# status-im/nim-blscurve

Measured on NVIDIA B200. Metric: batch-verified signature sets/sec, higher is better.
Workload: dtype u32x12 (Fp 381-bit Montgomery)

## Files before the change

nim_blscurve_b200/csrc/acc_team.cuh:

```cuda
#pragma once
#include "pairing.cuh"

namespace bls {

#define ACC_TPW 5
#define ACC_BS 128
#define ACC_TPB (ACC_TPW * ACC_BS / 32)

enum { FV_C0 = 0, FV_C1 = 1, FV_S = 2, FV_D = 3, FV_DD = 4 };
struct __align__(16) acc_team_sm {
    fp f[6][5];
    fp l[9];
};

#ifdef __CUDACC__
template <int K>
__device__ __forceinline__ void fp_dot(fp &r, const uint32_t (&a)[K][12], const fp *const (&b)[K]) {
#ifdef __CUDA_ARCH__
    uint32_t E[13], O[12];
#pragma unroll
    for (int i = 0; i < 12; i++) { E[i] = 0; O[i] = 0; }
    E[12] = 0;
    uint32_t bl[K][4];
#pragma unroll
    for (int i = 0; i < 12; i++) {
        if ((i & 3) == 0) {
#pragma unroll
            for (int t = 0; t < K; t++) {
                uint4 v = ((const uint4 *)b[t])[i >> 2];
                bl[t][0] = v.x; bl[t][1] = v.y; bl[t][2] = v.z; bl[t][3] = v.w;
            }
        }
        if (i == 0) {
            mad6(O, a[0][1], a[0][3], a[0][5], a[0][7], a[0][9], a[0][11], bl[0][0]);
        } else {
            uint32_t s = E[1];
            uint32_t nO[12];
#pragma unroll
            for (int k = 0; k < 11; k++) nO[k] = E[k + 2];
            nO[11] = 0;
#pragma unroll
            for (int k = 0; k < 12; k++) E[k] = O[k];
            E[12] = 0;
#pragma unroll
            for (int k = 0; k < 12; k++) O[k] = nO[k];
            mad6_stray(O, E[0], s, a[0][1], a[0][3], a[0][5], a[0][7], a[0][9], a[0][11], bl[0][i & 3]);
        }
        mad6_top(E, a[0][0], a[0][2], a[0][4], a[0][6], a[0][8], a[0][10], bl[0][i & 3]);
#pragma unroll
        for (int t = 1; t < K; t++) {
            mad6(O, a[t][1], a[t][3], a[t][5], a[t][7], a[t][9], a[t][11], bl[t][i & 3]);
            mad6_top(E, a[t][0], a[t][2], a[t][4], a[t][6], a[t][8], a[t][10], bl[t][i & 3]);
        }
        const uint32_t m = E[0] * BLS_N0;
        mad6(O, P32(1), P32(3), P32(5), P32(7), P32(9), P32(11), m);
        mad6_top(E, P32(0), P32(2), P32(4), P32(6), P32(8), P32(10), m);
    }
    add12(O, E + 1);
    reduce_once12(r.l, O);
#endif
}

__device__ __forceinline__ void load_fp_regs(uint32_t (&dst)[12], const fp *src) {
    const uint4 *s = (const uint4 *)src;
    uint4 v0 = s[0], v1 = s[1], v2 = s[2];
    dst[0] = v0.x; dst[1] = v0.y; dst[2] = v0.z; dst[3] = v0.w;
    dst[4] = v1.x; dst[5] = v1.y; dst[6] = v1.z; dst[7] = v1.w;
    dst[8] = v2.x; dst[9] = v2.y; dst[10] = v2.z; dst[11] = v2.w;
}

__device__ __noinline__ void team_dot3(fp &r, const fp *a0, const fp *a1, const fp *a2, const fp *b0, const fp *b1, const fp *b2) {
    uint32_t a[3][12];
    load_fp_regs(a[0], a0);
    load_fp_regs(a[1], a1);
    load_fp_regs(a[2], a2);
    const fp *const b[3] = {b0, b1, b2};
    fp t;
    fp_dot<3>(t, a, b);
    r = t;
}

__device__ __noinline__ void team_dot4(fp &r, const fp *const *ap, const fp *const *bp, uint32_t dbl_mask, uint32_t zero_mask) {
    uint32_t a[4][12];
#pragma unroll
    for (int t = 0; t < 4; t++) {
        fp x;
        load_fp_regs(x.l, ap[t]);
        fp x2;
        fp_dbl(x2, x);
        const bool d = (dbl_mask >> t) & 1, z = (zero_mask >> t) & 1;
#pragma unroll
        for (int i = 0; i < 12; i++) a[t][i] = z ? 0u : (d ? x2.l[i] : x.l[i]);
    }
    const fp *const b[4] = {bp[0], bp[1], bp[2], bp[3]};
    fp t;
    fp_dot<4>(t, a, b);
    r = t;
}

__device__ __forceinline__ void team_store_coeff(acc_team_sm &T, int k, const fp &c0, const fp &c1) {
    fp s, d, dd;
    fp_add(s, c0, c1);
    fp_sub(d, c0, c1);
    fp_dbl(dd, c0);
    T.f[k][FV_C0] = c0;
    T.f[k][FV_C1] = c1;
    T.f[k][FV_S] = s;
    T.f[k][FV_D] = d;
    T.f[k][FV_DD] = dd;
}

__device__ __forceinline__ void team_operand(const acc_team_sm &T, int j, bool x, const fp *&re, const fp *&im, const fp *&sum) {
    re = x ? &T.f[j][FV_D] : &T.f[j][FV_C0];
    im = x ? &T.f[j][FV_S] : &T.f[j][FV_C1];
    sum = x ? &T.f[j][FV_DD] : &T.f[j][FV_S];
}

__device__ __forceinline__ void team_mul_line(acc_team_sm &T, int k, uint32_t mask) {
    const fp *x0[3], *x1[3], *sx[3];
    team_operand(T, k, false, x0[0], x1[0], sx[0]);
    team_operand(T, (k + 4) % 6, k < 2, x0[1], x1[1], sx[1]);
    team_operand(T, (k + 3) % 6, k < 3, x0[2], x1[2], sx[2]);
    fp D0, D1, D2, c0, c1;
    team_dot3(D0, &T.l[0], &T.l[2], &T.l[4], x0[0], x0[1], x0[2]);
    team_dot3(D1, &T.l[1], &T.l[3], &T.l[5], x1[0], x1[1], x1[2]);
    team_dot3(D2, &T.l[6], &T.l[7], &T.l[8], sx[0], sx[1], sx[2]);
    fp_sub(c0, D0, D1);
    fp_sub(c1, D2, D0);
    fp_sub(c1, c1, D1);
    __syncwarp(mask);
    team_store_coeff(T, k, c0, c1);
    __syncwarp(mask);
}

__device__ __forceinline__ void team_square(acc_team_sm &T, int k, uint32_t mask) {
    const int LI[6][4] = {{0, 3, 1, 2}, {0, 2, 3, 0}, {1, 4, 0, 3}, {0, 1, 4, 0}, {2, 5, 0, 1}, {0, 1, 2, 0}};
    const int RI[6][4] = {{0, 3, 5, 4}, {1, 5, 4, 0}, {1, 4, 2, 5}, {3, 2, 5, 0}, {2, 5, 4, 3}, {5, 4, 3, 0}};
    const int XI[6][4] = {{0, 1, 1, 1}, {0, 1, 1, 0}, {0, 1, 0, 1}, {0, 0, 1, 0}, {0, 1, 0, 0}, {0, 0, 0, 0}};
    const uint32_t DBL[6] = {0xc, 0x7, 0xc, 0x7, 0xc, 0x7}, ZERO[6] = {0, 8, 0, 8, 0, 8};
    const fp *a0[4], *a1[4], *as[4], *b0[4], *b1[4], *bs[4];
#pragma unroll
    for (int t = 0; t < 4; t++) {
        team_operand(T, RI[k][t], false, a0[t], a1[t], as[t]);
        team_operand(T, LI[k][t], XI[k][t] != 0, b0[t], b1[t], bs[t]);
    }
    fp D0, D1, D2, c0, c1;
    team_dot4(D0, a0, b0, DBL[k], ZERO[k]);
    team_dot4(D1, a1, b1, DBL[k], ZERO[k]);
    team_dot4(D2, as, bs, DBL[k], ZERO[k]);
    fp_sub(c0, D0, D1);
    fp_sub(c1, D2, D0);
    fp_sub(c1, c1, D1);
    __syncwarp(mask);
    team_store_coeff(T, k, c0, c1);
    __syncwarp(mask);
}
#endif

}
```

nim_blscurve_b200/csrc/ec.cuh:

```cuda
#pragma once
#include "fpx.cuh"

namespace bls {

BLS_FN void f_add(fp &r, const fp &a, const fp &b) { fp_add(r, a, b); }
BLS_FN void f_sub(fp &r, const fp &a, const fp &b) { fp_sub(r, a, b); }
BLS_FN void f_dbl(fp &r, const fp &a) { fp_dbl(r, a); }
BLS_FN void f_neg(fp &r, const fp &a) { fp_neg(r, a); }
BLS_FN void f_mul(fp &r, const fp &a, const fp &b) { fp_mul_ni(r, a, b); }
BLS_FN void f_sqr(fp &r, const fp &a) { fp_sqr_ni(r, a); }
BLS_FN bool f_is_zero(const fp &a) { return fp_is_zero(a); }
BLS_FN bool f_eq(const fp &a, const fp &b) { return fp_eq(a, b); }
BLS_FN void f_set_zero(fp &r) { fp_set_zero(r); }
BLS_FN void f_set_one(fp &r) { r = FP_ONE; }
BLS_FN void f_inv(fp &r, const fp &a) { fp_inv(r, a); }

BLS_FN void f_add(fp2 &r, const fp2 &a, const fp2 &b) { fp2_add(r, a, b); }
BLS_FN void f_sub(fp2 &r, const fp2 &a, const fp2 &b) { fp2_sub(r, a, b); }
BLS_FN void f_dbl(fp2 &r, const fp2 &a) { fp2_dbl(r, a); }
BLS_FN void f_neg(fp2 &r, const fp2 &a) { fp2_neg(r, a); }
BLS_FN void f_mul(fp2 &r, const fp2 &a, const fp2 &b) { fp2_mul(r, a, b); }
BLS_FN void f_sqr(fp2 &r, const fp2 &a) { fp2_sqr(r, a); }
BLS_FN bool f_is_zero(const fp2 &a) { return fp2_is_zero(a); }
BLS_FN bool f_eq(const fp2 &a, const fp2 &b) { return fp2_eq(a, b); }
BLS_FN void f_set_zero(fp2 &r) { fp2_set_zero(r); }
BLS_FN void f_set_one(fp2 &r) { r.c0 = FP_ONE; fp_set_zero(r.c1); }
BLS_FN void f_inv(fp2 &r, const fp2 &a) { fp2_inv(r, a); }
BLS_FN void f_inv_vt(fp &r, const fp &a) { fp_inv_vartime(r, a); }
BLS_FN void f_inv_vt(fp2 &r, const fp2 &a) { fp2_inv_vartime(r, a); }

template <class F> struct jac_t { F x, y, z; };
template <class F> struct aff_t { F x, y; };
typedef jac_t<fp> g1_jac;
typedef aff_t<fp> g1_aff;
typedef jac_t<fp2> g2_jac;
typedef aff_t<fp2> g2_aff;

template <class F> BLS_FN bool pt_is_inf(const jac_t<F> &p) { return f_is_zero(p.z); }
template <class F> BLS_FN bool aff_is_inf(const aff_t<F> &p) { return f_is_zero(p.x) & f_is_zero(p.y); }
template <class F> BLS_FN void pt_set_inf(jac_t<F> &p) { f_set_zero(p.x); f_set_zero(p.y); f_set_zero(p.z); }
template <class F> BLS_FN void pt_from_affine(jac_t<F> &r, const aff_t<F> &a) {
    r.x = a.x;
    r.y = a.y;
    if (aff_is_inf(a)) f_set_zero(r.z); else f_set_one(r.z);
}
template <class F> BLS_FN void pt_neg(jac_t<F> &r, const jac_t<F> &a) { r.x = a.x; f_neg(r.y, a.y); r.z = a.z; }

template <class F> BLS_NOINLINE void pt_dbl(jac_t<F> &r, const jac_t<F> &p) {
    F A, B, C, D, E, Fq, t;
    f_sqr(A, p.x);
    f_sqr(B, p.y);
    f_sqr(C, B);
    f_add(t, p.x, B);
    f_sqr(t, t);
    f_sub(t, t, A);
    f_sub(t, t, C);
    f_dbl(D, t);
    f_dbl(E, A);
    f_add(E, E, A);
    f_sqr(Fq, E);
    f_mul(t, p.y, p.z);
    f_dbl(r.z, t);
    f_sub(Fq, Fq, D);
    f_sub(Fq, Fq, D);
    f_sub(t, D, Fq);
    f_mul(t, E, t);
    f_dbl(C, C);
    f_dbl(C, C);
    f_dbl(C, C);
    r.x = Fq;
    f_sub(r.y, t, C);
}

template <class F> BLS_NOINLINE void pt_dbl_a(jac_t<F> &r, const jac_t<F> &p, const F &a) {
    F XX, YY, YYYY, ZZ, S, M, T, t;
    f_sqr(XX, p.x);
    f_sqr(YY, p.y);
    f_sqr(YYYY, YY);
    f_sqr(ZZ, p.z);
    f_add(t, p.x, YY);
    f_sqr(t, t);
    f_sub(t, t, XX);
    f_sub(t, t, YYYY);
    f_dbl(S, t);
    f_sqr(t, ZZ);
    f_mul(t, a, t);
    f_dbl(M, XX);
    f_add(M, M, XX);
    f_add(M, M, t);
    f_sqr(T, M);
    f_sub(T, T, S);
    f_sub(T, T, S);
    f_add(t, p.y, p.z);
    f_sqr(t, t);
    f_sub(t, t, YY);
    f_sub(r.z, t, ZZ);
    r.x = T;
    f_sub(t, S, T);
    f_mul(t, M, t);
    f_dbl(YYYY, YYYY);
    f_dbl(YYYY, YYYY);
    f_dbl(YYYY, YYYY);
    f_sub(r.y, t, YYYY);
}

template <class F> BLS_NOINLINE void pt_add(jac_t<F> &r, const jac_t<F> &p, const jac_t<F> &q, const F *a_coeff = nullptr) {
    if (pt_is_inf(p)) { r = q; return; }
    if (pt_is_inf(q)) { r = p; return; }
    F Z1Z1, Z2Z2, U1, U2, S1, S2, H, I, J, rr, V, t;
    f_sqr(Z1Z1, p.z);
    f_sqr(Z2Z2, q.z);
    f_mul(U1, p.x, Z2Z2);
    f_mul(U2, q.x, Z1Z1);
    f_mul(t, q.z, Z2Z2);
    f_mul(S1, p.y, t);
    f_mul(t, p.z, Z1Z1);
    f_mul(S2, q.y, t);
    f_sub(H, U2, U1);
    f_sub(rr, S2, S1);
    if (f_is_zero(H)) {
        if (f_is_zero(rr)) {
            if (a_coeff) pt_dbl_a(r, p, *a_coeff); else pt_dbl(r, p);
        } else {
            pt_set_inf(r);
        }
        return;
    }
    f_dbl(rr, rr);
    f_dbl(I, H);
    f_sqr(I, I);
    f_mul(J, H, I);
    f_mul(V, U1, I);
    f_add(t, p.z, q.z);
    f_sqr(t, t);
    f_sub(t, t, Z1Z1);
    f_sub(t, t, Z2Z2);
    f_mul(r.z, t, H);
    f_sqr(t, rr);
    f_sub(t, t, J);
    f_sub(t, t, V);
    f_sub(t, t, V);
    r.x = t;
    f_sub(t, V, t);
    f_mul(t, rr, t);
    f_mul(S1, S1, J);
    f_dbl(S1, S1);
    f_sub(r.y, t, S1);
}

template <class F> BLS_NOINLINE void pt_add_affine(jac_t<F> &r, const jac_t<F> &p, const aff_t<F> &q) {
    if (aff_is_inf(q)) { r = p; return; }
    if (pt_is_inf(p)) { pt_from_affine(r, q); return; }
    F Z1Z1, U2, S2, H, HH, I, J, rr, V, t;
    f_sqr(Z1Z1, p.z);
    f_mul(U2, q.x, Z1Z1);
    f_mul(t, p.z, Z1Z1);
    f_mul(S2, q.y, t);
    f_sub(H, U2, p.x);
    f_sub(rr, S2, p.y);
    if (f_is_zero(H)) {
        if (f_is_zero(rr)) pt_dbl(r, p); else pt_set_inf(r);
        return;
    }
    f_dbl(rr, rr);
    f_sqr(HH, H);
    f_dbl(I, HH);
    f_dbl(I, I);
    f_mul(J, H, I);
    f_mul(V, p.x, I);
    f_add(t, p.z, H);
    f_sqr(t, t);
    f_sub(t, t, Z1Z1);
    F y1 = p.y;
    f_sub(r.z, t, HH);
    f_sqr(t, rr);
    f_sub(t, t, J);
    f_sub(t, t, V);
    f_sub(t, t, V);
    r.x = t;
    f_sub(t, V, t);
    f_mul(t, rr, t);
    f_mul(J, y1, J);
    f_dbl(J, J);
    f_sub(r.y, t, J);
}

template <class F> BLS_NOINLINE void pt_to_affine(aff_t<F> &r, const jac_t<F> &p) {
    if (pt_is_inf(p)) { f_set_zero(r.x); f_set_zero(r.y); return; }
    F zi, zi2;
    f_inv(zi, p.z);
    f_sqr(zi2, zi);
    f_mul(r.x, p.x, zi2);
    f_mul(zi2, zi2, zi);
    f_mul(r.y, p.y, zi2);
}

template <class F> BLS_NOINLINE void pt_to_affine_vt(aff_t<F> &r, const jac_t<F> &p) {
    if (pt_is_inf(p)) { f_set_zero(r.x); f_set_zero(r.y); return; }
    F zi, zi2;
    f_inv_vt(zi, p.z);
    f_sqr(zi2, zi);
    f_mul(r.x, p.x, zi2);
    f_mul(zi2, zi2, zi);
    f_mul(r.y, p.y, zi2);
}

template <class F> BLS_NOINLINE void pt_to_affine_zinv(aff_t<F> &r, const jac_t<F> &p, const F &zi) {
    if (pt_is_inf(p)) { f_set_zero(r.x); f_set_zero(r.y); return; }
    F zi2;
    f_sqr(zi2, zi);
    f_mul(r.x, p.x, zi2);
    f_mul(zi2, zi2, zi);
    f_mul(r.y, p.y, zi2);
}

template <class F> BLS_NOINLINE void pt_mul_u64(jac_t<F> &r, const aff_t<F> &p, uint64_t k) {
    jac_t<F> acc;
    pt_set_inf(acc);
    if (k != 0 && !aff_is_inf(p)) {
        int top = 63;
        while (!((k >> top) & 1)) top--;
        pt_from_affine(acc, p);
        for (int i = top - 1; i >= 0; i--) {
            pt_dbl(acc, acc);
            if ((k >> i) & 1) pt_add_affine(acc, acc, p);
        }
    }
    r = acc;
}

template <class F> BLS_NOINLINE void pt_mul_u64_w4(jac_t<F> &r, const aff_t<F> &p, uint64_t k) {
    jac_t<F> tbl[8], acc;
    pt_from_affine(tbl[0], p);
    pt_dbl(tbl[1], tbl[0]);
    pt_add_affine(tbl[2], tbl[1], p);
    pt_dbl(tbl[3], tbl[1]);
    pt_add_affine(tbl[4], tbl[3], p);
    pt_dbl(tbl[5], tbl[2]);
    pt_add_affine(tbl[6], tbl[5], p);
    pt_dbl(tbl[7], tbl[3]);
    int dig[17], carry = 0;
    for (int j = 0; j < 16; j++) {
        int w = (int)((k >> (4 * j)) & 15) + carry;
        if (w > 8) { w -= 16; carry = 1; } else carry = 0;
        dig[j] = w;
    }
    dig[16] = carry;
    pt_set_inf(acc);
    for (int j = 16; j >= 0; j--) {
        if (j != 16) for (int d = 0; d < 4; d++) pt_dbl(acc, acc);
        const int d = dig[j];
        if (d != 0) {
            jac_t<F> q = tbl[(d < 0 ? -d : d) - 1];
            if (d < 0) f_neg(q.y, q.y);
            pt_add(acc, acc, q);
        }
    }
    r = acc;
}

template <class F> BLS_NOINLINE void pt_mul_words(jac_t<F> &r, const jac_t<F> &p, const uint32_t *k, int nwords) {
    jac_t<F> acc;
    pt_set_inf(acc);
    int i = nwords * 32 - 1;
    while (i >= 0 && !((k[i >> 5] >> (i & 31)) & 1)) i--;
    for (; i >= 0; i--) {
        pt_dbl(acc, acc);
        if ((k[i >> 5] >> (i & 31)) & 1) pt_add(acc, acc, p);
    }
    r = acc;
}

}
```

nim_blscurve_b200/csrc/fp.cuh:

```cuda
#pragma once
#include <stdint.h>

#ifdef __CUDACC__
#define BLS_FN __device__ __forceinline__
#define BLS_HD __host__ __device__ __forceinline__
#define BLS_NOINLINE __device__ __noinline__
#define BLS_TABLE __device__ __constant__ const
#else
#define BLS_FN static inline
#define BLS_HD static inline
#define BLS_NOINLINE static
#define BLS_TABLE static const
#endif

namespace bls {

struct alignas(16) fp { uint32_t l[12]; };

BLS_FN constexpr uint32_t P32(int i) {
    return i == 0 ? 0xffffaaabu : i == 1 ? 0xb9feffffu : i == 2 ? 0xb153ffffu : i == 3 ? 0x1eabfffeu
         : i == 4 ? 0xf6b0f624u : i == 5 ? 0x6730d2a0u : i == 6 ? 0xf38512bfu : i == 7 ? 0x64774b84u
         : i == 8 ? 0x434bacd7u : i == 9 ? 0x4b1ba7b6u : i == 10 ? 0x397fe69au : 0x1a0111eau;
}
#define BLS_N0 0xfffcfffdu

BLS_FN void fp_set_zero(fp &r) {
#pragma unroll
    for (int i = 0; i < 12; i++) r.l[i] = 0;
}

BLS_FN bool fp_is_zero(const fp &a) {
    uint32_t t = 0;
#pragma unroll
    for (int i = 0; i < 12; i++) t |= a.l[i];
    return t == 0;
}

BLS_FN bool fp_eq(const fp &a, const fp &b) {
    uint32_t t = 0;
#pragma unroll
    for (int i = 0; i < 12; i++) t |= a.l[i] ^ b.l[i];
    return t == 0;
}

BLS_FN void fp_select(fp &r, bool c, const fp &a, const fp &b) {
#pragma unroll
    for (int i = 0; i < 12; i++) r.l[i] = c ? a.l[i] : b.l[i];
}

#ifdef __CUDA_ARCH__
#define BLS_R12(x) "+r"(x[0]), "+r"(x[1]), "+r"(x[2]), "+r"(x[3]), "+r"(x[4]), "+r"(x[5]), \
                   "+r"(x[6]), "+r"(x[7]), "+r"(x[8]), "+r"(x[9]), "+r"(x[10]), "+r"(x[11])

BLS_FN void add12(uint32_t *acc, const uint32_t *b) {
    asm("add.cc.u32 %0,%0,%12;\n\taddc.cc.u32 %1,%1,%13;\n\taddc.cc.u32 %2,%2,%14;\n\t"
        "addc.cc.u32 %3,%3,%15;\n\taddc.cc.u32 %4,%4,%16;\n\taddc.cc.u32 %5,%5,%17;\n\t"
        "addc.cc.u32 %6,%6,%18;\n\taddc.cc.u32 %7,%7,%19;\n\taddc.cc.u32 %8,%8,%20;\n\t"
        "addc.cc.u32 %9,%9,%21;\n\taddc.cc.u32 %10,%10,%22;\n\taddc.u32 %11,%11,%23;"
        : BLS_R12(acc)
        : "r"(b[0]), "r"(b[1]), "r"(b[2]), "r"(b[3]), "r"(b[4]), "r"(b[5]), "r"(b[6]), "r"(b[7]), "r"(b[8]),
          "r"(b[9]), "r"(b[10]), "r"(b[11]));
}

BLS_FN uint32_t sub12(uint32_t *acc, const uint32_t *b) {
    uint32_t bw;
    asm("sub.cc.u32 %0,%0,%13;\n\tsubc.cc.u32 %1,%1,%14;\n\tsubc.cc.u32 %2,%2,%15;\n\t"
        "subc.cc.u32 %3,%3,%16;\n\tsubc.cc.u32 %4,%4,%17;\n\tsubc.cc.u32 %5,%5,%18;\n\t"
        "subc.cc.u32 %6,%6,%19;\n\tsubc.cc.u32 %7,%7,%20;\n\tsubc.cc.u32 %8,%8,%21;\n\t"
        "subc.cc.u32 %9,%9,%22;\n\tsubc.cc.u32 %10,%10,%23;\n\tsubc.cc.u32 %11,%11,%24;\n\t"
        "subc.u32 %12,0,0;"
        : BLS_R12(acc), "=r"(bw)
        : "r"(b[0]), "r"(b[1]), "r"(b[2]), "r"(b[3]), "r"(b[4]), "r"(b[5]), "r"(b[6]), "r"(b[7]), "r"(b[8]),
          "r"(b[9]), "r"(b[10]), "r"(b[11]));
    return bw;
}

BLS_FN uint32_t sub_p12(uint32_t *acc) {
    uint32_t bw;
    asm("sub.cc.u32 %0,%0,0xffffaaab;\n\tsubc.cc.u32 %1,%1,0xb9feffff;\n\tsubc.cc.u32 %2,%2,0xb153ffff;\n\t"
        "subc.cc.u32 %3,%3,0x1eabfffe;\n\tsubc.cc.u32 %4,%4,0xf6b0f624;\n\tsubc.cc.u32 %5,%5,0x6730d2a0;\n\t"
        "subc.cc.u32 %6,%6,0xf38512bf;\n\tsubc.cc.u32 %7,%7,0x64774b84;\n\tsubc.cc.u32 %8,%8,0x434bacd7;\n\t"
        "subc.cc.u32 %9,%9,0x4b1ba7b6;\n\tsubc.cc.u32 %10,%10,0x397fe69a;\n\tsubc.cc.u32 %11,%11,0x1a0111ea;\n\t"
        "subc.u32 %12,0,0;"
        : BLS_R12(acc), "=r"(bw));
    return bw;
}

BLS_FN void add_p12(uint32_t *acc) {
    asm("add.cc.u32 %0,%0,0xffffaaab;\n\taddc.cc.u32 %1,%1,0xb9feffff;\n\taddc.cc.u32 %2,%2,0xb153ffff;\n\t"
        "addc.cc.u32 %3,%3,0x1eabfffe;\n\taddc.cc.u32 %4,%4,0xf6b0f624;\n\taddc.cc.u32 %5,%5,0x6730d2a0;\n\t"
        "addc.cc.u32 %6,%6,0xf38512bf;\n\taddc.cc.u32 %7,%7,0x64774b84;\n\taddc.cc.u32 %8,%8,0x434bacd7;\n\t"
        "addc.cc.u32 %9,%9,0x4b1ba7b6;\n\taddc.cc.u32 %10,%10,0x397fe69a;\n\taddc.u32 %11,%11,0x1a0111ea;"
        : BLS_R12(acc));
}

BLS_FN void reduce_once12(uint32_t *r, const uint32_t *t) {
    uint32_t u[12];
#pragma unroll
    for (int i = 0; i < 12; i++) u[i] = t[i];
    uint32_t bw = sub_p12(u);
#pragma unroll
    for (int i = 0; i < 12; i++) r[i] = bw ? t[i] : u[i];
}

#define BLS_LANE_C(lo, hi, a, b) \
    "madc.lo.cc.u32 " lo "," a "," b "," lo ";\n\tmadc.hi.cc.u32 " hi "," a "," b "," hi ";\n\t"
#define BLS_LANE_0(lo, hi, a, b) \
    "mad.lo.cc.u32 " lo "," a "," b "," lo ";\n\tmadc.hi.cc.u32 " hi "," a "," b "," hi ";\n\t"

BLS_FN void mad6_top(uint32_t *acc, uint32_t x0, uint32_t x1, uint32_t x2, uint32_t x3, uint32_t x4,
                     uint32_t x5, uint32_t m) {
    asm(BLS_LANE_0("%0", "%1", "%13", "%19") BLS_LANE_C("%2", "%3", "%14", "%19")
        BLS_LANE_C("%4", "%5", "%15", "%19") BLS_LANE_C("%6", "%7", "%16", "%19")
        BLS_LANE_C("%8", "%9", "%17", "%19") BLS_LANE_C("%10", "%11", "%18", "%19")
        "addc.u32 %12,%12,0;"
        : BLS_R12(acc), "+r"(acc[12])
        : "r"(x0), "r"(x1), "r"(x2), "r"(x3), "r"(x4), "r"(x5), "r"(m));
}

BLS_FN void mad6(uint32_t *acc, uint32_t x0, uint32_t x1, uint32_t x2, uint32_t x3, uint32_t x4,
                 uint32_t x5, uint32_t m) {
    asm(BLS_LANE_0("%0", "%1", "%12", "%18") BLS_LANE_C("%2", "%3", "%13", "%18")
        BLS_LANE_C("%4", "%5", "%14", "%18") BLS_LANE_C("%6", "%7", "%15", "%18")
        BLS_LANE_C("%8", "%9", "%16", "%18") BLS_LANE_C("%10", "%11", "%17", "%18")
        : BLS_R12(acc)
        : "r"(x0), "r"(x1), "r"(x2), "r"(x3), "r"(x4), "r"(x5), "r"(m));
}

BLS_FN void mad6_stray(uint32_t *acc, uint32_t &lo, uint32_t s, uint32_t x0, uint32_t x1, uint32_t x2,
                       uint32_t x3, uint32_t x4, uint32_t x5, uint32_t m) {
    asm("add.cc.u32 %12,%12,%13;\n\t"
        BLS_LANE_C("%0", "%1", "%14", "%20") BLS_LANE_C("%2", "%3", "%15", "%20")
        BLS_LANE_C("%4", "%5", "%16", "%20") BLS_LANE_C("%6", "%7", "%17", "%20")
        BLS_LANE_C("%8", "%9", "%18", "%20") BLS_LANE_C("%10", "%11", "%19", "%20")
        : BLS_R12(acc), "+r"(lo)
        : "r"(s), "r"(x0), "r"(x1), "r"(x2), "r"(x3), "r"(x4), "r"(x5), "r"(m));
}
#endif

BLS_FN void fp_add(fp &r, const fp &a, const fp &b) {
#ifdef __CUDA_ARCH__
    uint32_t t[12];
#pragma unroll
    for (int i = 0; i < 12; i++) t[i] = a.l[i];
    add12(t, b.l);
    reduce_once12(r.l, t);
#else
    uint32_t t[12], u[12];
    uint64_t c = 0;
    for (int i = 0; i < 12; i++) { c += (uint64_t)a.l[i] + b.l[i]; t[i] = (uint32_t)c; c >>= 32; }
    int64_t bw = 0;
    for (int i = 0; i < 12; i++) { bw += (int64_t)t[i] - P32(i); u[i] = (uint32_t)bw; bw >>= 32; }
    for (int i = 0; i < 12; i++) r.l[i] = bw ? t[i] : u[i];
#endif
}

BLS_FN void fp_sub(fp &r, const fp &a, const fp &b) {
#ifdef __CUDA_ARCH__
    uint32_t t[12], u[12];
#pragma unroll
    for (int i = 0; i < 12; i++) t[i] = a.l[i];
    uint32_t bw = sub12(t, b.l);
#pragma unroll
    for (int i = 0; i < 12; i++) u[i] = t[i];
    add_p12(u);
#pragma unroll
    for (int i = 0; i < 12; i++) r.l[i] = bw ? u[i] : t[i];
#else
    uint32_t t[12];
    int64_t bw = 0;
    for (int i = 0; i < 12; i++) { bw += (int64_t)a.l[i] - b.l[i]; t[i] = (uint32_t)bw; bw >>= 32; }
    uint64_t c = 0;
    for (int i = 0; i < 12; i++) { c += (uint64_t)t[i] + (bw ? P32(i) : 0u); r.l[i] = (uint32_t)c; c >>= 32; }
#endif
}

BLS_FN void fp_neg(fp &r, const fp &a) {
    fp z;
    fp_set_zero(z);
    fp_sub(r, z, a);
}

BLS_FN void fp_cneg(fp &r, const fp &a, bool c) {
    fp n;
    fp_neg(n, a);
    fp_select(r, c, n, a);
}

BLS_FN void fp_dbl(fp &r, const fp &a) { fp_add(r, a, a); }

BLS_FN void fp_mul(fp &r, const fp &a, const fp &b) {
#ifdef __CUDA_ARCH__
    uint32_t E[13], O[12];
#pragma unroll
    for (int i = 0; i < 12; i++) { E[i] = 0; O[i] = 0; }
    E[12] = 0;
#pragma unroll
    for (int i = 0; i < 12; i++) {
        const uint32_t bi = b.l[i];
        if (i == 0) {
            mad6(O, a.l[1], a.l[3], a.l[5], a.l[7], a.l[9], a.l[11], bi);
        } else {
            uint32_t s = E[1];
            uint32_t nO[12];
#pragma unroll
            for (int k = 0; k < 11; k++) nO[k] = E[k + 2];
            nO[11] = 0;
#pragma unroll
            for (int k = 0; k < 12; k++) E[k] = O[k];
            E[12] = 0;
#pragma unroll
            for (int k = 0; k < 12; k++) O[k] = nO[k];
            mad6_stray(O, E[0], s, a.l[1], a.l[3], a.l[5], a.l[7], a.l[9], a.l[11], bi);
        }
        mad6_top(E, a.l[0], a.l[2], a.l[4], a.l[6], a.l[8], a.l[10], bi);
        const uint32_t m = E[0] * BLS_N0;
        mad6(O, P32(1), P32(3), P32(5), P32(7), P32(9), P32(11), m);
        mad6_top(E, P32(0), P32(2), P32(4), P32(6), P32(8), P32(10), m);
    }
    add12(O, E + 1);
    reduce_once12(r.l, O);
#else
#ifdef BLS_COUNT_MULS
    extern unsigned long long g_fp_mul_count;
    g_fp_mul_count++;
#endif
    uint32_t t[14];
    for (int i = 0; i < 14; i++) t[i] = 0;
    for (int i = 0; i < 12; i++) {
        uint64_t c = 0;
        for (int j = 0; j < 12; j++) {
            c += (uint64_t)a.l[j] * b.l[i] + t[j];
            t[j] = (uint32_t)c; c >>= 32;
        }
        c += t[12]; t[12] = (uint32_t)c; t[13] = (uint32_t)(c >> 32);
        uint32_t m = t[0] * BLS_N0;
        c = ((uint64_t)m * P32(0) + t[0]) >> 32;
        for (int j = 1; j < 12; j++) {
            c += (uint64_t)m * P32(j) + t[j];
            t[j - 1] = (uint32_t)c; c >>= 32;
        }
        c += t[12]; t[11] = (uint32_t)c;
        t[12] = t[13] + (uint32_t)(c >> 32);
    }
    uint32_t u[12];
    int64_t bw = 0;
    for (int i = 0; i < 12; i++) { bw += (int64_t)t[i] - P32(i); u[i] = (uint32_t)bw; bw >>= 32; }
    for (int i = 0; i < 12; i++) r.l[i] = bw ? t[i] : u[i];
#endif
}

}
#include "fp_gen.cuh"
namespace bls {

BLS_FN void fp_sqr(fp &r, const fp &a) {
#if defined(__CUDA_ARCH__) && !defined(BLS_NO_FP_SQR)
    uint32_t t[12];
    fp_sqr_ptx(t, a.l);
    reduce_once12(r.l, t);
#else
    fp_mul(r, a, a);
#endif
}

BLS_FN void fp_from_mont(fp &r, const fp &a) {
    fp one;
    fp_set_zero(one);
    one.l[0] = 1;
    fp_mul(r, a, one);
}

BLS_FN uint32_t fp_parity(const fp &a) {
    fp t;
    fp_from_mont(t, a);
    return t.l[0] & 1;
}

BLS_FN bool fp_is_lexically_largest_canon(const fp &c) {
    uint64_t carry = 0;
    uint32_t d[13];
    for (int i = 0; i < 12; i++) {
        carry += ((uint64_t)c.l[i] << 1);
        d[i] = (uint32_t)carry;
        carry >>= 32;
    }
    d[12] = (uint32_t)carry;
    int64_t bw = 0;
    for (int i = 0; i < 12; i++) { bw += (int64_t)d[i] - P32(i); bw >>= 32; }
    bw += d[12];
    return bw >= 0;
}

}
```

nim_blscurve_b200/csrc/fp2.cuh:

```cuda
#pragma once
#include "fp.cuh"

namespace bls {

struct fp2 { fp c0, c1; };

BLS_NOINLINE void fp_mul_ni(fp &r, const fp &a, const fp &b) {
    fp x = a, y = b, t;
    fp_mul(t, x, y);
    r = t;
}
BLS_NOINLINE void fp_sqr_ni(fp &r, const fp &a) {
    fp x = a, t;
    fp_sqr(t, x);
    r = t;
}

#if defined(__CUDACC__) && !defined(BLS_SMALL_CODE)
#define BLS_SMALL_CODE 1
#endif
#if defined(BLS_SMALL_CODE) && BLS_SMALL_CODE >= 2
BLS_NOINLINE void fp_add_ni(fp &r, const fp &a, const fp &b) { fp t; fp_add(t, a, b); r = t; }
BLS_NOINLINE void fp_sub_ni(fp &r, const fp &a, const fp &b) { fp t; fp_sub(t, a, b); r = t; }
#define FP_ADD fp_add_ni
#define FP_SUB fp_sub_ni
#define FP_MUL fp_mul_ni
#elif defined(BLS_SMALL_CODE) && BLS_SMALL_CODE >= 1
#define FP_ADD fp_add
#define FP_SUB fp_sub
#define FP_MUL fp_mul_ni
#else
#define FP_ADD fp_add
#define FP_SUB fp_sub
#define FP_MUL fp_mul
#endif

BLS_FN void fp2_set_zero(fp2 &r) { fp_set_zero(r.c0); fp_set_zero(r.c1); }
BLS_FN bool fp2_is_zero(const fp2 &a) { return fp_is_zero(a.c0) & fp_is_zero(a.c1); }
BLS_FN bool fp2_eq(const fp2 &a, const fp2 &b) { return fp_eq(a.c0, b.c0) & fp_eq(a.c1, b.c1); }
BLS_FN void fp2_select(fp2 &r, bool c, const fp2 &a, const fp2 &b) {
    fp_select(r.c0, c, a.c0, b.c0);
    fp_select(r.c1, c, a.c1, b.c1);
}
BLS_FN void fp2_add(fp2 &r, const fp2 &a, const fp2 &b) { FP_ADD(r.c0, a.c0, b.c0); FP_ADD(r.c1, a.c1, b.c1); }
BLS_FN void fp2_sub(fp2 &r, const fp2 &a, const fp2 &b) { FP_SUB(r.c0, a.c0, b.c0); FP_SUB(r.c1, a.c1, b.c1); }
BLS_FN void fp2_neg(fp2 &r, const fp2 &a) { fp_neg(r.c0, a.c0); fp_neg(r.c1, a.c1); }
BLS_FN void fp2_dbl(fp2 &r, const fp2 &a) { FP_ADD(r.c0, a.c0, a.c0); FP_ADD(r.c1, a.c1, a.c1); }
BLS_FN void fp2_conj(fp2 &r, const fp2 &a) { r.c0 = a.c0; fp_neg(r.c1, a.c1); }
BLS_FN void fp2_cneg(fp2 &r, const fp2 &a, bool c) { fp_cneg(r.c0, a.c0, c); fp_cneg(r.c1, a.c1, c); }

BLS_FN void fp2_mul_xi(fp2 &r, const fp2 &a) {
    fp t0, t1;
    FP_SUB(t0, a.c0, a.c1);
    FP_ADD(t1, a.c0, a.c1);
    r.c0 = t0;
    r.c1 = t1;
}

#ifdef __CUDA_ARCH__
BLS_FN void mul_wide12(uint32_t *T, const uint32_t *a, const uint32_t *b) {
    uint32_t E[13], O[12];
#pragma unroll
    for (int i = 0; i < 12; i++) { E[i] = 0; O[i] = 0; }
    E[12] = 0;
#pragma unroll
    for (int i = 0; i < 12; i++) {
        const uint32_t bi = b[i];
        if (i == 0) {
            mad6(O, a[1], a[3], a[5], a[7], a[9], a[11], bi);
        } else {
            uint32_t s = E[1];
            uint32_t nO[12];
#pragma unroll
            for (int k = 0; k < 11; k++) nO[k] = E[k + 2];
            nO[11] = 0;
#pragma unroll
            for (int k = 0; k < 12; k++) E[k] = O[k];
            E[12] = 0;
#pragma unroll
            for (int k = 0; k < 12; k++) O[k] = nO[k];
            mad6_stray(O, E[0], s, a[1], a[3], a[5], a[7], a[9], a[11], bi);
        }
        mad6_top(E, a[0], a[2], a[4], a[6], a[8], a[10], bi);
        T[i] = E[0];
    }
    add12(O, E + 1);
#pragma unroll
    for (int k = 0; k < 12; k++) T[12 + k] = O[k];
}
BLS_FN void redc24(uint32_t *r, const uint32_t *T) {
    uint32_t E[13], O[12];
#pragma unroll
    for (int i = 0; i < 12; i++) { E[i] = T[i]; O[i] = 0; }
    E[12] = 0;
#pragma unroll
    for (int i = 0; i < 12; i++) {
        uint32_t m;
        if (i == 0) {
            m = E[0] * BLS_N0;
            mad6(O, P32(1), P32(3), P32(5), P32(7), P32(9), P32(11), m);
        } else {
            uint32_t s = E[1];
            uint32_t nO[12];
#pragma unroll
            for (int k = 0; k < 11; k++) nO[k] = E[k + 2];
            nO[11] = 0;
#pragma unroll
            for (int k = 0; k < 12; k++) E[k] = O[k];
            E[12] = 0;
#pragma unroll
            for (int k = 0; k < 12; k++) O[k] = nO[k];
            m = (E[0] + s) * BLS_N0;
            mad6_stray(O, E[0], s, P32(1), P32(3), P32(5), P32(7), P32(9), P32(11), m);
        }
        mad6_top(E, P32(0), P32(2), P32(4), P32(6), P32(8), P32(10), m);
    }
    add12(O, E + 1);
    add12(O, T + 12);
    reduce_once12(r, O);
}
BLS_FN uint32_t sub12_b(uint32_t *acc, const uint32_t *b, uint32_t bw_in) {
    uint32_t bw;
    asm("{\n\t.reg .u32 t;\n\tsub.cc.u32 t,0,%25;\n\tsubc.cc.u32 %0,%0,%13;\n\tsubc.cc.u32 %1,%1,%14;\n\tsubc.cc.u32 %2,%2,%15;\n\t"
        "subc.cc.u32 %3,%3,%16;\n\tsubc.cc.u32 %4,%4,%17;\n\tsubc.cc.u32 %5,%5,%18;\n\t"
        "subc.cc.u32 %6,%6,%19;\n\tsubc.cc.u32 %7,%7,%20;\n\tsubc.cc.u32 %8,%8,%21;\n\t"
        "subc.cc.u32 %9,%9,%22;\n\tsubc.cc.u32 %10,%10,%23;\n\tsubc.cc.u32 %11,%11,%24;\n\t"
        "subc.u32 %12,0,0;\n\t}"
        : BLS_R12(acc), "=r"(bw)
        : "r"(b[0]), "r"(b[1]), "r"(b[2]), "r"(b[3]), "r"(b[4]), "r"(b[5]), "r"(b[6]), "r"(b[7]), "r"(b[8]),
          "r"(b[9]), "r"(b[10]), "r"(b[11]), "r"(bw_in));
    return bw;
}
BLS_FN uint32_t sub24(uint32_t *acc, const uint32_t *b) {
    const uint32_t bw = sub12(acc, b);
    return sub12_b(acc + 12, b + 12, bw);
}
#endif

BLS_NOINLINE void fp2_mul_r3(fp2 &r, const fp2 &a, const fp2 &b) {
    fp s0, s1, t0, t1, t2;
    FP_ADD(s0, a.c0, a.c1);
    FP_ADD(s1, b.c0, b.c1);
    FP_MUL(t2, s0, s1);
    FP_MUL(t0, a.c0, b.c0);
    FP_MUL(t1, a.c1, b.c1);
    FP_SUB(t2, t2, t0);
    FP_SUB(t2, t2, t1);
    FP_SUB(t0, t0, t1);
    r.c0 = t0;
    r.c1 = t2;
}

#ifndef BLS_FP2_LAZY
#define BLS_FP2_LAZY 0
#endif

BLS_NOINLINE void fp2_mul(fp2 &r, const fp2 &a, const fp2 &b) {
#if defined(__CUDA_ARCH__) && BLS_FP2_LAZY
    uint32_t T2[24], T0[24];
    {
        uint32_t s0[12], s1[12];
#pragma unroll
        for (int i = 0; i < 12; i++) { s0[i] = a.c0.l[i]; s1[i] = b.c0.l[i]; }
        add12(s0, a.c1.l);
        add12(s1, b.c1.l);
        mul_wide12(T2, s0, s1);
    }
    mul_wide12(T0, a.c0.l, b.c0.l);
    sub24(T2, T0);
    {
        uint32_t T1[24];
        mul_wide12(T1, a.c1.l, b.c1.l);
        sub24(T2, T1);
        const uint32_t bw = sub24(T0, T1);
        uint32_t u[12];
#pragma unroll
        for (int i = 0; i < 12; i++) u[i] = T0[12 + i];
        add_p12(u);
#pragma unroll
        for (int i = 0; i < 12; i++) T0[12 + i] = bw ? u[i] : T0[12 + i];
    }
    fp re, im;
    redc24(im.l, T2);
    redc24(re.l, T0);
    r.c0 = re;
    r.c1 = im;
    return;
#else
    fp2_mul_r3(r, a, b);
#endif
}

BLS_NOINLINE void fp2_sqr(fp2 &r, const fp2 &a) {
    fp s, d, t, u;
    FP_ADD(s, a.c0, a.c1);
    FP_SUB(d, a.c0, a.c1);
    FP_MUL(u, s, d);
    FP_MUL(t, a.c0, a.c1);
    FP_ADD(t, t, t);
    r.c0 = u;
    r.c1 = t;
}

BLS_FN void fp2_mul_fp(fp2 &r, const fp2 &a, const fp &k) {
    fp_mul_ni(r.c0, a.c0, k);
    fp_mul_ni(r.c1, a.c1, k);
}

BLS_FN void fp2_mul3(fp2 &r, const fp2 &a) { fp2 t; fp2_dbl(t, a); fp2_add(r, t, a); }
BLS_FN void fp_mul3(fp &r, const fp &a) { fp t; fp_dbl(t, a); fp_add(r, t, a); }

}
```

nim_blscurve_b200/csrc/fp2h.cuh:

```cuda
#pragma once
#include "tower.cuh"

namespace bls {
#ifdef __CUDACC__

struct fp2h { fp v; };

__device__ __forceinline__ bool h_odd() { return (threadIdx.x & 1) != 0; }
__device__ __forceinline__ uint32_t h_mask() { return 3u << (threadIdx.x & 30); }

__device__ __forceinline__ void h_xchg(fp &r, const fp &a) {
    const uint32_t m = h_mask();
#pragma unroll
    for (int i = 0; i < 12; i++) r.l[i] = __shfl_xor_sync(m, a.l[i], 1);
}
__device__ __forceinline__ bool h_both(bool mine) {
    const uint32_t m = h_mask();
    return mine & (__shfl_xor_sync(m, (int)mine, 1) != 0);
}
__device__ __forceinline__ void h_take(fp2h &r, const fp2 &a) { r.v = h_odd() ? a.c1 : a.c0; }
__device__ __forceinline__ void h_full(fp2 &r, const fp2h &a) {
    fp o;
    h_xchg(o, a.v);
    const bool odd = h_odd();
    fp_select(r.c0, odd, o, a.v);
    fp_select(r.c1, odd, a.v, o);
}

__device__ __forceinline__ void fp_dot2(fp &r, const fp &x0, const fp &y0, const fp &x1, const fp &y1) {
#ifdef __CUDA_ARCH__
    uint32_t E[13], O[12];
#pragma unroll
    for (int i = 0; i < 12; i++) { E[i] = 0; O[i] = 0; }
    E[12] = 0;
#pragma unroll
    for (int i = 0; i < 12; i++) {
        if (i == 0) {
            mad6(O, x0.l[1], x0.l[3], x0.l[5], x0.l[7], x0.l[9], x0.l[11], y0.l[0]);
        } else {
            uint32_t s = E[1];
            uint32_t nO[12];
#pragma unroll
            for (int k = 0; k < 11; k++) nO[k] = E[k + 2];
            nO[11] = 0;
#pragma unroll
            for (int k = 0; k < 12; k++) E[k] = O[k];
            E[12] = 0;
#pragma unroll
            for (int k = 0; k < 12; k++) O[k] = nO[k];
            mad6_stray(O, E[0], s, x0.l[1], x0.l[3], x0.l[5], x0.l[7], x0.l[9], x0.l[11], y0.l[i]);
        }
        mad6_top(E, x0.l[0], x0.l[2], x0.l[4], x0.l[6], x0.l[8], x0.l[10], y0.l[i]);
        mad6(O, x1.l[1], x1.l[3], x1.l[5], x1.l[7], x1.l[9], x1.l[11], y1.l[i]);
        mad6_top(E, x1.l[0], x1.l[2], x1.l[4], x1.l[6], x1.l[8], x1.l[10], y1.l[i]);
        const uint32_t m = E[0] * BLS_N0;
        mad6(O, P32(1), P32(3), P32(5), P32(7), P32(9), P32(11), m);
        mad6_top(E, P32(0), P32(2), P32(4), P32(6), P32(8), P32(10), m);
    }
    add12(O, E + 1);
    reduce_once12(r.l, O);
#endif
}

BLS_NOINLINE void h_mul(fp2h &r, const fp2h &a, const fp2h &b) {
    fp ao = a.v, bo = b.v, ap, bp, nap, x0, x1, t;
    h_xchg(ap, ao);
    h_xchg(bp, bo);
    fp_neg(nap, ap);
    const bool odd = h_odd();
    fp_select(x0, odd, ap, ao);
    fp_select(x1, odd, ao, nap);
    fp_dot2(t, x0, bo, x1, bp);
    r.v = t;
}
BLS_NOINLINE void h_sqr(fp2h &r, const fp2h &a) {
    fp ao = a.v, ap, x, y, d, t;
    h_xchg(ap, ao);
    const bool odd = h_odd();
    fp_select(t, odd, ao, ap);
    fp_add(x, ao, t);
    fp_sub(d, ao, ap);
    fp_select(y, odd, ap, d);
    fp_mul(t, x, y);
    r.v = t;
}
__device__ __forceinline__ void h_mul_fp(fp2h &r, const fp2h &a, const fp &k) { fp_mul_ni(r.v, a.v, k); }
__device__ __forceinline__ void h_mul_xi(fp2h &r, const fp2h &a) {
    fp ap, s, d;
    h_xchg(ap, a.v);
    fp_add(s, a.v, ap);
    fp_sub(d, a.v, ap);
    fp_select(r.v, h_odd(), s, d);
}
__device__ __forceinline__ void h_conj(fp2h &r, const fp2h &a) { fp_cneg(r.v, a.v, h_odd()); }
__device__ __forceinline__ void h_cneg(fp2h &r, const fp2h &a, bool c) { fp_cneg(r.v, a.v, c); }
__device__ __forceinline__ void h_mul3(fp2h &r, const fp2h &a) { fp t; fp_dbl(t, a.v); fp_add(r.v, t, a.v); }
BLS_NOINLINE void h_inv(fp2h &r, const fp2h &a) {
    fp n, np, t;
    fp_sqr_ni(n, a.v);
    h_xchg(np, n);
    fp_add(n, n, np);
    fp_inv(n, n);
    fp_mul_ni(t, a.v, n);
    fp_cneg(r.v, t, h_odd());
}

__device__ __forceinline__ void f_add(fp2h &r, const fp2h &a, const fp2h &b) { fp_add(r.v, a.v, b.v); }
__device__ __forceinline__ void f_sub(fp2h &r, const fp2h &a, const fp2h &b) { fp_sub(r.v, a.v, b.v); }
__device__ __forceinline__ void f_dbl(fp2h &r, const fp2h &a) { fp_add(r.v, a.v, a.v); }
__device__ __forceinline__ void f_neg(fp2h &r, const fp2h &a) { fp_neg(r.v, a.v); }
__device__ __forceinline__ void f_mul(fp2h &r, const fp2h &a, const fp2h &b) { h_mul(r, a, b); }
__device__ __forceinline__ void f_sqr(fp2h &r, const fp2h &a) { h_sqr(r, a); }
__device__ __forceinline__ bool f_is_zero(const fp2h &a) { return h_both(fp_is_zero(a.v)); }
__device__ __forceinline__ bool f_eq(const fp2h &a, const fp2h &b) { return h_both(fp_eq(a.v, b.v)); }
__device__ __forceinline__ void f_set_zero(fp2h &r) { fp_set_zero(r.v); }
__device__ __forceinline__ void f_set_one(fp2h &r) { if (h_odd()) fp_set_zero(r.v); else r.v = FP_ONE; }
__device__ __forceinline__ void f_inv(fp2h &r, const fp2h &a) { h_inv(r, a); }
__device__ __forceinline__ void f_inv_vt(fp2h &r, const fp2h &a) { h_inv(r, a); }

typedef jac_t<fp2h> g2h_jac;
typedef aff_t<fp2h> g2h_aff;

#endif
}
```

nim_blscurve_b200/csrc/fpx.cuh:

```cuda
#pragma once
#include "consts.cuh"

namespace bls {

BLS_NOINLINE void fp_pow_chain(fp &r, const fp &a, int first, const uint8_t (*ops)[2], int len) {
    fp tbl[16];
    fp a2, acc;
    tbl[0] = a;
    fp_sqr_ni(a2, a);
    for (int i = 1; i < 16; i++) fp_mul_ni(tbl[i], tbl[i - 1], a2);
    acc = tbl[first];
    for (int k = 0; k < len; k++) {
        int ns = ops[k][0], idx = ops[k][1];
        for (int s = 0; s < ns; s++) fp_sqr_ni(acc, acc);
        if (idx != 255) fp_mul_ni(acc, acc, tbl[idx]);
    }
    r = acc;
}

BLS_FN void fp_inv(fp &r, const fp &a) { fp_pow_chain(r, a, CHAIN_PM2_FIRST, CHAIN_PM2_OPS, CHAIN_PM2_LEN); }

BLS_NOINLINE void fp_inv_vartime(fp &r, const fp &a) {
    if (fp_is_zero(a)) { fp_set_zero(r); return; }
    uint32_t u[12], v[12], x1[12], x2[12];
#pragma unroll
    for (int i = 0; i < 12; i++) { u[i] = a.l[i]; v[i] = P32(i); x1[i] = 0; x2[i] = 0; }
    x1[0] = 1;
    auto is_one = [](const uint32_t *t) {
        uint32_t z = t[0] ^ 1u;
#pragma unroll
        for (int i = 1; i < 12; i++) z |= t[i];
        return z == 0;
    };
    auto halve = [](uint32_t *t, uint32_t *x) {
#pragma unroll
        for (int i = 0; i < 11; i++) t[i] = (t[i] >> 1) | (t[i + 1] << 31);
        t[11] >>= 1;
        uint32_t top = 0;
        if (x[0] & 1) {
            uint64_t c = 0;
#pragma unroll
            for (int i = 0; i < 12; i++) { c += (uint64_t)x[i] + P32(i); x[i] = (uint32_t)c; c >>= 32; }
            top = (uint32_t)c;
        }
#pragma unroll
        for (int i = 0; i < 11; i++) x[i] = (x[i] >> 1) | (x[i + 1] << 31);
        x[11] = (x[11] >> 1) | (top << 31);
    };
    auto sub_step = [](uint32_t *t, const uint32_t *s, uint32_t *x, const uint32_t *y) {
        int64_t bw = 0;
#pragma unroll
        for (int i = 0; i < 12; i++) { bw += (int64_t)t[i] - s[i]; t[i] = (uint32_t)bw; bw >>= 32; }
        bw = 0;
#pragma unroll
        for (int i = 0; i < 12; i++) { bw += (int64_t)x[i] - y[i]; x[i] = (uint32_t)bw; bw >>= 32; }
        if (bw) {
            uint64_t c = 0;
#pragma unroll
            for (int i = 0; i < 12; i++) { c += (uint64_t)x[i] + P32(i); x[i] = (uint32_t)c; c >>= 32; }
        }
    };
    while (!is_one(u) && !is_one(v)) {
        while (!(u[0] & 1)) halve(u, x1);
        while (!(v[0] & 1)) halve(v, x2);
        bool ge = true;
        for (int i = 11; i >= 0; i--) if (u[i] != v[i]) { ge = u[i] > v[i]; break; }
        if (ge) sub_step(u, v, x1, x2); else sub_step(v, u, x2, x1);
    }
    fp x, t;
    const bool first = is_one(u);
#pragma unroll
    for (int i = 0; i < 12; i++) x.l[i] = first ? x1[i] : x2[i];
    fp_mul_ni(t, x, FP_R2);
    fp_mul_ni(r, t, FP_R2);
}

BLS_FN void fp_pow_p34(fp &r, const fp &a) { fp_pow_chain(r, a, CHAIN_P34_FIRST, CHAIN_P34_OPS, CHAIN_P34_LEN); }

BLS_NOINLINE void fp2_inv(fp2 &r, const fp2 &a) {
    fp n, t;
    fp_sqr_ni(n, a.c0);
    fp_sqr_ni(t, a.c1);
    fp_add(n, n, t);
    fp_inv(n, n);
    fp_mul_ni(r.c0, a.c0, n);
    fp_mul_ni(t, a.c1, n);
    fp_neg(r.c1, t);
}

BLS_NOINLINE void fp2_inv_vartime(fp2 &r, const fp2 &a) {
    fp n, t;
    fp_sqr_ni(n, a.c0);
    fp_sqr_ni(t, a.c1);
    fp_add(n, n, t);
    fp_inv_vartime(n, n);
    fp_mul_ni(r.c0, a.c0, n);
    fp_mul_ni(t, a.c1, n);
    fp_neg(r.c1, t);
}

BLS_FN uint32_t fp2_sgn0(const fp2 &a) {
    uint32_t s0 = fp_parity(a.c0), s1 = fp_parity(a.c1);
    return fp_is_zero(a.c0) ? s1 : s0;
}

BLS_FN bool fp2_is_lexically_largest(const fp2 &a) {
    fp c0, c1;
    fp_from_mont(c0, a.c0);
    fp_from_mont(c1, a.c1);
    return fp_is_zero(c1) ? fp_is_lexically_largest_canon(c0) : fp_is_lexically_largest_canon(c1);
}

BLS_NOINLINE bool fp2_rsqrt_or_z(fp2 &r, const fp2 &a_in) {
    fp2 a = a_in;
    fp n, t, rs, s, chk;
    fp_sqr_ni(n, a.c0);
    fp_sqr_ni(t, a.c1);
    fp_add(n, n, t);
    fp_pow_p34(rs, n);
    fp_mul_ni(s, rs, n);
    fp_mul_ni(chk, s, rs);
    bool is_sq = fp_eq(chk, FP_ONE) | fp_is_zero(n);
    if (!is_sq) {
        fp2 za;
        fp2_mul(za, a, SSWU_Z);
        a = za;
        fp_mul_ni(n, n, FP_FIVE);
        fp_mul_ni(rs, rs, FP_C5);
        fp_mul_ni(s, rs, n);
    }
    fp h, e, x, xi, other, two_inv_x;
    fp_add(h, a.c0, s);
    fp_mul_ni(h, h, FP_INV2);
    if (fp_is_zero(h)) {
        fp_sub(h, a.c0, s);
        fp_mul_ni(h, h, FP_INV2);
    }
    fp_pow_p34(e, h);
    fp_mul_ni(x, e, h);
    fp_mul_ni(chk, x, e);
    bool h_sq = fp_eq(chk, FP_ONE);
    fp_mul_ni(xi, e, chk);
    fp_mul_ni(two_inv_x, xi, FP_INV2);
    fp_mul_ni(other, a.c1, two_inv_x);
    fp2 root;
    if (h_sq) {
        root.c0 = x;
        root.c1 = other;
    } else {
        root.c0 = other;
        root.c1 = x;
    }
    fp nr, t2;
    fp_sqr_ni(nr, root.c0);
    fp_sqr_ni(t2, root.c1);
    fp_add(nr, nr, t2);
    bool pos = fp_eq(nr, s);
    fp sc;
    fp_cneg(sc, rs, !pos);
    fp_mul_ni(r.c0, root.c0, sc);
    fp_mul_ni(t2, root.c1, sc);
    fp_neg(r.c1, t2);
    return is_sq;
}

}
```

nim_blscurve_b200/csrc/kernels.cuh:

```cuda
#pragma once
#include <cuda_runtime.h>
#include "h2c.cuh"
#include "pairing.cuh"
#include "acc_team.cuh"
#include "io.cuh"
#include "pair_route.cuh"
#include "tma_stage.cuh"
#include "fplin.cuh"

namespace bls {

constexpr int fpprog_const_count = 36;

#ifndef BLS_LB_BLOCKS
#define BLS_LB_BLOCKS 4
#endif
#define BLS_LB __launch_bounds__(128, BLS_LB_BLOCKS)

struct sigset { g1_aff pk; uint8_t msg[32]; g2_aff sig; };
static_assert(sizeof(sigset) == 320, "SignatureSet layout (bls_batch_verifier.nim:34)");
static_assert(sizeof(fp12) == 576 && sizeof(g2_jac) == 288 && sizeof(g1_jac) == 144, "layout");


struct words8 { uint32_t w[8]; };

__device__ __forceinline__ void sha256_of_32(uint32_t *out, const uint32_t *in) {
    uint32_t h[8] = {0x6a09e667u, 0xbb67ae85u, 0x3c6ef372u, 0xa54ff53au, 0x510e527fu, 0x9b05688cu, 0x1f83d9abu, 0x5be0cd19u};
    uint32_t w[16];
#pragma unroll
    for (int i = 0; i < 8; i++) w[i] = in[i];
    w[8] = 0x80000000u;
#pragma unroll
    for (int i = 9; i < 15; i++) w[i] = 0;
    w[15] = 256;
    sha256_block_regs(h, w);
#pragma unroll
    for (int i = 0; i < 8; i++) out[i] = h[i];
}

__device__ __forceinline__ uint64_t le64_of_be_words(const uint32_t *d) {
    uint32_t lo = __byte_perm(d[0], 0, 0x0123), hi = __byte_perm(d[1], 0, 0x0123);
    return ((uint64_t)hi << 32) | lo;
}

__device__ __forceinline__ void chunk_range(size_t nchunks, size_t total, size_t cid, size_t &off, size_t &len) {
    size_t base = total / nchunks, rem = total % nchunks;
    if (cid < rem) { off = (base + 1) * cid; len = base + 1; }
    else { off = base * cid + rem; len = base; }
}

__device__ __forceinline__ unsigned long long gtimer() { unsigned long long t; asm volatile("mov.u64 %0, %%globaltimer;" : "=l"(t)); return t; }
__device__ __forceinline__ unsigned smid() { unsigned v; asm volatile("mov.u32 %0, %%smid;" : "=r"(v)); return v; }
__device__ __forceinline__ void rlc_chains(words8 &srb, const uint32_t *d_srb, size_t total_n, uint32_t chunks, size_t first,
                                           size_t n, uint64_t *out, unsigned long long *dbg, size_t block) {
    if (d_srb) for (int k = 0; k < 8; k++) srb.w[k] = d_srb[k];
    size_t nb = chunks == 0 ? 1 : (total_n < chunks ? total_n : (size_t)chunks);
    size_t c = block * blockDim.x + threadIdx.x;
    if (c >= nb) return;
    size_t off, len;
    chunk_range(nb, total_n, c, off, len);
    if (off >= first + n || off + len <= first) return;
    uint32_t seed[8];
    if (chunks == 0) {
        sha256_of_32(seed, srb.w);
    } else {
        uint32_t h[8] = {0x6a09e667u, 0xbb67ae85u, 0x3c6ef372u, 0xa54ff53au, 0x510e527fu, 0x9b05688cu, 0x1f83d9abu, 0x5be0cd19u};
        uint32_t w[16];
        for (int i = 0; i < 8; i++) w[i] = srb.w[i];
        w[8] = __byte_perm((uint32_t)c, 0, 0x0123);
        w[9] = __byte_perm((uint32_t)((uint64_t)c >> 32), 0, 0x0123);
        w[10] = 0x80000000u;
        for (int i = 11; i < 15; i++) w[i] = 0;
        w[15] = 320;
        sha256_block(h, w);
        for (int i = 0; i < 8; i++) seed[i] = h[i];
    }
    for (size_t i = off; i < off + len; i++) {
        uint64_t r;
        do {
            uint32_t t[8];
            sha256_of_32(t, seed);
#pragma unroll
            for (int k = 0; k < 8; k++) seed[k] = t[k];
            r = le64_of_be_words(seed);
        } while (r == 0);
        if (i >= first && i < first + n) out[i - first] = r;
    }
    if (dbg && c == 0) dbg[1] = gtimer();
}
__global__ void k_rlc_scalars(words8 srb, const uint32_t *d_srb, size_t total_n, uint32_t chunks, size_t first, size_t n,
                              uint64_t *out, volatile int *started, unsigned long long *dbg = nullptr) {
    if (started && blockIdx.x == 0 && threadIdx.x == 0) { *started = 1; __threadfence(); }
    if (dbg && blockIdx.x == 0 && threadIdx.x == 0) { dbg[0] = gtimer(); dbg[3] = smid(); }
    rlc_chains(srb, d_srb, total_n, chunks, first, n, out, dbg, blockIdx.x);
}

__global__ void k_wait_started(volatile int *started, long long budget, unsigned long long *dbg = nullptr) {
    if (blockIdx.x != 0 || threadIdx.x != 0) return;
    const long long t0 = clock64();
    while (*started == 0 && clock64() - t0 < budget) __nanosleep(200);
    if (dbg) { dbg[2] = gtimer(); dbg[4] = *started; }
}

__global__ void k_combine_scalars(words8 srb, size_t n, uint64_t *out) {
    if (blockIdx.x != 0 || threadIdx.x != 0) return;
    uint32_t seed[8];
    for (int k = 0; k < 8; k++) seed[k] = srb.w[k];
    int avail = 0;
    for (size_t i = 0; i < n; i++) {
        for (;;) {
            if (avail == 0) {
                uint32_t t[8];
                sha256_of_32(t, seed);
                for (int k = 0; k < 8; k++) seed[k] = t[k];
                avail = 4;
            }
            avail--;
            uint64_t v = le64_of_be_words(seed + 2 * avail);
            if (v != 0) { out[i] = v; break; }
        }
    }
}

__global__ void BLS_LB k_hash_sets(const sigset *sets, size_t n, g2_jac *H) {
    __shared__ __align__(128) uint8_t tile[128 * 32];
    __shared__ uint64_t bar;
    const size_t base = (size_t)blockIdx.x * blockDim.x;
    const size_t cnt = n - base < blockDim.x ? n - base : blockDim.x;
    tma_stage_rows(tile, 32, sets[base].msg, sizeof(sigset), (uint32_t)cnt, &bar);
    size_t i = base + threadIdx.x;
    if (i >= n) return;
    alignas(16) uint8_t msg[32];
    {
        const uint4 *m = (const uint4 *)(tile + 32 * threadIdx.x);
        uint4 m0 = m[0], m1 = m[1];
        *(uint4 *)msg = m0;
        *(uint4 *)(msg + 16) = m1;
    }
    g2_jac h;
    hash_to_g2_jac_eth2(h, msg);
    H[i] = h;
}

__global__ void BLS_LB k_hash_sets_pair(const sigset *sets, size_t n, g2_jac *H) {
    const size_t t = (size_t)blockIdx.x * blockDim.x + threadIdx.x;
    const size_t i = t >> 1;
    const bool odd = t & 1;
    const bool live = i < n;
    uint8_t msg[32], dst[43];
    for (int k = 0; k < 32; k++) msg[k] = live ? sets[i].msg[k] : 0;
    for (int k = 0; k < 43; k++) dst[k] = DST_ETH2[k];
    fp2 u0, u1;
    hash_to_field_fp2x2(u0, u1, msg, 32, dst, 43);
    g2_jac q, other;
    sswu_g2(q, odd ? u1 : u0);
    {
        uint32_t *d = (uint32_t *)&other;
        const uint32_t *sp = (const uint32_t *)&q;
        for (int k = 0; k < (int)(sizeof(g2_jac) / 4); k++) d[k] = __shfl_down_sync(0xffffffffu, sp[k], 1);
    }
    if (odd || !live) return;
    pt_add(q, q, other, &SSWU_A);
    iso3_g2(q, q);
    g2_jac h;
    g2_clear_cofactor(h, q);
    H[i] = h;
}

__global__ void BLS_LB k_hash_sets_lanes2(const sigset *sets, size_t n, g2_jac *H) {
    __shared__ __align__(128) uint8_t tile[64 * 32];
    __shared__ uint64_t bar;
    const size_t base = (size_t)blockIdx.x * (blockDim.x >> 1);
    const size_t cnt = n - base < (blockDim.x >> 1) ? n - base : (blockDim.x >> 1);
    tma_stage_rows(tile, 32, sets[base].msg, sizeof(sigset), (uint32_t)cnt, &bar);
    const size_t i = base + (threadIdx.x >> 1);
    if (i >= n) return;
    alignas(16) uint8_t msg[32];
    {
        const uint4 *m = (const uint4 *)(tile + 32 * (threadIdx.x >> 1));
        *(uint4 *)msg = m[0];
        *(uint4 *)(msg + 16) = m[1];
    }
    g2h_jac h;
    hash_to_g2_pair(h, msg, 32, nullptr, 0);
    fp *out = (fp *)&H[i] + (h_odd() ? 1 : 0);
    out[0] = h.x.v;
    out[2] = h.y.v;
    out[4] = h.z.v;
}
__global__ void __launch_bounds__(128, BLS_LB_BLOCKS) k_miller_lines_lanes2(const g2_aff *Q, const g1_aff *P, size_t np,
                                                                            uint32_t *lines, size_t stride) {
    const size_t t = (size_t)blockIdx.x * blockDim.x + threadIdx.x;
    const size_t p = t >> 1;
    if (p >= np) return;
    const fp *q = (const fp *)&Q[p] + (h_odd() ? 1 : 0);
    g2h_aff qh;
    qh.x.v = q[0];
    qh.y.v = q[2];
    g1_aff a = P[p];
    const bool inf = (f_is_zero(qh.x) & f_is_zero(qh.y)) | aff_is_inf(a);
    miller_lines_pair(qh, a, inf, lines + p, stride);
}

BLS_NOINLINE void g2_jac_to_hom(fp *hom, const g2_jac &p) {
    fp2 x, y, z;
    if (pt_is_inf(p)) {
        fp2_set_zero(x); fp2_set_zero(y); y.c0 = FP_ONE; fp2_set_zero(z);
    } else {
        fp2 z2;
        fp2_mul(x, p.x, p.z);
        y = p.y;
        fp2_sqr(z2, p.z);
        fp2_mul(z, z2, p.z);
    }
    hom[0] = x.c0; hom[1] = x.c1; hom[2] = y.c0; hom[3] = y.c1; hom[4] = z.c0; hom[5] = z.c1;
}
__global__ void BLS_LB k_hash_map_pair(const sigset *sets, size_t n, fp *hom) {
    const size_t t = (size_t)blockIdx.x * blockDim.x + threadIdx.x;
    const size_t i = t >> 1;
    const bool odd = t & 1;
    const bool live = i < n;
    uint8_t msg[32], dst[43];
    for (int k = 0; k < 32; k++) msg[k] = live ? sets[i].msg[k] : 0;
    for (int k = 0; k < 43; k++) dst[k] = DST_ETH2[k];
    fp2 u0, u1;
    hash_to_field_fp2x2(u0, u1, msg, 32, dst, 43);
    g2_jac q, other;
    sswu_g2(q, odd ? u1 : u0);
    {
        uint32_t *d = (uint32_t *)&other;
        const uint32_t *sp = (const uint32_t *)&q;
        for (int k = 0; k < (int)(sizeof(g2_jac) / 4); k++) d[k] = __shfl_down_sync(0xffffffffu, sp[k], 1);
    }
    if (odd || !live) return;
    pt_add(q, q, other, &SSWU_A);
    iso3_g2(q, q);
    g2_jac_to_hom(hom + 6 * i, q);
}
__global__ void BLS_LB k_hash_map_lanes2(const sigset *sets, const uint8_t *msgs, const uint32_t *offs, const uint8_t *dst_g,
                                         uint32_t dst_len, size_t n, fp *hom) {
    const size_t t = (size_t)blockIdx.x * blockDim.x + threadIdx.x;
    const size_t i = t >> 1;
    if (i >= n) return;
    g2h_jac q;
    if (msgs) {
        hash_map_to_e2_pair(q, msgs + offs[i], offs[i + 1] - offs[i], dst_g, dst_len);
    } else {
        uint8_t msg[32];
        for (int k = 0; k < 32; k++) msg[k] = sets[i].msg[k];
        hash_map_to_e2_pair(q, msg, 32, nullptr, 0);
    }
    fp2h X, Y, Z;
    jac_to_hom_pair(X, Y, Z, q);
    fp *out = hom + 6 * i + (h_odd() ? 1 : 0);
    out[0] = X.v;
    out[2] = Y.v;
    out[4] = Z.v;
}
__global__ void BLS_LB k_hash_map_pair_msgs(const uint8_t *msgs, const uint32_t *offs, const uint8_t *dst, uint32_t dst_len,
                                            size_t n, fp *hom) {
    const size_t t = (size_t)blockIdx.x * blockDim.x + threadIdx.x;
    const size_t i = t >> 1;
    const bool odd = t & 1;
    const bool live = i < n;
    const size_t j = live ? i : 0;
    fp2 u0, u1;
    hash_to_field_fp2x2(u0, u1, msgs + offs[j], offs[j + 1] - offs[j], dst, dst_len);
    g2_jac q, other;
    sswu_g2(q, odd ? u1 : u0);
    {
        uint32_t *d = (uint32_t *)&other;
        const uint32_t *sp = (const uint32_t *)&q;
        for (int k = 0; k < (int)(sizeof(g2_jac) / 4); k++) d[k] = __shfl_down_sync(0xffffffffu, sp[k], 1);
    }
    if (odd || !live) return;
    pt_add(q, q, other, &SSWU_A);
    iso3_g2(q, q);
    g2_jac_to_hom(hom + 6 * i, q);
}
__global__ void k_g2_hom_to_affine(const fp *hom, size_t n, g2_aff *out) {
    if (threadIdx.x != 0 || blockIdx.x >= n) return;
    const fp *h = hom + 6 * (size_t)blockIdx.x;
    fp2 X, Y, Z, zi;
    X.c0 = h[0]; X.c1 = h[1]; Y.c0 = h[2]; Y.c1 = h[3]; Z.c0 = h[4]; Z.c1 = h[5];
    g2_aff a;
    fp2_inv_vartime(zi, Z);
    fp2_mul(a.x, X, zi);
    fp2_mul(a.y, Y, zi);
    out[blockIdx.x] = a;
}
__global__ void k_g2_hom_to_jac(const fp *hom, size_t n, g2_jac *out) {
    const size_t i = (size_t)blockIdx.x * blockDim.x + threadIdx.x;
    if (i >= n) return;
    const fp *h = hom + 6 * i;
    fp2 X, Y, Z;
    X.c0 = h[0]; X.c1 = h[1]; Y.c0 = h[2]; Y.c1 = h[3]; Z.c0 = h[4]; Z.c1 = h[5];
    g2_jac j;
    if (fp2_is_zero(Z)) pt_set_inf(j);
    else { fp2 z2; fp2_mul(j.x, X, Z); fp2_sqr(z2, Z); fp2_mul(j.y, Y, z2); j.z = Z; }
    out[i] = j;
}
__global__ void k_g2_mul_prep(const sigset *sets, const uint64_t *r, size_t n, fp *hom, fp *bits) {
    const size_t t = (size_t)blockIdx.x * blockDim.x + threadIdx.x;
    const size_t i = t >> 6;
    const int b = (int)(t & 63);
    if (i >= n) return;
    fp v;
    if ((r[i] >> b) & 1) v = FP_ONE; else fp_set_zero(v);
    bits[64 * i + b] = v;
    if (b == 0) {
        g2_aff a = sets[i].sig;
        g2_jac j;
        pt_from_affine(j, a);
        g2_jac_to_hom(hom + 6 * i, j);
    }
}

__global__ void BLS_LB k_g1_mul(const sigset *sets, const uint64_t *r, size_t n, g1_jac *Pj, int *flags) {
    __shared__ __align__(128) sigset tile[128];
    __shared__ uint64_t bar;
    const size_t base = (size_t)blockIdx.x * blockDim.x;
    const size_t cnt = n - base < blockDim.x ? n - base : blockDim.x;
    tma_stage_tile(tile, sets + base, (uint32_t)(cnt * sizeof(sigset)), &bar);
    size_t i = base + threadIdx.x;
    if (i >= n) return;
    g1_aff pk = tile[threadIdx.x].pk;
    if (aff_is_inf(pk)) atomicOr(flags, 1);
    g1_jac j;
    pt_mul_u64_w4(j, pk, r[i]);
    Pj[i] = j;
}

#define AFF_B 8
__global__ void BLS_LB k_pairs_affine(const g2_jac *H, const g1_jac *Pj, size_t n, g2_aff *Q, g1_aff *P, int vartime, int spread,
                                      int per) {
    __shared__ fp sc[2][128];
    __shared__ fp sinv;
    size_t t = (size_t)blockIdx.x * blockDim.x + threadIdx.x, nthreads = (size_t)gridDim.x * blockDim.x;
    if (spread) {
        if (threadIdx.x != 0) return;
        t = blockIdx.x;
        nthreads = gridDim.x;
    }
    const bool block_mode = vartime == 2;
    if (t >= n && !block_mode) return;
    fp nz[AFF_B], zp[AFF_B], pre[AFF_B];
    int cnt = 0;
    for (int k = 0; k < per; k++) {
        const size_t i = t + (size_t)k * nthreads;
        if (i >= n) break;
        fp2 hz = H[i].z;
        fp a, b;
        fp_sqr_ni(a, hz.c0);
        fp_sqr_ni(b, hz.c1);
        fp_add(a, a, b);
        b = Pj[i].z;
        if (fp_is_zero(a)) a = FP_ONE;
        if (fp_is_zero(b)) b = FP_ONE;
        nz[k] = a;
        zp[k] = b;
        fp c;
        fp_mul_ni(c, a, b);
        if (k) fp_mul_ni(pre[k], pre[k - 1], c); else pre[k] = c;
        cnt = k + 1;
    }
    fp inv;
    if (block_mode) {
        const int tid = threadIdx.x;
        fp tot;
        if (cnt) tot = pre[cnt - 1]; else tot = FP_ONE;
        sc[0][tid] = tot;
        sc[1][tid] = tot;
        __syncthreads();
        for (int d = 1; d < 128; d <<= 1) {
            fp a, b, x, y;
            const bool ha = tid >= d, hb = tid + d < 128;
            if (ha) { a = sc[0][tid - d]; x = sc[0][tid]; }
            if (hb) { b = sc[1][tid + d]; y = sc[1][tid]; }
            __syncthreads();
            if (ha) { fp_mul_ni(x, x, a); sc[0][tid] = x; }
            if (hb) { fp_mul_ni(y, y, b); sc[1][tid] = y; }
            __syncthreads();
        }
        if (tid == 0) { fp all = sc[0][127], r; fp_inv_vartime(r, all); sinv = r; }
        __syncthreads();
        inv = sinv;
        if (tid > 0) { fp a = sc[0][tid - 1]; fp_mul_ni(inv, inv, a); }
        if (tid < 127) { fp b = sc[1][tid + 1]; fp_mul_ni(inv, inv, b); }
        if (!cnt) return;
    } else if (vartime) fp_inv_vartime(inv, pre[cnt - 1]);
    else fp_inv(inv, pre[cnt - 1]);
    for (int k = cnt - 1; k >= 0; k--) {
        const size_t i = t + (size_t)k * nthreads;
        fp ik, ninv, zpinv, tt;
        if (k) {
            fp_mul_ni(ik, inv, pre[k - 1]);
            fp_mul_ni(tt, nz[k], zp[k]);
            fp_mul_ni(inv, inv, tt);
        } else {
            ik = inv;
        }
        fp_mul_ni(ninv, ik, zp[k]);
        fp_mul_ni(zpinv, ik, nz[k]);
        g2_jac h = H[i];
        g1_jac p = Pj[i];
        fp2 zhinv;
        fp_mul_ni(zhinv.c0, h.z.c0, ninv);
        fp_mul_ni(tt, h.z.c1, ninv);
        fp_neg(zhinv.c1, tt);
        g2_aff q;
        g1_aff a;
        pt_to_affine_zinv(q, h, zhinv);
        pt_to_affine_zinv(a, p, zpinv);
        Q[i] = q;
        P[i] = a;
    }
}

__global__ void BLS_LB k_g2_mul(const sigset *sets, const uint64_t *r, size_t n, g2_jac *S) {
    size_t i = (size_t)blockIdx.x * blockDim.x + threadIdx.x;
    if (i >= n) return;
    g2_aff sig = sets[i].sig;
    g2_jac j;
    pt_mul_u64(j, sig, r[i]);
    S[i] = j;
}

__global__ void BLS_LB k_g2_tree(g2_jac *S, size_t n, size_t half) {
    size_t i = (size_t)blockIdx.x * blockDim.x + threadIdx.x;
    if (i >= half || i + half >= n) return;
    g2_jac a = S[i], b = S[i + half];
    pt_add(a, a, b);
    S[i] = a;
}

__global__ void BLS_LB k_g1_tree(g1_jac *S, size_t n, size_t half) {
    size_t i = (size_t)blockIdx.x * blockDim.x + threadIdx.x;
    if (i >= half || i + half >= n) return;
    g1_jac a = S[i], b = S[i + half];
    pt_add(a, a, b);
    S[i] = a;
}

__global__ void BLS_LB k_fp12_tree(fp12 *F, size_t n, size_t half) {
    size_t i = (size_t)blockIdx.x * blockDim.x + threadIdx.x;
    if (i >= half || i + half >= n) return;
    fp12 a = F[i], b = F[i + half];
    fp12_mul(a, a, b);
    F[i] = a;
}


__global__ void k_sig_pair(const g2_jac *S, size_t n, g2_aff *Q, g1_aff *P) {
    if (blockIdx.x != 0 || threadIdx.x != 0) return;
    g2_jac s = *S;
    g2_aff sa;
    pt_to_affine_vt(sa, s);
    Q[n] = sa;
    g1_aff g;
    g.x = G1_GEN_X;
    fp_neg(g.y, G1_GEN_Y);
    P[n] = g;
}

#ifndef BLS_LINES_BLOCKS
#define BLS_LINES_BLOCKS 4
#endif
__global__ void __launch_bounds__(128, BLS_LINES_BLOCKS) k_miller_lines(const g2_aff *Q, const g1_aff *P, size_t np,
                                                                       uint32_t *lines, size_t stride) {
    size_t p = (size_t)blockIdx.x * blockDim.x + threadIdx.x;
    if (p >= np) return;
    g2_aff q = Q[p];
    g1_aff a = P[p];
    miller_lines(q, a, lines + p, stride);
}

__global__ void k_lines_from_prog(const uint32_t *prog_out, const g2_aff *Q, const g1_aff *P, size_t np, uint32_t *lines,
                                  size_t stride) {
    const size_t t = (size_t)blockIdx.x * blockDim.x + threadIdx.x;
    const size_t per = (size_t)ML_NLINES * ML_LINE_WORDS;
    if (t >= np * per) return;
    const size_t p = t % np, sw = t / np;
    uint32_t v;
    if (aff_is_inf(Q[p]) | aff_is_inf(P[p])) {
        const int w = (int)(sw % ML_LINE_WORDS);
        v = w < 12 ? FP_ONE.l[w] : 0u;
    } else {
        v = prog_out[p * per + sw];
    }
    lines[sw * stride + p] = v;
}

#define BLS_ACC_BS 128
#ifndef BLS_ACC_BLOCKS
#define BLS_ACC_BLOCKS 2
#endif
__device__ __forceinline__ void block_fp12_product(fp12 &f, uint32_t *sm, int live = BLS_ACC_BS) {
    const int tid = threadIdx.x;
    int top = BLS_ACC_BS / 2;
    while (top >= 1 && top >= live) top >>= 1;
    for (int half = top; half >= 1; half >>= 1) {
        if (tid >= half && tid < 2 * half) {
            const uint32_t *w = (const uint32_t *)&f;
            for (int k = 0; k < 144; k++) sm[k * half + (tid - half)] = w[k];
        }
        __syncthreads();
        if (tid < half) {
            fp12 b;
            uint32_t *w = (uint32_t *)&b;
            for (int k = 0; k < 144; k++) w[k] = sm[k * half + tid];
            fp12_mul(f, f, b);
        }
        __syncthreads();
    }
}

__global__ void __launch_bounds__(BLS_ACC_BS, BLS_ACC_BLOCKS) k_miller_acc(const uint32_t *lines, size_t stride, size_t np,
                                                                           size_t ngroups, int G, int nseg, fp12 *Fseg,
                                                                           size_t row_stride, size_t col_off) {
    __shared__ uint32_t sm[(BLS_ACC_BS / 2) * 144];
    const size_t g = (size_t)blockIdx.x * blockDim.x + threadIdx.x;
    const int j = blockIdx.y;
    fp12 f;
    if (g < ngroups) miller_accumulate(f, lines, stride, np, g, ngroups, G, ml_seg_hi(j, nseg), ml_seg_lo(j, nseg));
    else fp12_set_one(f);
    block_fp12_product(f, sm);
    if (threadIdx.x == 0) Fseg[(size_t)j * row_stride + col_off + blockIdx.x] = f;
}

#ifndef BLS_ACCT_BLOCKS
#define BLS_ACCT_BLOCKS 3
#endif
__global__ void __launch_bounds__(ACC_BS, BLS_ACCT_BLOCKS) k_miller_acc_team(const uint32_t *lines, size_t stride, size_t np,
                                                                            size_t ngroups, int G, int nseg, fp12 *Fteam,
                                                                            size_t row_stride, size_t col_off) {
    __shared__ acc_team_sm sm[ACC_TPB];
    const int lane = threadIdx.x & 31, warp = threadIdx.x >> 5;
    if (lane >= 6 * ACC_TPW) return;
    const uint32_t mask = (1u << (6 * ACC_TPW)) - 1;
    const int team = lane / 6, k = lane % 6;
    acc_team_sm &T = sm[warp * ACC_TPW + team];
    const size_t g = ((size_t)blockIdx.x * (ACC_BS / 32) + warp) * ACC_TPW + team;
    const int j = blockIdx.y, i_hi = ml_seg_hi(j, nseg), i_lo = ml_seg_lo(j, nseg);
    const bool team_valid = g < ngroups;
    bool first = true;
    for (int i = i_hi; i >= i_lo; i--) {
        if (!first) team_square(T, k, mask);
        const int s0 = ml_line_index(i), nl = 1 + ml_bit(i);
        for (int a = 0; a < nl; a++)
            for (int kk = 0; kk < G; kk++) {
                const size_t p = g + (size_t)kk * ngroups;
                fp v;
                if (team_valid && p < np) {
                    const uint32_t *src = lines + ((size_t)(s0 + a) * ML_LINE_WORDS + 12 * k) * stride + p;
#pragma unroll
                    for (int w = 0; w < 12; w++) v.l[w] = src[(size_t)w * stride];
                } else if (k == 0) {
                    v = FP_ONE;
                } else {
                    fp_set_zero(v);
                }
                T.l[k] = v;
                __syncwarp(mask);
                if (k < 3) { fp sum; fp_add(sum, T.l[2 * k], T.l[2 * k + 1]); T.l[6 + k] = sum; }
                __syncwarp(mask);
                if (first) {
                    fp c0, c1;
                    const int li = k == 0 ? 0 : (k == 2 ? 1 : (k == 3 ? 2 : -1));
                    if (li >= 0) { c0 = T.l[2 * li]; c1 = T.l[2 * li + 1]; } else { fp_set_zero(c0); fp_set_zero(c1); }
                    team_store_coeff(T, k, c0, c1);
                    __syncwarp(mask);
                    first = false;
                } else {
                    team_mul_line(T, k, mask);
                }
            }
    }
    if (team_valid) {
        fp2 *dst = (fp2 *)&Fteam[(size_t)j * row_stride + col_off + g];
        fp2 out;
        out.c0 = T.f[k][FV_C0];
        out.c1 = T.f[k][FV_C1];
        dst[3 * (k & 1) + (k >> 1)] = out;
    }
}

__global__ void __launch_bounds__(BLS_ACC_BS, BLS_ACC_BLOCKS) k_fp12_rows_step(const fp12 *in, size_t in_stride, size_t ncols,
                                                                               fp12 *out, size_t out_stride) {
    __shared__ uint32_t sm[(BLS_ACC_BS / 2) * 144];
    const size_t c = (size_t)blockIdx.x * BLS_ACC_BS + threadIdx.x;
    fp12 f;
    if (c < ncols) f = in[(size_t)blockIdx.y * in_stride + c]; else fp12_set_one(f);
    block_fp12_product(f, sm);
    if (threadIdx.x == 0) out[(size_t)blockIdx.y * out_stride + blockIdx.x] = f;
}

__global__ void k_fp12_pad_one(fp12 *F, size_t stride, size_t ncols) {
    const size_t c = ncols + threadIdx.x;
    if (c >= stride) return;
    fp12 one;
    fp12_set_one(one);
    F[(size_t)blockIdx.x * stride + c] = one;
}

__global__ void __launch_bounds__(BLS_ACC_BS, BLS_ACC_BLOCKS) k_fp12_rows(const fp12 *Fseg, size_t row_stride, size_t ncols,
                                                                          fp12 *seg) {
    __shared__ uint32_t sm[(BLS_ACC_BS / 2) * 144];
    const fp12 *row = Fseg + (size_t)blockIdx.x * row_stride;
    fp12 f;
    fp12_set_one(f);
    bool have = false;
    for (size_t c = threadIdx.x; c < ncols; c += BLS_ACC_BS) {
        fp12 b = row[c];
        if (have) fp12_mul(f, f, b); else { f = b; have = true; }
    }
    block_fp12_product(f, sm, ncols < BLS_ACC_BS ? (int)ncols : BLS_ACC_BS);
    if (threadIdx.x == 0) seg[blockIdx.x] = f;
}

__global__ void k_combine(const fp12 *seg, int nseg, fp12 *out) {
    if (blockIdx.x != 0 || threadIdx.x != 0) return;
    fp12 F;
    miller_combine(F, seg, nseg);
    *out = F;
}

__global__ void k_partial_one(fp12 *out, int *flag_out) {
    if (blockIdx.x != 0 || threadIdx.x != 0) return;
    fp12 one;
    fp12_set_one(one);
    *out = one;
    if (flag_out) *flag_out = 0;
}
__global__ void k_partial_seal(const int *flags, uint32_t *partial, int *flag_out) {
    const int f = flags[0];
    if (flag_out && threadIdx.x == 0) *flag_out = f;
    if (f) for (int w = threadIdx.x; w < 144; w += blockDim.x) partial[w] = 0u;
}

__global__ void k_fill_consts(fp *dst) {
    const int t = threadIdx.x;
    if (t >= fpprog_const_count) return;
    const fp *src;
    int k;
    if (t < 10) { src = (const fp *)FROB1; k = t; }
    else if (t < 20) { src = (const fp *)FROB2; k = t - 10; }
    else if (t < 30) { src = (const fp *)FROB3; k = t - 20; }
    else if (t < 32) { src = (const fp *)&PSI_CX; k = t - 30; }
    else if (t < 34) { src = (const fp *)&PSI_CY; k = t - 32; }
    else if (t < 35) { src = &PSI2_CX; k = 0; }
    else { src = &FP_ONE; k = 0; }
    dst[t] = src[k];
}

template <bool STREAM>
__device__ __forceinline__ void fp_program_body(const uint32_t *prog, const fp *in0, const fp *in1, const fp *cst, fp *out0,
                                                size_t s_in0, size_t s_in1, size_t s_out) {
    extern __shared__ uint4 sm4[];
    fp *slots = (fp *)sm4;
    const int lane = threadIdx.x;
    if (s_in0 != ~(size_t)0) {
        in0 += (size_t)blockIdx.x * s_in0;
        if (in1) in1 += (size_t)blockIdx.x * s_in1;
        out0 += (size_t)blockIdx.x * s_out;
    }
    const uint32_t nr = prog[0], nin = prog[2], nout = prog[3];
    if (lane == 0) fp_set_zero(slots[0]);
    for (uint32_t e = lane; e < nin; e += 32) {
        uint32_t sl = prog[4 + 2 * e], ref = prog[5 + 2 * e], buf = ref >> 24, idx = ref & 0xffffffu;
        const fp *src = buf == 0 ? in0 : (buf == 1 ? in1 : cst);
        slots[sl] = src[idx];
    }
    __syncwarp();
    const uint32_t *rp = prog + 4 + 2 * (nin + nout) + lane;
    uint32_t wq[4];
#pragma unroll
    for (int k = 0; k < 4; k++) wq[k] = (uint32_t)k < nr ? rp[32 * k] : 0u;
    for (uint32_t r = 0; r < nr; r += 4) {
#pragma unroll
        for (int k = 0; k < 4; k++) {
            const uint32_t w = wq[k];
            wq[k] = r + k + 4 < nr ? rp[32 * (r + k + 4)] : 0u;
            if (STREAM) {
                const uint32_t opc = w >> 30;
                if (opc) {
                    fp x = slots[(w >> 10) & 1023], y = slots[w & 1023], t;
                    if (opc == 1) fp_mul(t, x, y);
                    else if (opc == 2) fp_add(t, x, y);
                    else fp_sub(t, x, y);
                    slots[(w >> 20) & 1023] = t;
                } else if (w) {
                    out0[(((w >> 20) & 1023) << 10) | (w & 1023)] = slots[(w >> 10) & 1023];
                }
            } else if (w) {
                fp x = slots[(w >> 10) & 1023], y = slots[w & 1023], t;
                const uint32_t opc = w >> 30;
                if (opc == 1) fp_mul(t, x, y);
                else if (opc == 2) fp_add(t, x, y);
                else fp_sub(t, x, y);
                slots[(w >> 20) & 1023] = t;
            }
            __syncwarp();
        }
    }
    const uint32_t *op = prog + 4 + 2 * nin;
    for (uint32_t e = lane; e < nout; e += 32) out0[op[2 * e + 1] & 0xffffffu] = slots[op[2 * e]];
}
__global__ void __launch_bounds__(32) k_fp_program(const uint32_t *prog, const fp *in0, const fp *in1, const fp *cst, fp *out0,
                                                   size_t s_in0, size_t s_in1, size_t s_out) {
    fp_program_body<false>(prog, in0, in1, cst, out0, s_in0, s_in1, s_out);
}
__global__ void __launch_bounds__(32) k_fp_program_stream(const uint32_t *prog, const fp *in0, const fp *in1, const fp *cst,
                                                          fp *out0, size_t s_in0, size_t s_in1, size_t s_out) {
    fp_program_body<true>(prog, in0, in1, cst, out0, s_in0, s_in1, s_out);
}

template <bool STREAM>
__device__ __forceinline__ void fp_program2_body(const uint32_t *prog, const fp *in0, const fp *in1, const fp *cst, fp *out0,
                                                 size_t s_in0, size_t s_in1, size_t s_out) {
    extern __shared__ uint4 sm4[];
    fp *slots = (fp *)sm4;
    const int lane = threadIdx.x;
    if (s_in0 != ~(size_t)0) {
        in0 += (size_t)blockIdx.x * s_in0;
        if (in1) in1 += (size_t)blockIdx.x * s_in1;
        out0 += (size_t)blockIdx.x * s_out;
    }
    const uint32_t nr = prog[0], nin = prog[2], nout = prog[3];
    if (lane == 0) fp_set_zero(slots[0]);
    for (uint32_t e = lane; e < nin; e += 32) {
        uint32_t sl = prog[4 + 2 * e], ref = prog[5 + 2 * e], buf = ref >> 24, idx = ref & 0xffffffu;
        const fp *src = buf == 0 ? in0 : (buf == 1 ? in1 : cst);
        slots[sl] = src[idx];
    }
    __syncwarp();
    const uint4 *rp = (const uint4 *)(prog + ((4 + 2 * (nin + nout) + 3) & ~3u)) + lane;
    uint4 wq[4];
#pragma unroll
    for (int k = 0; k < 4; k++) wq[k] = (uint32_t)k < nr ? rp[32 * k] : make_uint4(0, 0, 0, 0);
    for (uint32_t r = 0; r < nr; r += 4) {
#pragma unroll
        for (int k = 0; k < 4; k++) {
            const uint4 w = wq[k];
            wq[k] = r + k + 4 < nr ? rp[32 * (r + k + 4)] : make_uint4(0, 0, 0, 0);
            const uint32_t op = w.x >> 30;
            if (__any_sync(0xffffffffu, op == 1)) {
                if (op == 1) {
                    fp x = slots[w.y & 1023], y = slots[(w.y >> 10) & 1023], t;
                    fp_mul(t, x, y);
                    slots[(w.x >> 20) & 1023] = t;
                }
            } else {
                const uint32_t npos = op == 2 ? (w.x >> 17) & 7 : 0, nneg = op == 2 ? (w.x >> 14) & 7 : 0;
                const uint32_t mp = __reduce_max_sync(0xffffffffu, npos), mn = __reduce_max_sync(0xffffffffu, nneg);
                if (__any_sync(0xffffffffu, op == 2)) {
                    const uint32_t t[7] = {w.y & 0x3fffu, (w.y >> 14) & 0x3fffu, w.z & 0x3fffu, (w.z >> 14) & 0x3fffu,
                                           w.w & 0x3fffu, (w.w >> 14) & 0x3fffu, w.x & 0x3fffu};
                    lin_acc A;
                    lin_clear(A);
#pragma unroll
                    for (int j = 0; j < 7; j++)
                        if ((uint32_t)j < mp) {
                            const uint32_t code = (uint32_t)j < npos ? t[j] : 0u;
                            fp x = slots[code & 1023];
                            lin_add_term(A.P, x, code >> 10);
                        }
#pragma unroll
                    for (int j = 0; j < 7; j++)
                        if ((uint32_t)j < mn) {
                            const uint32_t code = (uint32_t)j < nneg ? t[6 - j] : 0u;
                            fp x = slots[code & 1023];
                            lin_add_term(A.N, x, code >> 10);
                        }
                    if (op == 2) {
                        fp rr;
                        lin_finish(rr, A);
                        slots[(w.x >> 20) & 1023] = rr;
                    }
                }
            }
            if (STREAM && op == 0 && w.x) out0[w.z] = slots[w.y];
            __syncwarp();
        }
    }
    const uint32_t *op = prog + 4 + 2 * nin;
    for (uint32_t e = lane; e < nout; e += 32) out0[op[2 * e + 1] & 0xffffffu] = slots[op[2 * e]];
}
__global__ void __launch_bounds__(32) k_fp_program2(const uint32_t *prog, const fp *in0, const fp *in1, const fp *cst, fp *out0,
                                                    size_t s_in0, size_t s_in1, size_t s_out) {
    fp_program2_body<false>(prog, in0, in1, cst, out0, s_in0, s_in1, s_out);
}
__global__ void __launch_bounds__(32) k_fp_program2_stream(const uint32_t *prog, const fp *in0, const fp *in1, const fp *cst,
                                                           fp *out0, size_t s_in0, size_t s_in1, size_t s_out) {
    fp_program2_body<true>(prog, in0, in1, cst, out0, s_in0, s_in1, s_out);
}
__global__ void __launch_bounds__(32) k_fp_program2_rows(const uint32_t *prog, const fp *in, const fp *cst, fp *out, unsigned m,
                                                         size_t in_stride, size_t out_stride) {
    const size_t j = blockIdx.x / m, g = blockIdx.x % m;
    fp_program2_body<false>(prog, in + (j * in_stride + 8 * g) * 12, nullptr, cst, out + (j * out_stride + g) * 12, ~(size_t)0, 0, 0);
}

__global__ void __launch_bounds__(32) k_fp_program_rows(const uint32_t *prog, const fp *in, const fp *cst, fp *out, unsigned m,
                                                        size_t in_stride, size_t out_stride) {
    const size_t j = blockIdx.x / m, g = blockIdx.x % m;
    fp_program_body<false>(prog, in + (j * in_stride + 8 * g) * 12, nullptr, cst, out + (j * out_stride + g) * 12, ~(size_t)0, 0, 0);
}

__global__ void k_fp_inv_one(const fp *in, fp *out) {
    if (blockIdx.x != 0 || threadIdx.x != 0) return;
    fp a = *in, r;
    fp_inv_vartime(r, a);
    *out = r;
}

__global__ void k_final_out(const fp12 *gt, int count, const int *flags, uint8_t *gt_bytes, int *is_one) {
    const int t = threadIdx.x;
    if (blockIdx.x != 0 || t >= 12) return;
    if (t == 0) {
        int bad = 0;
        if (flags) for (int i = 0; i < count; i++) bad |= flags[i];
        is_one[1] = bad;
        is_one[0] = fp12_is_one(*gt) ? 1 : 0;
    }
    const int i = t >> 2, j = (t >> 1) & 1, k = t & 1;
    const fp2 *c = &gt->c0.c0;
    fp v;
    fp_from_mont(v, k ? c[3 * j + i].c1 : c[3 * j + i].c0);
    uint8_t *out = gt_bytes + 48 * t;
    for (int b = 0; b < 48; b++) out[b] = (uint8_t)(v.l[(47 - b) >> 2] >> (8 * ((47 - b) & 3)));
}

__global__ void k_final(const fp12 *partials, int count, const int *flags, uint8_t *gt_bytes, int *is_one) {
    if (blockIdx.x != 0 || threadIdx.x != 0) return;
    int bad = 0;
    if (flags) for (int i = 0; i < count; i++) bad |= flags[i];
    is_one[1] = bad;
    fp12 acc = partials[0];
    for (int i = 1; i < count; i++) { fp12 b = partials[i]; fp12_mul(acc, acc, b); }
    fp12 gt;
    final_exp(gt, acc);
    *is_one = fp12_is_one(gt) ? 1 : 0;
    fp12_to_bytes(gt_bytes, gt);
}

__global__ void BLS_LB k_hash_to_g2(const uint8_t *msgs, size_t n, size_t msg_len, const uint32_t *offs, const uint8_t *dst,
                                    uint32_t dst_len, g2_aff *out_aff, uint8_t *out_comp) {
    size_t i = (size_t)blockIdx.x * blockDim.x + threadIdx.x;
    if (i >= n) return;
    g2_jac h;
    if (offs) hash_to_g2_jac(h, msgs + offs[i], offs[i + 1] - offs[i], dst, dst_len);
    else hash_to_g2_jac(h, msgs + i * msg_len, msg_len, dst, dst_len);
    g2_aff a;
    pt_to_affine(a, h);
    if (out_aff) out_aff[i] = a;
    if (out_comp) g2_compress(out_comp + 96 * i, a);
}

__global__ void k_verify_pairs(const g1_aff *pks, size_t n, const g2_aff *sig, g2_aff *Q, g1_aff *P, int *flags) {
    size_t i = (size_t)blockIdx.x * blockDim.x + threadIdx.x;
    if (i < n) {
        g1_aff pk = pks[i];
        if (aff_is_inf(pk)) atomicOr(flags, 1);
        P[i] = pk;
    } else if (i == n) {
        Q[n] = *sig;
        g1_aff g;
        g.x = G1_GEN_X;
        fp_neg(g.y, G1_GEN_Y);
        P[n] = g;
    }
}

__global__ void __launch_bounds__(128) k_g1_seg_sum(const g1_aff *pts, const uint32_t *offs, size_t nseg, g1_jac *out) {
    __shared__ g1_jac sm[4][16];
    const int lane = threadIdx.x & 31, warp = threadIdx.x >> 5;
    const size_t sgm = (size_t)blockIdx.x * 4 + warp;
    if (sgm >= nseg) return;
    const uint32_t lo = offs[sgm], hi = offs[sgm + 1];
    g1_jac acc;
    pt_set_inf(acc);
    for (uint32_t i = lo + lane; i < hi; i += 32) {
        g1_aff a = pts[i];
        pt_add_affine(acc, acc, a);
    }
    for (int half = 16; half >= 1; half >>= 1) {
        if (lane >= half && lane < 2 * half) sm[warp][lane - half] = acc;
        __syncwarp();
        if (lane < half) {
            g1_jac b = sm[warp][lane];
            pt_add(acc, acc, b);
        }
        __syncwarp();
    }
    if (lane == 0) out[sgm] = acc;
}
__global__ void BLS_LB k_g1_to_affine_many(const g1_jac *in, size_t n, g1_aff *out) {
    size_t i = (size_t)blockIdx.x * blockDim.x + threadIdx.x;
    if (i >= n) return;
    g1_jac j = in[i];
    g1_aff a;
    pt_to_affine(a, j);
    out[i] = a;
}

__global__ void BLS_LB k_pubkeys_from_bytes(const uint8_t *in, size_t n, int len, int group_check, g1_aff *out,
                                            uint8_t *status, int *nfail) {
    size_t i = (size_t)blockIdx.x * blockDim.x + threadIdx.x;
    if (i >= n) return;
    uint8_t raw[96];
    for (int k = 0; k < len; k++) raw[k] = in[i * len + k];
    g1_aff p;
    int err = pubkey_from_bytes(p, raw, len, group_check != 0);
    out[i] = p;
    status[i] = (uint8_t)err;
    if (err) atomicAdd(nfail, 1);
}
__global__ void BLS_LB k_signatures_from_bytes(const uint8_t *in, size_t n, int len, int group_check, g2_aff *out,
                                               uint8_t *status, int *nfail) {
    size_t i = (size_t)blockIdx.x * blockDim.x + threadIdx.x;
    if (i >= n) return;
    uint8_t raw[192];
    for (int k = 0; k < len; k++) raw[k] = in[i * len + k];
    g2_aff p;
    int err = signature_from_bytes(p, raw, len, group_check != 0);
    out[i] = p;
    status[i] = (uint8_t)err;
    if (err) atomicAdd(nfail, 1);
}
__global__ void k_g1_compress(const g1_aff *in, size_t n, uint8_t *out) {
    size_t i = (size_t)blockIdx.x * blockDim.x + threadIdx.x;
    if (i >= n) return;
    g1_aff a = in[i];
    g1_compress(out + 48 * i, a);
}
__global__ void k_g2_compress(const g2_aff *in, size_t n, uint8_t *out) {
    size_t i = (size_t)blockIdx.x * blockDim.x + threadIdx.x;
    if (i >= n) return;
    g2_aff a = in[i];
    g2_compress(out + 96 * i, a);
}

__global__ void __launch_bounds__(128) k_g1_load(const g1_aff *in, size_t n, g1_jac *out) {
    size_t i = (size_t)blockIdx.x * blockDim.x + threadIdx.x;
    if (i >= n) return;
    g1_aff a = in[i];
    g1_jac j;
    pt_from_affine(j, a);
    out[i] = j;
}
__global__ void __launch_bounds__(128) k_g2_load(const g2_aff *in, size_t n, g2_jac *out) {
    size_t i = (size_t)blockIdx.x * blockDim.x + threadIdx.x;
    if (i >= n) return;
    g2_aff a = in[i];
    g2_jac j;
    pt_from_affine(j, a);
    out[i] = j;
}
__global__ void k_g1_to_affine(const g1_jac *in, g1_aff *out) {
    if (blockIdx.x != 0 || threadIdx.x != 0) return;
    g1_jac j = *in;
    g1_aff a;
    pt_to_affine_vt(a, j);
    *out = a;
}
__global__ void k_g2_to_affine(const g2_jac *in, g2_aff *out) {
    if (blockIdx.x != 0 || threadIdx.x != 0) return;
    g2_jac j = *in;
    g2_aff a;
    pt_to_affine_vt(a, j);
    *out = a;
}

template <class F> __global__ void k_pt_neg(jac_t<F> *p) {
    if (blockIdx.x != 0 || threadIdx.x != 0) return;
    jac_t<F> a = *p, r;
    pt_neg(r, a);
    *p = r;
}

__global__ void k_test_fp(int op, const fp *a, const fp *b, size_t n, fp *out) {
    size_t i = (size_t)blockIdx.x * blockDim.x + threadIdx.x;
    if (i >= n) return;
    fp x = a[i], y, r;
    if (b) y = b[i]; else y = x;
    switch (op) {
        case 0: fp_mul(r, x, y); break;
        case 1: fp_add(r, x, y); break;
        case 2: fp_sub(r, x, y); break;
        case 3: fp_sqr(r, x); break;
        case 6: fp_inv_vartime(r, x); break;
        default: fp_inv(r, x); break;
    }
    out[i] = r;
}

template <int WIDE>
__global__ void __launch_bounds__(256) k_imad_peak(uint32_t *sink, int iters, uint32_t seed) {
    uint32_t a = seed + threadIdx.x, b = seed * 3 + blockIdx.x;
    if (WIDE) {
        uint64_t acc[8];
        for (int k = 0; k < 8; k++) acc[k] = k;
        for (int i = 0; i < iters; i++) {
#pragma unroll
            for (int u = 0; u < 8; u++) {
#pragma unroll
                for (int k = 0; k < 8; k++)
                    asm volatile("mad.wide.u32 %0, %1, %2, %0;" : "+l"(acc[k]) : "r"(a + k), "r"(b + u));
            }
        }
        uint64_t s = 0;
        for (int k = 0; k < 8; k++) s ^= acc[k];
        if (s == 0x1234567) sink[0] = (uint32_t)s;
    } else {
        uint32_t acc[8];
        for (int k = 0; k < 8; k++) acc[k] = k;
        for (int i = 0; i < iters; i++) {
#pragma unroll
            for (int u = 0; u < 8; u++) {
#pragma unroll
                for (int k = 0; k < 8; k++)
                    asm volatile("mad.lo.u32 %0, %1, %2, %0;" : "+r"(acc[k]) : "r"(a + k), "r"(b + u));
            }
        }
        uint32_t s = 0;
        for (int k = 0; k < 8; k++) s ^= acc[k];
        if (s == 0x1234567) sink[0] = s;
    }
}

__global__ void k_fpmul_peak(fp *sink, int iters, uint32_t seed) {
    fp x, y;
#pragma unroll
    for (int i = 0; i < 12; i++) { x.l[i] = seed + i + threadIdx.x; y.l[i] = seed * 7 + i + blockIdx.x; }
    x.l[11] &= 0x0fffffffu;
    y.l[11] &= 0x0fffffffu;
    for (int i = 0; i < iters; i++) {
        fp_mul(x, x, y);
        fp_mul(y, y, x);
    }
    if (x.l[0] == 0x12345 && y.l[3] == 0x54321) sink[0] = x;
}

__global__ void BLS_LB k_make_sets(words8 seed, size_t first, size_t n, sigset *out) {
    size_t i = (size_t)blockIdx.x * blockDim.x + threadIdx.x;
    if (i >= n) return;
    uint64_t idx = first + i;
    uint32_t h[8] = {0x6a09e667u, 0xbb67ae85u, 0x3c6ef372u, 0xa54ff53au, 0x510e527fu, 0x9b05688cu, 0x1f83d9abu, 0x5be0cd19u};
    uint32_t w[16];
    for (int k = 0; k < 8; k++) w[k] = seed.w[k];
    w[8] = __byte_perm((uint32_t)idx, 0, 0x0123);
    w[9] = __byte_perm((uint32_t)(idx >> 32), 0, 0x0123);
    w[10] = 0x80000000u;
    for (int k = 11; k < 15; k++) w[k] = 0;
    w[15] = 320;
    sha256_block(h, w);
    uint32_t sk[8];
    for (int k = 0; k < 8; k++) sk[k] = h[7 - k];
    sk[7] &= 0x03ffffffu;
    sk[0] |= 1;
    uint8_t pre[14] = {'b', 'l', 's', 'g', 'p', 'u'};
    for (int k = 0; k < 8; k++) pre[6 + k] = (uint8_t)(idx >> (8 * k));
    sha256_ctx c;
    sha256_init(c);
    sha256_update(c, pre, 14);
    uint32_t md[8];
    sha256_final(c, md);
    uint8_t msg[32], dst[43];
    for (int k = 0; k < 32; k++) msg[k] = (uint8_t)(md[k >> 2] >> (24 - 8 * (k & 3)));
    for (int k = 0; k < 43; k++) dst[k] = DST_ETH2[k];
    g1_jac g, pkj;
    g.x = G1_GEN_X; g.y = G1_GEN_Y; g.z = FP_ONE;
    pt_mul_words(pkj, g, sk, 8);
    g2_jac hj, sj;
    hash_to_g2_jac(hj, msg, 32, dst, 43);
    pt_mul_words(sj, hj, sk, 8);
    sigset s;
    pt_to_affine(s.pk, pkj);
    pt_to_affine(s.sig, sj);
    for (int k = 0; k < 32; k++) s.msg[k] = msg[k];
    out[i] = s;
}

}
```

nim_blscurve_b200/csrc/msm.cuh:

```cuda
#pragma once
#include <cstdlib>
#include <map>
#include <string>
#include <type_traits>
#include "kernels.cuh"
#include "fpprog.hpp"

namespace bls {

struct msm_state {
    uint8_t *buf = nullptr;
    size_t bytes = 0;
    int sms = 148;
    struct horner_prog { uint32_t *d = nullptr; int nslots = 0, version = 1; };
    std::map<int, horner_prog> horner;
    cudaStream_t tail = nullptr;
    cudaEvent_t ev_group[8] = {}, ev_done = nullptr;
    bool ev_ok = false;
};

static inline void msm_free(msm_state &m) {
    if (m.ev_ok) { for (int i = 0; i < 8; i++) cudaEventDestroy(m.ev_group[i]); cudaEventDestroy(m.ev_done); m.ev_ok = false; }
    if (m.tail) { cudaStreamDestroy(m.tail); m.tail = nullptr; }
    for (auto &kv : m.horner) cudaFree(kv.second.d);
    m.horner.clear();
    if (m.buf) cudaFree(m.buf);
    m.buf = nullptr;
    m.bytes = 0;
}

#ifndef MSM_BIG
#define MSM_BIG 8
#endif

__device__ __forceinline__ int msm_digit(const uint8_t *sc, int sb, int nbits, int c, int w, int &carry) {
    int bit = w * c;
    uint32_t raw = 0;
    for (int k = 0; k < c; k += 8) {
        int b0 = bit + k;
        if (b0 >= nbits) break;
        int byte = b0 >> 3, sh = b0 & 7;
        uint32_t v = sc[byte];
        if (byte + 1 < sb) v |= (uint32_t)sc[byte + 1] << 8;
        v >>= sh;
        int take = c - k < 8 ? c - k : 8;
        if (b0 + take > nbits) take = nbits - b0;
        v &= (1u << take) - 1;
        raw |= v << k;
    }
    int d = (int)raw + carry;
    if (d > (1 << (c - 1))) { d -= (1 << c); carry = 1; } else carry = 0;
    return d;
}

__global__ void __launch_bounds__(256) k_msm_count(const uint8_t *scalars, size_t sstride, size_t n, int sb, int nbits, int c,
                                                   int nwin, uint32_t *counts) {
    size_t i = (size_t)blockIdx.x * blockDim.x + threadIdx.x;
    if (i >= n) return;
    const uint8_t *sc = scalars + i * sstride;
    int carry = 0;
    const uint32_t B = 1u << (c - 1);
    for (int w = 0; w < nwin; w++) {
        int d = msm_digit(sc, sb, nbits, c, w, carry);
        if (d != 0) atomicAdd(&counts[(size_t)w * B + (uint32_t)(d < 0 ? -d : d) - 1], 1u);
    }
}

__device__ __forceinline__ void msm_block_scan2(uint32_t v0, uint32_t v1, uint32_t &x0, uint32_t &x1, uint32_t &t0, uint32_t &t1,
                                                uint32_t (*ws)[32]) {
    const int lane = threadIdx.x & 31, wid = threadIdx.x >> 5;
    x0 = v0; x1 = v1;
    for (int o = 1; o < 32; o <<= 1) {
        uint32_t y0 = __shfl_up_sync(0xffffffffu, x0, o), y1 = __shfl_up_sync(0xffffffffu, x1, o);
        if (lane >= o) { x0 += y0; x1 += y1; }
    }
    if (lane == 31) { ws[0][wid] = x0; ws[1][wid] = x1; }
    __syncthreads();
    if (wid < 2) {
        uint32_t s = ws[wid][lane], t = s;
        for (int o = 1; o < 32; o <<= 1) {
            uint32_t y = __shfl_up_sync(0xffffffffu, t, o);
            if (lane >= o) t += y;
        }
        ws[wid][lane] = t - s;
        if (lane == 31) ws[2 + wid][0] = t;
    }
    __syncthreads();
    x0 += ws[0][wid];
    x1 += ws[1][wid];
    t0 = ws[2][0];
    t1 = ws[3][0];
}

__global__ void __launch_bounds__(1024) k_msm_scan_blocks(const uint32_t *counts, size_t m, uint32_t *bsums) {
    __shared__ uint32_t ws[4][32];
    size_t i = (size_t)blockIdx.x * 1024 + threadIdx.x;
    uint32_t v0 = i < m ? counts[i] : 0, v1 = v0 ? 1u : 0u, x0, x1, t0, t1;
    msm_block_scan2(v0, v1, x0, x1, t0, t1, ws);
    if (threadIdx.x == 0) { bsums[2 * blockIdx.x] = t0; bsums[2 * blockIdx.x + 1] = t1; }
}

__global__ void __launch_bounds__(1024) k_msm_scan_top(uint32_t *bsums, size_t nblk) {
    __shared__ uint32_t ws[4][32];
    __shared__ uint32_t carry_s[2];
    if (threadIdx.x < 2) carry_s[threadIdx.x] = 0;
    __syncthreads();
    for (size_t base = 0; base < nblk; base += 1024) {
        size_t i = base + threadIdx.x;
        uint32_t v0 = i < nblk ? bsums[2 * i] : 0, v1 = i < nblk ? bsums[2 * i + 1] : 0, x0, x1, t0, t1;
        msm_block_scan2(v0, v1, x0, x1, t0, t1, ws);
        uint32_t c0 = carry_s[0], c1 = carry_s[1];
        if (i < nblk) { bsums[2 * i] = c0 + x0 - v0; bsums[2 * i + 1] = c1 + x1 - v1; }
        __syncthreads();
        if (threadIdx.x == 0) { carry_s[0] = c0 + t0; carry_s[1] = c1 + t1; }
        __syncthreads();
    }
}

__global__ void __launch_bounds__(1024) k_msm_scan_apply(const uint32_t *counts, size_t m, const uint32_t *bsums,
                                                         uint32_t *offsets, uint32_t *cursor, uint32_t *rank) {
    __shared__ uint32_t ws[4][32];
    size_t i = (size_t)blockIdx.x * 1024 + threadIdx.x;
    uint32_t v0 = i < m ? counts[i] : 0, v1 = v0 ? 1u : 0u, x0, x1, t0, t1;
    msm_block_scan2(v0, v1, x0, x1, t0, t1, ws);
    uint32_t e0 = bsums[2 * blockIdx.x] + x0 - v0, e1 = bsums[2 * blockIdx.x + 1] + x1 - v1;
    if (i < m) { offsets[i] = e0; cursor[i] = e0; rank[i] = e1; }
    if (i == m - 1) { offsets[m] = e0 + v0; rank[m] = e1 + v1; }
}

__global__ void __launch_bounds__(256) k_msm_scatter(const uint8_t *scalars, size_t sstride, size_t n, int sb, int nbits, int c,
                                                     int nwin, uint32_t *cursor, uint32_t *entries) {
    size_t i = (size_t)blockIdx.x * blockDim.x + threadIdx.x;
    if (i >= n) return;
    const uint8_t *sc = scalars + i * sstride;
    int carry = 0;
    const uint32_t B = 1u << (c - 1);
    for (int w = 0; w < nwin; w++) {
        int d = msm_digit(sc, sb, nbits, c, w, carry);
        if (d != 0) {
            uint32_t pos = atomicAdd(&cursor[(size_t)w * B + (uint32_t)(d < 0 ? -d : d) - 1], 1u);
            entries[pos] = ((uint32_t)i << 1) | (d < 0 ? 1u : 0u);
        }
    }
}

template <class F>
__global__ void BLS_LB k_msm_chunks(const uint8_t *points, size_t pstride, const uint32_t *offsets, const uint32_t *rank,
                                    const uint32_t *entries, size_t b0, size_t b1, uint32_t K, jac_t<F> *partials) {
    const size_t t = (size_t)blockIdx.x * blockDim.x + threadIdx.x;
    const uint32_t S = offsets[b0], E = offsets[b1], rank0 = rank[b0];
    if (t * K >= (size_t)(E - S)) return;
    const uint32_t e0 = S + (uint32_t)(t * K), e1 = E - e0 > K ? e0 + K : E;
    size_t lo = b0, hi = b1;
    while (hi - lo > 1) {
        size_t mid = (lo + hi) >> 1;
        if (offsets[mid] <= e0) lo = mid; else hi = mid;
    }
    size_t b = lo;
    uint32_t bend = offsets[b + 1];
    jac_t<F> acc;
    pt_set_inf(acc);
    for (uint32_t e = e0; e < e1; e++) {
        if (e == bend) {
            partials[t + (rank[b] - rank0)] = acc;
            pt_set_inf(acc);
            do { b++; bend = offsets[b + 1]; } while (bend <= e);
        }
        uint32_t ent = entries[e];
        aff_t<F> p = *(const aff_t<F> *)(points + (size_t)(ent >> 1) * pstride);
        if (ent & 1) f_neg(p.y, p.y);
        pt_add_affine(acc, acc, p);
    }
    partials[t + (rank[b] - rank0)] = acc;
}

__device__ __forceinline__ void msm_bucket_slots(const uint32_t *offsets, const uint32_t *rank, size_t b, uint32_t K,
                                                 uint32_t S, uint32_t rank0, uint32_t &base, uint32_t &np) {
    const uint32_t o0 = offsets[b], o1 = offsets[b + 1];
    if (o1 == o0) { base = 0; np = 0; return; }
    const uint32_t t0 = (o0 - S) / K, t1 = (o1 - 1 - S) / K;
    base = t0 + (rank[b] - rank0);
    np = t1 - t0 + 1;
}

template <class F>
__global__ void BLS_LB k_msm_combine(const jac_t<F> *partials, const uint32_t *offsets, const uint32_t *rank, size_t b0,
                                     size_t b1, uint32_t K, jac_t<F> *buckets, uint32_t *biglist, uint32_t *bigcount) {
    size_t b = b0 + (size_t)blockIdx.x * blockDim.x + threadIdx.x;
    if (b >= b1) return;
    uint32_t base, np;
    msm_bucket_slots(offsets, rank, b, K, offsets[b0], rank[b0], base, np);
    if (np > MSM_BIG) {
        biglist[b0 + atomicAdd(bigcount, 1u)] = (uint32_t)b;
        return;
    }
    jac_t<F> acc;
    pt_set_inf(acc);
    if (np) acc = partials[base];
    for (uint32_t t = 1; t < np; t++) {
        jac_t<F> x = partials[base + t];
        pt_add(acc, acc, x);
    }
    buckets[b] = acc;
}

template <class F>
__global__ void BLS_LB k_msm_combine_big(const jac_t<F> *partials, const uint32_t *offsets, const uint32_t *rank, size_t b0,
                                         uint32_t K, const uint32_t *biglist, const uint32_t *bigcount, jac_t<F> *buckets) {
    __shared__ jac_t<F> wsum[4];
    const int lane = threadIdx.x & 31, wid = threadIdx.x >> 5;
    const uint32_t nbig = *bigcount;
    for (uint32_t i = blockIdx.x; i < nbig; i += gridDim.x) {
        const uint32_t b = biglist[b0 + i];
        uint32_t base, np;
        msm_bucket_slots(offsets, rank, b, K, offsets[b0], rank[b0], base, np);
        jac_t<F> acc;
        pt_set_inf(acc);
        for (uint32_t t = threadIdx.x; t < np; t += blockDim.x) {
            jac_t<F> x = partials[base + t];
            pt_add(acc, acc, x);
        }
        for (int o = 16; o >= 1; o >>= 1) {
            jac_t<F> other;
            uint32_t *dst = (uint32_t *)&other;
            const uint32_t *src = (const uint32_t *)&acc;
            for (int k = 0; k < (int)(sizeof(jac_t<F>) / 4); k++) dst[k] = __shfl_down_sync(0xffffffffu, src[k], o);
            pt_add(acc, acc, other);
        }
        if (lane == 0) wsum[wid] = acc;
        __syncthreads();
        if (threadIdx.x == 0) {
            for (int w = 1; w < 4; w++) { jac_t<F> x = wsum[w]; pt_add(acc, acc, x); }
            buckets[b] = acc;
        }
        __syncthreads();
    }
}

template <class F>
__global__ void BLS_LB k_msm_segment(const jac_t<F> *buckets, int c, int nwin, uint32_t L, jac_t<F> *segs) {
    const uint32_t B = 1u << (c - 1);
    const uint32_t nseg = B / L;
    size_t t = (size_t)blockIdx.x * blockDim.x + threadIdx.x;
    if (t >= (size_t)nwin * nseg) return;
    uint32_t w = (uint32_t)(t / nseg), j = (uint32_t)(t % nseg);
    const jac_t<F> *bk = buckets + (size_t)w * B + (size_t)j * L;
    jac_t<F> running, acc;
    pt_set_inf(running);
    pt_set_inf(acc);
    for (int b = (int)L - 1; b >= 0; b--) {
        jac_t<F> x = bk[b];
        pt_add(running, running, x);
        pt_add(acc, acc, running);
    }
    uint32_t k = j * L;
    if (k) {
        jac_t<F> m;
        pt_mul_words(m, running, &k, 1);
        pt_add(acc, acc, m);
    }
    segs[t] = acc;
}

template <class F>
__global__ void BLS_LB k_tree_rows(jac_t<F> *S, int rows, size_t stride, size_t m, size_t half) {
    size_t t = (size_t)blockIdx.x * blockDim.x + threadIdx.x;
    if (t >= (size_t)rows * half) return;
    size_t r = t / half, i = t % half;
    if (i + half >= m) return;
    jac_t<F> a = S[r * stride + i], b = S[r * stride + i + half];
    pt_add(a, a, b);
    S[r * stride + i] = a;
}

template <class F>
__global__ void k_msm_horner(const jac_t<F> *W, size_t stride, int nwin, int c, int first, int last, jac_t<F> *carry,
                             jac_t<F> *out_jac, aff_t<F> *out_aff) {
    if (blockIdx.x != 0 || threadIdx.x != 0) return;
    jac_t<F> acc;
    int w = nwin - 1;
    if (first) { acc = W[(size_t)w * stride]; w--; } else acc = *carry;
    for (; w >= 0; w--) {
        for (int k = 0; k < c; k++) pt_dbl(acc, acc);
        jac_t<F> x = W[(size_t)w * stride];
        pt_add(acc, acc, x);
    }
    if (!last) { *carry = acc; return; }
    if (out_jac) *out_jac = acc;
    if (out_aff) {
        aff_t<F> a;
        pt_to_affine_vt(a, acc);
        *out_aff = a;
    }
}

__global__ void k_msm_horner_prep(const g1_jac *W, size_t stride, int nwin, fp *hom) {
    const int w = blockIdx.x * blockDim.x + threadIdx.x;
    if (w >= nwin) return;
    g1_jac p = W[(size_t)w * stride];
    fp x, y, z;
    if (pt_is_inf(p)) {
        fp_set_zero(x); y = FP_ONE; fp_set_zero(z);
    } else {
        fp z2;
        fp_mul_ni(x, p.x, p.z);
        y = p.y;
        fp_sqr_ni(z2, p.z);
        fp_mul_ni(z, z2, p.z);
    }
    hom[3 * w] = x; hom[3 * w + 1] = y; hom[3 * w + 2] = z;
}
__global__ void k_msm_horner_finish(const fp *hom, g1_jac *out_jac, g1_aff *out_aff) {
    if (blockIdx.x != 0 || threadIdx.x != 0) return;
    fp X = hom[0], Y = hom[1], Z = hom[2];
    if (out_jac) {
        g1_jac j;
        if (fp_is_zero(Z)) pt_set_inf(j);
        else { fp z2; fp_mul_ni(j.x, X, Z); fp_sqr_ni(z2, Z); fp_mul_ni(j.y, Y, z2); j.z = Z; }
        *out_jac = j;
    }
    if (out_aff) {
        g1_aff a;
        fp zi;
        fp_inv_vartime(zi, Z);
        fp_mul_ni(a.x, X, zi);
        fp_mul_ni(a.y, Y, zi);
        *out_aff = a;
    }
}

__global__ void k_msm_horner_prep_g2(const g2_jac *W, size_t stride, int nwin, fp *hom) {
    const int w = blockIdx.x * blockDim.x + threadIdx.x;
    if (w >= nwin) return;
    g2_jac p = W[(size_t)w * stride];
    g2_jac_to_hom(hom + 6 * w, p);
}
__global__ void k_msm_horner_finish_g2(const fp *hom, g2_jac *out_jac, g2_aff *out_aff) {
    if (blockIdx.x != 0 || threadIdx.x != 0) return;
    fp2 X, Y, Z;
    X.c0 = hom[0]; X.c1 = hom[1]; Y.c0 = hom[2]; Y.c1 = hom[3]; Z.c0 = hom[4]; Z.c1 = hom[5];
    if (out_jac) {
        g2_jac j;
        if (fp2_is_zero(Z)) pt_set_inf(j);
        else { fp2 z2; fp2_mul(j.x, X, Z); fp2_sqr(z2, Z); fp2_mul(j.y, Y, z2); j.z = Z; }
        *out_jac = j;
    }
    if (out_aff) {
        g2_aff a;
        fp2 zi;
        fp2_inv_vartime(zi, Z);
        fp2_mul(a.x, X, zi);
        fp2_mul(a.y, Y, zi);
        *out_aff = a;
    }
}

__global__ void BLS_LB k_msm_make_inputs(uint64_t seed, size_t n, g1_aff *points, uint8_t *scalars) {
    size_t i = (size_t)blockIdx.x * blockDim.x + threadIdx.x;
    if (i >= n) return;
    uint64_t s = seed ^ (0xFACADEull + i * 0x100000001b3ull);
    uint64_t v[6];
    for (int k = 0; k < 6; k++) {
        s += 0x9e3779b97f4a7c15ull;
        uint64_t z = s;
        z = (z ^ (z >> 30)) * 0xbf58476d1ce4e5b9ull;
        z = (z ^ (z >> 27)) * 0x94d049bb133111ebull;
        v[k] = z ^ (z >> 31);
    }
    uint32_t kw[3] = {(uint32_t)v[0], (uint32_t)(v[0] >> 32), (uint32_t)v[1]};
    g1_jac g, r;
    g.x = G1_GEN_X; g.y = G1_GEN_Y; g.z = FP_ONE;
    pt_mul_words(r, g, kw, 3);
    g1_aff a;
    pt_to_affine(a, r);
    points[i] = a;
    for (int w = 0; w < 4; w++)
        for (int b = 0; b < 8; b++) scalars[32 * i + 8 * w + b] = (uint8_t)(v[2 + w] >> (8 * b));
    scalars[32 * i + 31] &= 0x7f;
}

static inline void msm_shape(size_t n, int nbits, int &c, int &nwin) {
    int lg = 0;
    while ((n >> (lg + 1)) != 0) lg++;
    static const int c_env = getenv("BLSGPU_MSM_C") ? atoi(getenv("BLSGPU_MSM_C")) : 0;
    int best_c = 0;
    double best = 0.0;
    const int hi = lg - 2 > 16 ? 16 : lg - 2, lo = lg - 8 < 2 ? 2 : lg - 8;
    for (int cc = hi; cc >= lo; cc--) {
        const int nw = (nbits + 1 + cc - 1) / cc, top = nbits + 1 - (nw - 1) * cc;
        if (nw > 1 && top < (cc < 6 ? cc : 6)) continue;
        const double cost = (double)nw * (11.0 * (double)n + 32.0 * (double)((size_t)1 << (cc - 1)));
        if (!best_c || cost < best) { best_c = cc; best = cost; }
    }
    if (!best_c) best_c = lg - 4 < 2 ? 2 : (lg - 4 > 16 ? 16 : lg - 4);
    c = c_env > 0 ? c_env : best_c;
    nwin = (nbits + 1 + c - 1) / c;
}

template <class F>
static inline int msm_run(msm_state &st, const uint8_t *d_points, size_t pstride, const uint8_t *d_scalars, size_t sstride,
                          size_t n, int nbits, cudaStream_t s, jac_t<F> *d_out_jac, aff_t<F> *d_out_aff, int *launches,
                          std::string &err) {
    typedef jac_t<F> J;
    if (n >= ((size_t)1 << 31)) { err = "msm: too many points"; return -2; }
    const int sb = (nbits + 7) / 8;
    int c, nwin;
    msm_shape(n, nbits, c, nwin);
    const size_t B = (size_t)1 << (c - 1);
    const size_t nb = (size_t)nwin * B;
    const size_t emax = n * (size_t)nwin;
    const size_t wave = (size_t)st.sms * BLS_LB_BLOCKS * 128;
    size_t L = B / 512;
    if (L < 4) L = 4;
    if (L > 32) L = 32;
    static const int l_env = getenv("BLSGPU_MSM_L") ? atoi(getenv("BLSGPU_MSM_L")) : 0;
    if (l_env > 0) L = (size_t)l_env;
    if (L > B) L = B;
    const size_t nseg = B / L;
    static const int g_env = getenv("BLSGPU_MSM_GROUPS") ? atoi(getenv("BLSGPU_MSM_GROUPS")) : 0;
    int G = g_env > 0 ? g_env : 1;
    if (G > 8) G = 8;
    if (G > nwin) G = nwin;
    int gw0[9];
    gw0[0] = nwin;
    for (int g = 0; g < G; g++) gw0[g + 1] = nwin - (int)(((size_t)nwin * (g + 1)) / G);
    uint32_t Kg[8];
    size_t preg[9];
    preg[0] = 0;
    for (int g = 0; g < G; g++) {
        const size_t wg = (size_t)(gw0[g] - gw0[g + 1]), eg = n * wg;
        size_t waves = eg / (wave * 32);
        if (waves < 1) waves = 1;
        size_t Kz = (eg + waves * wave - 1) / (waves * wave);
        if (Kz < 8) Kz = 8;
        static const int k_env = getenv("BLSGPU_MSM_K") ? atoi(getenv("BLSGPU_MSM_K")) : 0;
        if (k_env > 0) Kz = (size_t)k_env;
        Kg[g] = (uint32_t)Kz;
        preg[g + 1] = preg[g] + (eg + Kz - 1) / Kz + 1 + wg * B + 1;
    }
    const size_t pmax = preg[G];
    const size_t nsb = (nb + 1023) / 1024;
    auto al = [](size_t x) { return (x + 255) & ~(size_t)255; };
    size_t o_counts = 0;
    size_t o_offsets = o_counts + al(nb * 4);
    size_t o_cursor = o_offsets + al((nb + 1) * 4);
    size_t o_rank = o_cursor + al(nb * 4);
    size_t o_bsums = o_rank + al((nb + 1) * 4);
    size_t o_big = o_bsums + al(nsb * 8);
    size_t o_bigcount = o_big + al(nb * 4);
    size_t o_carry = o_bigcount + 256;
    size_t o_hom = o_carry + al(sizeof(J));
    size_t o_entries = o_hom + al((size_t)(6 * nwin + 6) * 48);
    size_t o_partials = o_entries + al(emax * 4);
    size_t o_buckets = o_partials + al(pmax * sizeof(J));
    size_t o_segs = o_buckets + al(nb * sizeof(J));
    size_t total = o_segs + al((size_t)nwin * nseg * sizeof(J));
    cudaError_t e;
#define MCK(call) if ((e = (call)) != cudaSuccess) { err = std::string(#call ": ") + cudaGetErrorString(e); return -1; }
    if (st.bytes < total) {
        if (st.buf) { MCK(cudaStreamSynchronize(s)); if (st.tail) MCK(cudaStreamSynchronize(st.tail)); cudaFree(st.buf); }
        st.buf = nullptr;
        st.bytes = 0;
        MCK(cudaMalloc((void **)&st.buf, total));
        st.bytes = total;
    }
    if (G > 1 && !st.tail) {
        int lo_pri = 0, hi_pri = 0;
        MCK(cudaDeviceGetStreamPriorityRange(&lo_pri, &hi_pri));
        MCK(cudaStreamCreateWithPriority(&st.tail, cudaStreamNonBlocking, hi_pri));
        for (int i = 0; i < 8; i++) MCK(cudaEventCreateWithFlags(&st.ev_group[i], cudaEventDisableTiming));
        MCK(cudaEventCreateWithFlags(&st.ev_done, cudaEventDisableTiming));
        st.ev_ok = true;
    }
    uint32_t *counts = (uint32_t *)(st.buf + o_counts), *offsets = (uint32_t *)(st.buf + o_offsets);
    uint32_t *cursor = (uint32_t *)(st.buf + o_cursor), *rank = (uint32_t *)(st.buf + o_rank);
    uint32_t *bsums = (uint32_t *)(st.buf + o_bsums);
    uint32_t *biglist = (uint32_t *)(st.buf + o_big), *bigcount = (uint32_t *)(st.buf + o_bigcount);
    uint32_t *entries = (uint32_t *)(st.buf + o_entries);
    J *partials = (J *)(st.buf + o_partials), *buckets = (J *)(st.buf + o_buckets), *segs = (J *)(st.buf + o_segs);
    J *carry = (J *)(st.buf + o_carry);
    MCK(cudaMemsetAsync(counts, 0, nb * 4, s));
    MCK(cudaMemsetAsync(bigcount, 0, 4 * 8, s));
    int nl = 0;
    k_msm_count<<<(unsigned)((n + 255) / 256), 256, 0, s>>>(d_scalars, sstride, n, sb, nbits, c, nwin, counts);
    k_msm_scan_blocks<<<(unsigned)nsb, 1024, 0, s>>>(counts, nb, bsums);
    k_msm_scan_top<<<1, 1024, 0, s>>>(bsums, nsb);
    k_msm_scan_apply<<<(unsigned)nsb, 1024, 0, s>>>(counts, nb, bsums, offsets, cursor, rank);
    k_msm_scatter<<<(unsigned)((n + 255) / 256), 256, 0, s>>>(d_scalars, sstride, n, sb, nbits, c, nwin, cursor, entries);
    nl += 5;
    for (int g = 0; g < G; g++) {
        const int w0 = gw0[g + 1], wg = gw0[g] - gw0[g + 1];
        const size_t b0 = (size_t)w0 * B, b1 = b0 + (size_t)wg * B;
        const uint32_t K = Kg[g];
        const size_t gchunks = (n * (size_t)wg + K - 1) / K + 1;
        J *pg = partials + preg[g];
        k_msm_chunks<F><<<(unsigned)((gchunks + 127) / 128), 128, 0, s>>>(d_points, pstride, offsets, rank, entries, b0, b1, K, pg);
        cudaStream_t ts = s;
        if (G > 1) {
            MCK(cudaEventRecord(st.ev_group[g], s));
            MCK(cudaStreamWaitEvent(st.tail, st.ev_group[g], 0));
            ts = st.tail;
        }
        k_msm_combine<F><<<(unsigned)(((size_t)wg * B + 127) / 128), 128, 0, ts>>>(pg, offsets, rank, b0, b1, K, buckets, biglist, bigcount + g);
        k_msm_combine_big<F><<<128, 128, 0, ts>>>(pg, offsets, rank, b0, K, biglist, bigcount + g, buckets);
        size_t nt = (size_t)wg * nseg;
        J *sg = segs + (size_t)w0 * nseg;
        k_msm_segment<F><<<(unsigned)((nt + 127) / 128), 128, 0, ts>>>(buckets + b0, c, wg, (uint32_t)L, sg);
        nl += 4;
        for (size_t m = nseg; m > 1;) {
            size_t half = (m + 1) / 2;
            k_tree_rows<F><<<(unsigned)(((size_t)wg * half + 127) / 128), 128, 0, ts>>>(sg, wg, nseg, m, half);
            nl++;
            m = half;
        }
        bool programmed = false;
        {
            static const bool prog_env = !(getenv("BLSGPU_MSM_HORNER_PROG") && atoi(getenv("BLSGPU_MSM_HORNER_PROG")) == 0);
            constexpr bool is_g1 = std::is_same<F, fp>::value;
            constexpr int per = is_g1 ? 3 : 6;
            if (G == 1 && nwin <= 128 && prog_env) {
                msm_state::horner_prog hp;
                const int key = (nwin * 64 + c) * 2 + (is_g1 ? 0 : 1);
                auto it = st.horner.find(key);
                if (it != st.horner.end()) hp = it->second;
                else {
                    fpprog::Program P = is_g1 ? fpprog::build_msm_horner_g1(nwin, c) : fpprog::build_msm_horner_g2(nwin, c);
                    if (P.ok && (size_t)P.nslots * sizeof(fp) <= 48 * 1024) {
                        MCK(cudaMalloc((void **)&hp.d, P.words.size() * 4));
                        MCK(cudaMemcpyAsync(hp.d, P.words.data(), P.words.size() * 4, cudaMemcpyHostToDevice, s));
                        MCK(cudaStreamSynchronize(s));
                        hp.nslots = P.nslots;
                        hp.version = P.version;
                    }
                    st.horner[key] = hp;
                }
                if (hp.d) {
                    fp *hom = (fp *)(st.buf + o_hom);
                    if constexpr (is_g1) k_msm_horner_prep<<<1, 128, 0, ts>>>(sg, nseg, nwin, hom);
                    else k_msm_horner_prep_g2<<<1, 128, 0, ts>>>(sg, nseg, nwin, hom);
                    if (hp.version == 2)
                        k_fp_program2<<<1, 32, (size_t)hp.nslots * sizeof(fp), ts>>>(hp.d, hom, nullptr, nullptr, hom + per * nwin, 0, 0, 0);
                    else
                        k_fp_program<<<1, 32, (size_t)hp.nslots * sizeof(fp), ts>>>(hp.d, hom, nullptr, nullptr, hom + per * nwin, 0, 0, 0);
                    if constexpr (is_g1) k_msm_horner_finish<<<1, 32, 0, ts>>>(hom + per * nwin, d_out_jac, d_out_aff);
                    else k_msm_horner_finish_g2<<<1, 32, 0, ts>>>(hom + per * nwin, d_out_jac, d_out_aff);
                    nl += 3;
                    programmed = true;
                }
            }
        }
        if (!programmed) {
            k_msm_horner<F><<<1, 32, 0, ts>>>(sg, nseg, wg, c, g == 0, g == G - 1, carry, d_out_jac, d_out_aff);
            nl++;
        }
    }
    if (G > 1) {
        MCK(cudaEventRecord(st.ev_done, st.tail));
        MCK(cudaStreamWaitEvent(s, st.ev_done, 0));
    }
    MCK(cudaGetLastError());
#undef MCK
    if (launches) *launches += nl;
    return 0;
}

}
```

nim_blscurve_b200/csrc/pair_route.cuh:

```cuda
#pragma once
#include "fp2h.cuh"
#include "h2c.cuh"
#include "pairing.cuh"

namespace bls {
#ifdef __CUDACC__

__device__ __forceinline__ void hk(fp2h &r, const fp2 &c) { h_take(r, c); }

__device__ __forceinline__ uint32_t h_sgn0(const fp2h &a) {
    const uint32_t m = h_mask();
    const uint32_t par = fp_parity(a.v), zero = fp_is_zero(a.v) ? 1u : 0u;
    const uint32_t mine = par | (zero << 1);
    const uint32_t other = __shfl_xor_sync(m, mine, 1);
    const uint32_t re = h_odd() ? other : mine, im = h_odd() ? mine : other;
    return (re & 2) ? (im & 1) : (re & 1);
}

struct sswu_mid { fp2h u, tv1, x1n, x1d, d3, gxn, t; };

BLS_NOINLINE void sswu_pre_pair(sswu_mid &s, const fp2h &u) {
    fp2h tv2, d2, t, one, c;
    f_set_one(one);
    s.u = u;
    h_sqr(s.tv1, u);
    hk(c, SSWU_Z);
    h_mul(s.tv1, s.tv1, c);
    h_sqr(tv2, s.tv1);
    f_add(tv2, tv2, s.tv1);
    f_add(s.x1n, tv2, one);
    hk(c, SSWU_B);
    h_mul(s.x1n, s.x1n, c);
    if (f_is_zero(tv2)) {
        hk(s.x1d, SSWU_ZA);
    } else {
        hk(c, SSWU_NEG_A);
        h_mul(s.x1d, tv2, c);
    }
    h_sqr(d2, s.x1d);
    h_mul(s.d3, d2, s.x1d);
    h_sqr(s.gxn, s.x1n);
    hk(c, SSWU_A);
    h_mul(t, d2, c);
    f_add(s.gxn, s.gxn, t);
    h_mul(s.gxn, s.gxn, s.x1n);
    hk(c, SSWU_B);
    h_mul(t, s.d3, c);
    f_add(s.gxn, s.gxn, t);
    h_mul(s.t, s.gxn, s.d3);
}

BLS_NOINLINE void sswu_post_pair(g2h_jac &out, const sswu_mid &s, const fp2h &rs, bool is_sq) {
    fp2h y, xn, c;
    h_mul(y, s.gxn, rs);
    if (is_sq) {
        xn = s.x1n;
    } else {
        hk(c, SSWU_Z);
        h_mul(y, y, c);
        h_mul(y, y, s.tv1);
        h_mul(y, y, s.u);
        h_mul(xn, s.tv1, s.x1n);
    }
    const bool flip = h_sgn0(s.u) != h_sgn0(y);
    h_cneg(y, y, flip);
    h_mul(out.x, xn, s.x1d);
    h_mul(out.y, y, s.d3);
    out.z = s.x1d;
}

BLS_NOINLINE void iso3_pair(g2h_jac &out, const g2h_jac &p) {
    fp2h W, W2, W3, X2, X3, XN, XD, YN, YD, t, X2W, XW2, XW, c;
    h_sqr(W, p.z);
    h_sqr(W2, W);
    h_mul(W3, W2, W);
    h_sqr(X2, p.x);
    h_mul(X3, X2, p.x);
    h_mul(X2W, X2, W);
    h_mul(XW, p.x, W);
    h_mul(XW2, p.x, W2);
    hk(c, ISO3_XNUM[3]); h_mul(XN, X3, c);
    hk(c, ISO3_XNUM[2]); h_mul(t, X2W, c); f_add(XN, XN, t);
    hk(c, ISO3_XNUM[1]); h_mul(t, XW2, c); f_add(XN, XN, t);
    hk(c, ISO3_XNUM[0]); h_mul(t, W3, c);  f_add(XN, XN, t);
    hk(c, ISO3_XDEN[1]); h_mul(XD, XW, c);
    f_add(XD, XD, X2);
    hk(c, ISO3_XDEN[0]); h_mul(t, W2, c);  f_add(XD, XD, t);
    hk(c, ISO3_YNUM[3]); h_mul(YN, X3, c);
    hk(c, ISO3_YNUM[2]); h_mul(t, X2W, c); f_add(YN, YN, t);
    hk(c, ISO3_YNUM[1]); h_mul(t, XW2, c); f_add(YN, YN, t);
    hk(c, ISO3_YNUM[0]); h_mul(t, W3, c);  f_add(YN, YN, t);
    hk(c, ISO3_YDEN[2]); h_mul(YD, X2W, c);
    f_add(YD, YD, X3);
    hk(c, ISO3_YDEN[1]); h_mul(t, XW2, c); f_add(YD, YD, t);
    hk(c, ISO3_YDEN[0]); h_mul(t, W3, c);  f_add(YD, YD, t);
    fp2h XDYD, YD2, XD2;
    h_mul(XDYD, XD, YD);
    h_sqr(YD2, YD);
    h_sqr(XD2, XD);
    h_mul(t, XN, XDYD);
    h_mul(out.x, t, YD);
    h_mul(t, p.y, YN);
    h_mul(t, t, XD2);
    h_mul(t, t, XDYD);
    h_mul(out.y, t, YD);
    h_mul(out.z, p.z, XDYD);
}

__device__ __forceinline__ void psi_pair(g2h_jac &r, const g2h_jac &p) {
    fp2h t, c;
    h_conj(t, p.x); hk(c, PSI_CX); h_mul(r.x, t, c);
    h_conj(t, p.y); hk(c, PSI_CY); h_mul(r.y, t, c);
    h_conj(r.z, p.z);
}
__device__ __forceinline__ void psi2_pair(g2h_jac &r, const g2h_jac &p) {
    h_mul_fp(r.x, p.x, PSI2_CX);
    f_neg(r.y, p.y);
    r.z = p.z;
}
BLS_NOINLINE void mul_by_x_pair(g2h_jac &r, const g2h_jac &p) {
    g2h_jac acc = p;
    const uint64_t z = BLS_Z_ABS;
    for (int i = 62; i >= 0; i--) {
        pt_dbl(acc, acc);
        if ((z >> i) & 1) pt_add(acc, acc, p);
    }
    pt_neg(r, acc);
}
BLS_NOINLINE void clear_cofactor_pair(g2h_jac &out, const g2h_jac &p) {
    g2h_jac t1, t2, t3, n;
    mul_by_x_pair(t1, p);
    psi_pair(t2, p);
    pt_dbl(t3, p);
    psi2_pair(t3, t3);
    pt_neg(n, t2);
    pt_add(t3, t3, n);
    pt_add(t2, t1, t2);
    mul_by_x_pair(t2, t2);
    pt_add(t3, t3, t2);
    pt_neg(n, t1);
    pt_add(t3, t3, n);
    pt_neg(n, p);
    pt_add(out, t3, n);
}

BLS_NOINLINE void hash_map_to_e2_pair(g2h_jac &out, const uint8_t *msg, size_t msg_len, const uint8_t *dst, uint32_t dst_len) {
    const bool odd = h_odd();
    fp2h u0, u1;
    {
        uint32_t xmd[64];
        if (dst) expand_message_xmd_256(xmd, msg, msg_len, dst, dst_len);
        else expand_message_xmd_256_eth2(xmd, msg);
        fp_from_be64(u0.v, xmd + (odd ? 16 : 0));
        fp_from_be64(u1.v, xmd + (odd ? 48 : 32));
    }
    sswu_mid s0, s1;
    sswu_pre_pair(s0, u0);
    sswu_pre_pair(s1, u1);
    fp send, recv;
    fp_select(send, odd, s0.t.v, s1.t.v);
    h_xchg(recv, send);
    fp2 arg, rs;
    fp_select(arg.c0, odd, recv, s0.t.v);
    fp_select(arg.c1, odd, s1.t.v, recv);
    const bool sq_mine = fp2_rsqrt_or_z(rs, arg);
    fp2h r0, r1;
    fp_select(send, odd, rs.c0, rs.c1);
    h_xchg(recv, send);
    fp_select(r0.v, odd, recv, rs.c0);
    fp_select(r1.v, odd, rs.c1, recv);
    const uint32_t m = h_mask();
    const int sq_other = __shfl_xor_sync(m, (int)sq_mine, 1);
    const bool sq0 = odd ? (sq_other != 0) : sq_mine, sq1 = odd ? sq_mine : (sq_other != 0);
    g2h_jac q0, q1;
    sswu_post_pair(q0, s0, r0, sq0);
    sswu_post_pair(q1, s1, r1, sq1);
    fp2h a;
    hk(a, SSWU_A);
    pt_add(q0, q0, q1, &a);
    iso3_pair(out, q0);
}
BLS_NOINLINE void hash_to_g2_pair(g2h_jac &out, const uint8_t *msg, size_t msg_len, const uint8_t *dst, uint32_t dst_len) {
    g2h_jac q;
    hash_map_to_e2_pair(q, msg, msg_len, dst, dst_len);
    clear_cofactor_pair(out, q);
}
__device__ __forceinline__ void jac_to_hom_pair(fp2h &X, fp2h &Y, fp2h &Z, const g2h_jac &p) {
    if (pt_is_inf(p)) {
        f_set_zero(X);
        f_set_one(Y);
        f_set_zero(Z);
    } else {
        fp2h z2;
        h_mul(X, p.x, p.z);
        Y = p.y;
        h_sqr(z2, p.z);
        h_mul(Z, z2, p.z);
    }
}

BLS_NOINLINE void line_dbl_pair(g2h_jac &T, fp2h &l0, fp2h &l1p, fp2h &l2p) {
    fp2h A2, B, Cc, E, F, H, J, t, u;
    h_sqr(B, T.y);
    h_sqr(Cc, T.z);
    h_sqr(J, T.x);
    f_add(t, T.x, T.y);
    h_sqr(A2, t);
    f_sub(A2, A2, J);
    f_sub(A2, A2, B);
    f_add(t, T.y, T.z);
    h_sqr(H, t);
    f_sub(H, H, B);
    f_sub(H, H, Cc);
    h_mul_xi(E, Cc);
    f_dbl(E, E);
    f_dbl(E, E);
    h_mul3(E, E);
    h_mul3(F, E);
    f_sub(l0, B, E);
    h_mul3(l1p, J);
    l2p = H;
    f_sub(t, B, F);
    h_mul(T.x, A2, t);
    f_add(t, B, F);
    h_sqr(t, t);
    f_dbl(u, E);
    h_sqr(u, u);
    h_mul3(u, u);
    f_sub(T.y, t, u);
    h_mul(t, B, H);
    f_dbl(t, t);
    f_dbl(T.z, t);
}
BLS_NOINLINE void line_add_pair(g2h_jac &T, const g2h_aff &Q, fp2h &l0, fp2h &l1p, fp2h &l2p) {
    fp2h th, la, c, d, e, f, g, h, t;
    h_mul(t, Q.y, T.z);
    f_sub(th, T.y, t);
    h_mul(t, Q.x, T.z);
    f_sub(la, T.x, t);
    h_sqr(c, th);
    h_sqr(d, la);
    h_mul(e, la, d);
    h_mul(f, T.z, c);
    h_mul(g, T.x, d);
    f_add(h, e, f);
    f_sub(h, h, g);
    f_sub(h, h, g);
    h_mul(T.x, la, h);
    f_sub(t, g, h);
    h_mul(t, th, t);
    h_mul(g, e, T.y);
    f_sub(T.y, t, g);
    h_mul(T.z, T.z, e);
    h_mul(l0, th, Q.x);
    h_mul(t, la, Q.y);
    f_sub(l0, l0, t);
    l1p = th;
    l2p = la;
}
__device__ __forceinline__ void line_store_pair(uint32_t *dst, size_t stride, int s, const fp2h &l0, const fp2h &l1, const fp2h &l2) {
    uint32_t *d = dst + ((size_t)s * ML_LINE_WORDS + (h_odd() ? 12 : 0)) * stride;
    for (int w = 0; w < 12; w++) {
        d[(size_t)w * stride] = l0.v.l[w];
        d[(size_t)(24 + w) * stride] = l1.v.l[w];
        d[(size_t)(48 + w) * stride] = l2.v.l[w];
    }
}
BLS_NOINLINE void miller_lines_pair(const g2h_aff &Q, const g1_aff &P, bool inf, uint32_t *dst, size_t stride) {
    fp2h l0, l1, l2;
    if (inf) {
        f_set_one(l0);
        f_set_zero(l1);
        f_set_zero(l2);
        for (int s = 0; s < ML_NLINES; s++) line_store_pair(dst, stride, s, l0, l1, l2);
        return;
    }
    g2h_jac T;
    T.x = Q.x;
    T.y = Q.y;
    f_set_one(T.z);
    fp npx, py = P.y;
    fp_neg(npx, P.x);
    int s = 0;
    for (int i = 62; i >= 0; i--) {
        line_dbl_pair(T, l0, l1, l2);
        h_mul_fp(l1, l1, npx);
        h_mul_fp(l2, l2, py);
        line_store_pair(dst, stride, s++, l0, l1, l2);
        if (ml_bit(i)) {
            line_add_pair(T, Q, l0, l1, l2);
            h_mul_fp(l1, l1, npx);
            h_mul_fp(l2, l2, py);
            line_store_pair(dst, stride, s++, l0, l1, l2);
        }
    }
}

#endif
}
```

nim_blscurve_b200/csrc/pairing.cuh:

```cuda
#pragma once
#include "tower.cuh"

namespace bls {

BLS_NOINLINE void line_dbl(g2_jac &T, fp2 &l0, fp2 &l1p, fp2 &l2p) {
    fp2 A, B, C, ZZ, E, D, Fq, t;
    fp2_sqr(A, T.x);
    fp2_sqr(B, T.y);
    fp2_sqr(C, B);
    fp2_sqr(ZZ, T.z);
    fp2_mul3(E, A);
    fp2_mul(l0, E, T.x);
    fp2_sub(l0, l0, B);
    fp2_sub(l0, l0, B);
    fp2_mul(l1p, E, ZZ);
    fp2_add(t, T.x, B);
    fp2_sqr(t, t);
    fp2_sub(t, t, A);
    fp2_sub(t, t, C);
    fp2_dbl(D, t);
    fp2_sqr(Fq, E);
    fp2_mul(t, T.y, T.z);
    fp2_dbl(T.z, t);
    fp2_mul(l2p, T.z, ZZ);
    fp2_sub(Fq, Fq, D);
    fp2_sub(Fq, Fq, D);
    T.x = Fq;
    fp2_sub(t, D, Fq);
    fp2_mul(t, E, t);
    fp2_dbl(C, C);
    fp2_dbl(C, C);
    fp2_dbl(C, C);
    fp2_sub(T.y, t, C);
}

BLS_NOINLINE void line_add(g2_jac &T, const g2_aff &Q, fp2 &l0, fp2 &l1p, fp2 &l2p) {
    fp2 Z1Z1, U2, S2, H, HH, I, J, rr, V, t;
    fp2_sqr(Z1Z1, T.z);
    fp2_mul(U2, Q.x, Z1Z1);
    fp2_mul(t, T.z, Z1Z1);
    fp2_mul(S2, Q.y, t);
    fp2_sub(H, U2, T.x);
    fp2_sub(rr, S2, T.y);
    fp2_dbl(rr, rr);
    fp2_sqr(HH, H);
    fp2_dbl(I, HH);
    fp2_dbl(I, I);
    fp2_mul(J, H, I);
    fp2_mul(V, T.x, I);
    fp2_add(t, T.z, H);
    fp2_sqr(t, t);
    fp2_sub(t, t, Z1Z1);
    fp2_sub(T.z, t, HH);
    fp2_sqr(t, rr);
    fp2_sub(t, t, J);
    fp2_sub(t, t, V);
    fp2_sub(t, t, V);
    T.x = t;
    fp2_sub(t, V, t);
    fp2_mul(t, rr, t);
    fp2_mul(J, T.y, J);
    fp2_dbl(J, J);
    fp2_sub(T.y, t, J);
    fp2_mul(l0, rr, Q.x);
    fp2_mul(t, Q.y, T.z);
    fp2_sub(l0, l0, t);
    l1p = rr;
    l2p = T.z;
}

BLS_NOINLINE void line_dbl_proj(g2_jac &T, fp2 &l0, fp2 &l1p, fp2 &l2p) {
    fp2 A2, B, C, E, F, H, J, t, u;
    fp2_sqr(B, T.y);
    fp2_sqr(C, T.z);
    fp2_sqr(J, T.x);
    fp2_add(t, T.x, T.y);
    fp2_sqr(A2, t);
    fp2_sub(A2, A2, J);
    fp2_sub(A2, A2, B);
    fp2_add(t, T.y, T.z);
    fp2_sqr(H, t);
    fp2_sub(H, H, B);
    fp2_sub(H, H, C);
    fp2_mul_xi(E, C);
    fp2_dbl(E, E);
    fp2_dbl(E, E);
    fp2_mul3(E, E);
    fp2_mul3(F, E);
    fp2_sub(l0, B, E);
    fp2_mul3(l1p, J);
    l2p = H;
    fp2_sub(t, B, F);
    fp2_mul(T.x, A2, t);
    fp2_add(t, B, F);
    fp2_sqr(t, t);
    fp2_dbl(u, E);
    fp2_sqr(u, u);
    fp2_mul3(u, u);
    fp2_sub(T.y, t, u);
    fp2_mul(t, B, H);
    fp2_dbl(t, t);
    fp2_dbl(T.z, t);
}

BLS_NOINLINE void line_add_proj(g2_jac &T, const g2_aff &Q, fp2 &l0, fp2 &l1p, fp2 &l2p) {
    fp2 th, la, c, d, e, f, g, h, t;
    fp2_mul(t, Q.y, T.z);
    fp2_sub(th, T.y, t);
    fp2_mul(t, Q.x, T.z);
    fp2_sub(la, T.x, t);
    fp2_sqr(c, th);
    fp2_sqr(d, la);
    fp2_mul(e, la, d);
    fp2_mul(f, T.z, c);
    fp2_mul(g, T.x, d);
    fp2_add(h, e, f);
    fp2_sub(h, h, g);
    fp2_sub(h, h, g);
    fp2_mul(T.x, la, h);
    fp2_sub(t, g, h);
    fp2_mul(t, th, t);
    fp2_mul(g, e, T.y);
    fp2_sub(T.y, t, g);
    fp2_mul(T.z, T.z, e);
    fp2_mul(l0, th, Q.x);
    fp2_mul(t, la, Q.y);
    fp2_sub(l0, l0, t);
    l1p = th;
    l2p = la;
}

BLS_FN void line_apply(fp12 &f, const fp2 &l0, const fp2 &l1p, const fp2 &l2p, const fp &neg_px, const fp &py) {
    fp2 l1, l2;
    fp2_mul_fp(l1, l1p, neg_px);
    fp2_mul_fp(l2, l2p, py);
    fp12_mul_by_line(f, l0, l1, l2);
}

BLS_NOINLINE void miller_loop_n(fp12 &f, const g2_aff *Q, const g1_aff *P, int n, g2_jac *T, fp *neg_px) {
    fp12_set_one(f);
    int live = 0;
    for (int k = 0; k < n; k++) {
        pt_from_affine(T[k], Q[k]);
        fp_neg(neg_px[k], P[k].x);
        if (aff_is_inf(P[k])) pt_set_inf(T[k]);
        live += !pt_is_inf(T[k]);
    }
    if (live == 0) return;
    const uint64_t z = BLS_Z_ABS;
    fp2 l0, l1p, l2p;
    for (int i = 62; i >= 0; i--) {
        if (i != 62) fp12_sqr(f, f);
        for (int k = 0; k < n; k++) {
            if (pt_is_inf(T[k])) continue;
            line_dbl(T[k], l0, l1p, l2p);
            line_apply(f, l0, l1p, l2p, neg_px[k], P[k].y);
        }
        if ((z >> i) & 1) {
            for (int k = 0; k < n; k++) {
                if (pt_is_inf(T[k])) continue;
                line_add(T[k], Q[k], l0, l1p, l2p);
                line_apply(f, l0, l1p, l2p, neg_px[k], P[k].y);
            }
        }
    }
    fp12_conj(f, f);
}

#define ML_NLINES 68
#define ML_LINE_WORDS 72

BLS_FN int ml_bit(int i) { return (int)((BLS_Z_ABS >> i) & 1); }
BLS_FN int ml_line_index(int i) { return (62 - i) + (i < 62) + (i < 60) + (i < 57) + (i < 48) + (i < 16); }
BLS_HD int ml_seg_hi(int j, int nseg) { return 62 - (63 * j) / nseg; }
BLS_HD int ml_seg_lo(int j, int nseg) { return 62 - (63 * (j + 1)) / nseg + 1; }

BLS_FN void line_store(uint32_t *dst, size_t stride, int s, const fp2 &l0, const fp2 &l1, const fp2 &l2) {
    uint32_t *d = dst + (size_t)s * ML_LINE_WORDS * stride;
    for (int w = 0; w < 12; w++) {
        d[(size_t)w * stride] = l0.c0.l[w];
        d[(size_t)(12 + w) * stride] = l0.c1.l[w];
        d[(size_t)(24 + w) * stride] = l1.c0.l[w];
        d[(size_t)(36 + w) * stride] = l1.c1.l[w];
        d[(size_t)(48 + w) * stride] = l2.c0.l[w];
        d[(size_t)(60 + w) * stride] = l2.c1.l[w];
    }
}

BLS_FN void line_load(fp2 &l0, fp2 &l1, fp2 &l2, const uint32_t *src, size_t stride, int s) {
    const uint32_t *d = src + (size_t)s * ML_LINE_WORDS * stride;
    for (int w = 0; w < 12; w++) {
        l0.c0.l[w] = d[(size_t)w * stride];
        l0.c1.l[w] = d[(size_t)(12 + w) * stride];
        l1.c0.l[w] = d[(size_t)(24 + w) * stride];
        l1.c1.l[w] = d[(size_t)(36 + w) * stride];
        l2.c0.l[w] = d[(size_t)(48 + w) * stride];
        l2.c1.l[w] = d[(size_t)(60 + w) * stride];
    }
}

BLS_NOINLINE void miller_lines(const g2_aff &Q, const g1_aff &P, uint32_t *dst, size_t stride) {
    fp2 l0, l1, l2;
    if (aff_is_inf(Q) | aff_is_inf(P)) {
        f_set_one(l0);
        fp2_set_zero(l1);
        fp2_set_zero(l2);
        for (int s = 0; s < ML_NLINES; s++) line_store(dst, stride, s, l0, l1, l2);
        return;
    }
    g2_jac T;
    pt_from_affine(T, Q);
    fp npx, py = P.y;
    fp_neg(npx, P.x);
    int s = 0;
    for (int i = 62; i >= 0; i--) {
        line_dbl_proj(T, l0, l1, l2);
        fp2_mul_fp(l1, l1, npx);
        fp2_mul_fp(l2, l2, py);
        line_store(dst, stride, s++, l0, l1, l2);
        if (ml_bit(i)) {
            line_add_proj(T, Q, l0, l1, l2);
            fp2_mul_fp(l1, l1, npx);
            fp2_mul_fp(l2, l2, py);
            line_store(dst, stride, s++, l0, l1, l2);
        }
    }
}

BLS_NOINLINE void miller_accumulate(fp12 &f, const uint32_t *lines, size_t stride, size_t np, size_t g, size_t ngroups,
                                    int G, int i_hi, int i_lo) {
    fp2 l0, l1, l2;
    bool first = true;
    fp12_set_one(f);
    for (int i = i_hi; i >= i_lo; i--) {
        if (!first) fp12_sqr(f, f);
        const int s = ml_line_index(i), nl = 1 + ml_bit(i);
        for (int a = 0; a < nl; a++)
            for (int k = 0; k < G; k++) {
                size_t p = g + (size_t)k * ngroups;
                if (p >= np) break;
                line_load(l0, l1, l2, lines + p, stride, s + a);
                if (first) {
                    f.c0.c0 = l0;
                    f.c0.c1 = l1;
                    f.c1.c1 = l2;
                    first = false;
                } else {
                    fp12_mul_by_line(f, l0, l1, l2);
                }
            }
    }
}

BLS_NOINLINE void miller_combine(fp12 &F, const fp12 *seg, int nseg) {
    fp12 acc = seg[0];
    for (int j = 1; j < nseg; j++) {
        int len = ml_seg_hi(j, nseg) - ml_seg_lo(j, nseg) + 1;
        for (int t = 0; t < len; t++) fp12_sqr(acc, acc);
        fp12 b = seg[j];
        fp12_mul(acc, acc, b);
    }
    fp12_conj(F, acc);
}

BLS_NOINLINE void cyc_exp_z(fp12 &r, const fp12 &a) {
    fp12 acc = a;
    const uint64_t z = BLS_Z_ABS;
    for (int i = 62; i >= 0; i--) {
        fp12_cyc_sqr(acc, acc);
        if ((z >> i) & 1) fp12_mul(acc, acc, a);
    }
    fp12_conj(r, acc);
}

BLS_NOINLINE void final_exp(fp12 &r, const fp12 &f) {
    fp12 t, a, b, c, d;
    fp12_conj(a, f);
    fp12_inv(b, f);
    fp12_mul(t, a, b);
    fp12_frob(a, t, 2);
    fp12_mul(t, a, t);
    cyc_exp_z(a, t);
    fp12_conj(b, t);
    fp12_mul(a, a, b);
    cyc_exp_z(b, a);
    fp12_conj(c, a);
    fp12_mul(a, b, c);
    cyc_exp_z(b, a);
    fp12_frob(c, a, 1);
    fp12_mul(b, b, c);
    cyc_exp_z(c, b);
    cyc_exp_z(c, c);
    fp12_frob(d, b, 2);
    fp12_mul(c, c, d);
    fp12_conj(d, b);
    fp12_mul(c, c, d);
    fp12_cyc_sqr(d, t);
    fp12_mul(d, d, t);
    fp12_mul(r, c, d);
}

}
```

nim_blscurve_b200/csrc/tower.cuh:

```cuda
#pragma once
#include "ec.cuh"

namespace bls {

struct fp6 { fp2 c0, c1, c2; };
struct fp12 { fp6 c0, c1; };

BLS_FN void fp6_add(fp6 &r, const fp6 &a, const fp6 &b) { fp2_add(r.c0, a.c0, b.c0); fp2_add(r.c1, a.c1, b.c1); fp2_add(r.c2, a.c2, b.c2); }
BLS_FN void fp6_sub(fp6 &r, const fp6 &a, const fp6 &b) { fp2_sub(r.c0, a.c0, b.c0); fp2_sub(r.c1, a.c1, b.c1); fp2_sub(r.c2, a.c2, b.c2); }
BLS_FN void fp6_neg(fp6 &r, const fp6 &a) { fp2_neg(r.c0, a.c0); fp2_neg(r.c1, a.c1); fp2_neg(r.c2, a.c2); }
BLS_FN void fp6_dbl(fp6 &r, const fp6 &a) { fp2_dbl(r.c0, a.c0); fp2_dbl(r.c1, a.c1); fp2_dbl(r.c2, a.c2); }
BLS_FN void fp6_mul_v(fp6 &r, const fp6 &a) {
    fp2 t;
    fp2_mul_xi(t, a.c2);
    r.c2 = a.c1;
    r.c1 = a.c0;
    r.c0 = t;
}

BLS_NOINLINE void fp6_mul(fp6 &r, const fp6 &a, const fp6 &b) {
    fp2 t0, t1, t2, s, u, c0, c1, c2;
    fp2_mul(t0, a.c0, b.c0);
    fp2_mul(t1, a.c1, b.c1);
    fp2_mul(t2, a.c2, b.c2);
    fp2_add(s, a.c1, a.c2);
    fp2_add(u, b.c1, b.c2);
    fp2_mul(c0, s, u);
    fp2_sub(c0, c0, t1);
    fp2_sub(c0, c0, t2);
    fp2_mul_xi(c0, c0);
    fp2_add(c0, c0, t0);
    fp2_add(s, a.c0, a.c1);
    fp2_add(u, b.c0, b.c1);
    fp2_mul(c1, s, u);
    fp2_sub(c1, c1, t0);
    fp2_sub(c1, c1, t1);
    fp2_mul_xi(s, t2);
    fp2_add(c1, c1, s);
    fp2_add(s, a.c0, a.c2);
    fp2_add(u, b.c0, b.c2);
    fp2_mul(c2, s, u);
    fp2_sub(c2, c2, t0);
    fp2_sub(c2, c2, t2);
    fp2_add(c2, c2, t1);
    r.c0 = c0;
    r.c1 = c1;
    r.c2 = c2;
}

BLS_NOINLINE void fp6_mul_by_01(fp6 &r, const fp6 &a, const fp2 &c0, const fp2 &c1) {
    fp2 t0, t1, t2, s, u, r0, r1, r2;
    fp2_mul(t0, a.c0, c0);
    fp2_mul(t1, a.c1, c1);
    fp2_mul(t2, a.c2, c1);
    fp2_mul_xi(t2, t2);
    fp2_add(r0, t0, t2);
    fp2_add(s, a.c0, a.c1);
    fp2_add(u, c0, c1);
    fp2_mul(r1, s, u);
    fp2_sub(r1, r1, t0);
    fp2_sub(r1, r1, t1);
    fp2_mul(r2, a.c2, c0);
    fp2_add(r2, r2, t1);
    r.c0 = r0;
    r.c1 = r1;
    r.c2 = r2;
}

BLS_NOINLINE void fp6_mul_by_1(fp6 &r, const fp6 &a, const fp2 &c1) {
    fp2 r0, r1, r2;
    fp2_mul(r0, a.c2, c1);
    fp2_mul_xi(r0, r0);
    fp2_mul(r1, a.c0, c1);
    fp2_mul(r2, a.c1, c1);
    r.c0 = r0;
    r.c1 = r1;
    r.c2 = r2;
}

BLS_NOINLINE void fp6_inv(fp6 &r, const fp6 &a) {
    fp2 c0, c1, c2, t, s;
    fp2_sqr(c0, a.c0);
    fp2_mul(t, a.c1, a.c2);
    fp2_mul_xi(t, t);
    fp2_sub(c0, c0, t);
    fp2_sqr(c1, a.c2);
    fp2_mul_xi(c1, c1);
    fp2_mul(t, a.c0, a.c1);
    fp2_sub(c1, c1, t);
    fp2_sqr(c2, a.c1);
    fp2_mul(t, a.c0, a.c2);
    fp2_sub(c2, c2, t);
    fp2_mul(t, a.c2, c1);
    fp2_mul(s, a.c1, c2);
    fp2_add(t, t, s);
    fp2_mul_xi(t, t);
    fp2_mul(s, a.c0, c0);
    fp2_add(t, t, s);
    fp2_inv(t, t);
    fp2_mul(r.c0, c0, t);
    fp2_mul(r.c1, c1, t);
    fp2_mul(r.c2, c2, t);
}

BLS_FN void fp12_set_one(fp12 &r) {
    fp2 *c = &r.c0.c0;
    for (int i = 0; i < 6; i++) fp2_set_zero(c[i]);
    r.c0.c0.c0 = FP_ONE;
}

BLS_FN bool fp12_is_one(const fp12 &a) {
    const fp2 *c = &a.c0.c0;
    bool ok = fp_eq(c[0].c0, FP_ONE) & fp_is_zero(c[0].c1);
    for (int i = 1; i < 6; i++) ok &= fp2_is_zero(c[i]);
    return ok;
}

BLS_FN void fp12_conj(fp12 &r, const fp12 &a) { r.c0 = a.c0; fp6_neg(r.c1, a.c1); }

BLS_NOINLINE void fp12_mul(fp12 &r, const fp12 &a, const fp12 &b) {
    fp6 t0, t1, s, u;
    fp6_mul(t0, a.c0, b.c0);
    fp6_mul(t1, a.c1, b.c1);
    fp6_add(s, a.c0, a.c1);
    fp6_add(u, b.c0, b.c1);
    fp6_mul(s, s, u);
    fp6_sub(s, s, t0);
    fp6_sub(r.c1, s, t1);
    fp6_mul_v(t1, t1);
    fp6_add(r.c0, t0, t1);
}

BLS_NOINLINE void fp12_sqr(fp12 &r, const fp12 &a) {
    fp6 t, s, u;
    fp6_mul(t, a.c0, a.c1);
    fp6_add(s, a.c0, a.c1);
    fp6_mul_v(u, a.c1);
    fp6_add(u, u, a.c0);
    fp6_mul(s, s, u);
    fp6_sub(s, s, t);
    fp6_mul_v(u, t);
    fp6_sub(r.c0, s, u);
    fp6_dbl(r.c1, t);
}

BLS_NOINLINE void fp12_mul_by_line(fp12 &f, const fp2 &l0, const fp2 &l1, const fp2 &l2) {
    fp6 t0, t1, t2, s;
    fp2 l12;
    fp6_mul_by_01(t0, f.c0, l0, l1);
    fp6_mul_by_1(t1, f.c1, l2);
    fp6_add(s, f.c0, f.c1);
    fp2_add(l12, l1, l2);
    fp6_mul_by_01(t2, s, l0, l12);
    fp6_sub(t2, t2, t0);
    fp6_sub(f.c1, t2, t1);
    fp6_mul_v(t1, t1);
    fp6_add(f.c0, t0, t1);
}

BLS_NOINLINE void fp12_inv(fp12 &r, const fp12 &a) {
    fp6 t0, t1;
    fp6_mul(t0, a.c0, a.c0);
    fp6_mul(t1, a.c1, a.c1);
    fp6_mul_v(t1, t1);
    fp6_sub(t0, t0, t1);
    fp6_inv(t0, t0);
    fp6_mul(r.c0, a.c0, t0);
    fp6_mul(t1, a.c1, t0);
    fp6_neg(r.c1, t1);
}

BLS_NOINLINE void fp12_frob(fp12 &r, const fp12 &a, int n) {
    const fp2 *g = n == 1 ? FROB1 : (n == 2 ? FROB2 : FROB3);
    const fp2 *src = &a.c0.c0;
    fp2 *dst = &r.c0.c0;
    for (int j = 0; j < 2; j++)
        for (int i = 0; i < 3; i++) {
            fp2 c = src[3 * j + i];
            if (n & 1) fp2_conj(c, c);
            int k = 2 * i + j;
            if (k) fp2_mul(c, c, g[k - 1]);
            dst[3 * j + i] = c;
        }
}

BLS_FN void fp4_sqr(fp2 &t0, fp2 &t1, const fp2 &a, const fp2 &b) {
    fp2 a2, b2, s;
    fp2_sqr(a2, a);
    fp2_sqr(b2, b);
    fp2_add(s, a, b);
    fp2_sqr(s, s);
    fp2_sub(s, s, a2);
    fp2_sub(t1, s, b2);
    fp2_mul_xi(b2, b2);
    fp2_add(t0, a2, b2);
}

BLS_NOINLINE void fp12_cyc_sqr(fp12 &r, const fp12 &a) {
    fp2 z0 = a.c0.c0, z4 = a.c0.c1, z3 = a.c0.c2, z2 = a.c1.c0, z1 = a.c1.c1, z5 = a.c1.c2;
    fp2 t0, t1, t2, t3, t;
    fp4_sqr(t0, t1, z0, z1);
    fp2_sub(t, t0, z0); fp2_dbl(t, t); fp2_add(z0, t, t0);
    fp2_add(t, t1, z1); fp2_dbl(t, t); fp2_add(z1, t, t1);
    fp4_sqr(t0, t1, z2, z3);
    fp4_sqr(t2, t3, z4, z5);
    fp2_sub(t, t0, z4); fp2_dbl(t, t); fp2_add(z4, t, t0);
    fp2_add(t, t1, z5); fp2_dbl(t, t); fp2_add(z5, t, t1);
    fp2_mul_xi(t3, t3);
    fp2_add(t, t3, z2); fp2_dbl(t, t); fp2_add(z2, t, t3);
    fp2_sub(t, t2, z3); fp2_dbl(t, t); fp2_add(z3, t, t2);
    r.c0.c0 = z0; r.c0.c1 = z4; r.c0.c2 = z3;
    r.c1.c0 = z2; r.c1.c1 = z1; r.c1.c2 = z5;
}

BLS_FN void fp12_to_bytes(uint8_t *out, const fp12 &a) {
    const fp2 *c = &a.c0.c0;
    for (int i = 0; i < 3; i++)
        for (int j = 0; j < 2; j++) {
            const fp2 &e = c[3 * j + i];
            for (int k = 0; k < 2; k++) {
                fp t;
                fp_from_mont(t, k ? e.c1 : e.c0);
                for (int b = 0; b < 48; b++) *out++ = (uint8_t)(t.l[(47 - b) >> 2] >> (8 * ((47 - b) & 3)));
            }
        }
}

}
```

Measured before the change: 2.382 million.

## Switch Fp arithmetic to redundant [0,2p) representation with canonicalization at boundaries

Removes the final conditional subtraction from Montgomery mul and sqr, and makes add and sub work modulo 2p, so field elements live in a redundant range below 2p. Values are canonicalized before equality and zero tests, on stores to global memory, on line coefficients and in the team accumulator paths. It also adds a multi-square loop to fp_sqr_ni to cut per-square call overhead in pow chains. The aim is fewer reduction instructions per field op across the Miller loop and the point arithmetic. The risk is correctness if any mul input bound assumption (inputs below 2p, needing 4p^2 < R*p) is violated, plus extra canonicalization cost at stores.

After: 2.421 million, median of 6. 1.02x the previous value.

```diff
diff --git a/nim_blscurve_b200/csrc/acc_team.cuh b/nim_blscurve_b200/csrc/acc_team.cuh
--- a/nim_blscurve_b200/csrc/acc_team.cuh
+++ b/nim_blscurve_b200/csrc/acc_team.cuh
@@ -87,7 +87,7 @@
         fp x;
         load_fp_regs(x.l, ap[t]);
         fp x2;
-        fp_dbl(x2, x);
+        fp_dbl_canon(x2, x);
         const bool d = (dbl_mask >> t) & 1, z = (zero_mask >> t) & 1;
 #pragma unroll
         for (int i = 0; i < 12; i++) a[t][i] = z ? 0u : (d ? x2.l[i] : x.l[i]);
@@ -100,9 +100,9 @@
 
 __device__ __forceinline__ void team_store_coeff(acc_team_sm &T, int k, const fp &c0, const fp &c1) {
     fp s, d, dd;
-    fp_add(s, c0, c1);
-    fp_sub(d, c0, c1);
-    fp_dbl(dd, c0);
+    fp_add_canon(s, c0, c1);
+    fp_sub_canon(d, c0, c1);
+    fp_dbl_canon(dd, c0);
     T.f[k][FV_C0] = c0;
     T.f[k][FV_C1] = c1;
     T.f[k][FV_S] = s;
@@ -125,9 +125,9 @@
     team_dot3(D0, &T.l[0], &T.l[2], &T.l[4], x0[0], x0[1], x0[2]);
     team_dot3(D1, &T.l[1], &T.l[3], &T.l[5], x1[0], x1[1], x1[2]);
     team_dot3(D2, &T.l[6], &T.l[7], &T.l[8], sx[0], sx[1], sx[2]);
-    fp_sub(c0, D0, D1);
-    fp_sub(c1, D2, D0);
-    fp_sub(c1, c1, D1);
+    fp_sub_canon(c0, D0, D1);
+    fp_sub_canon(c1, D2, D0);
+    fp_sub_canon(c1, c1, D1);
     __syncwarp(mask);
     team_store_coeff(T, k, c0, c1);
     __syncwarp(mask);
@@ -148,9 +148,9 @@
     team_dot4(D0, a0, b0, DBL[k], ZERO[k]);
     team_dot4(D1, a1, b1, DBL[k], ZERO[k]);
     team_dot4(D2, as, bs, DBL[k], ZERO[k]);
-    fp_sub(c0, D0, D1);
-    fp_sub(c1, D2, D0);
-    fp_sub(c1, c1, D1);
+    fp_sub_canon(c0, D0, D1);
+    fp_sub_canon(c1, D2, D0);
+    fp_sub_canon(c1, c1, D1);
     __syncwarp(mask);
     team_store_coeff(T, k, c0, c1);
     __syncwarp(mask);
diff --git a/nim_blscurve_b200/csrc/ec.cuh b/nim_blscurve_b200/csrc/ec.cuh
--- a/nim_blscurve_b200/csrc/ec.cuh
+++ b/nim_blscurve_b200/csrc/ec.cuh
@@ -45,6 +45,16 @@
     if (aff_is_inf(a)) f_set_zero(r.z); else f_set_one(r.z);
 }
 template <class F> BLS_FN void pt_neg(jac_t<F> &r, const jac_t<F> &a) { r.x = a.x; f_neg(r.y, a.y); r.z = a.z; }
+template <class F> BLS_FN jac_t<F> canon(const jac_t<F> &a) {
+    jac_t<F> r;
+    r.x = canon(a.x); r.y = canon(a.y); r.z = canon(a.z);
+    return r;
+}
+template <class F> BLS_FN aff_t<F> canon(const aff_t<F> &a) {
+    aff_t<F> r;
+    r.x = canon(a.x); r.y = canon(a.y);
+    return r;
+}
 
 template <class F> BLS_NOINLINE void pt_dbl(jac_t<F> &r, const jac_t<F> &p) {
     F A, B, C, D, E, Fq, t;
diff --git a/nim_blscurve_b200/csrc/fp.cuh b/nim_blscurve_b200/csrc/fp.cuh
--- a/nim_blscurve_b200/csrc/fp.cuh
+++ b/nim_blscurve_b200/csrc/fp.cuh
@@ -27,20 +27,6 @@
 BLS_FN void fp_set_zero(fp &r) {
 #pragma unroll
     for (int i = 0; i < 12; i++) r.l[i] = 0;
-}
-
-BLS_FN bool fp_is_zero(const fp &a) {
-    uint32_t t = 0;
-#pragma unroll
-    for (int i = 0; i < 12; i++) t |= a.l[i];
-    return t == 0;
-}
-
-BLS_FN bool fp_eq(const fp &a, const fp &b) {
-    uint32_t t = 0;
-#pragma unroll
-    for (int i = 0; i < 12; i++) t |= a.l[i] ^ b.l[i];
-    return t == 0;
 }
 
 BLS_FN void fp_select(fp &r, bool c, const fp &a, const fp &b) {
@@ -103,6 +89,25 @@
     for (int i = 0; i < 12; i++) r[i] = bw ? t[i] : u[i];
 }
 
+BLS_FN uint32_t sub_2p12(uint32_t *acc) {
+    uint32_t bw;
+    asm("sub.cc.u32 %0,%0,0xffff5556;\n\tsubc.cc.u32 %1,%1,0x73fdffff;\n\tsubc.cc.u32 %2,%2,0x62a7ffff;\n\t"
+        "subc.cc.u32 %3,%3,0x3d57fffd;\n\tsubc.cc.u32 %4,%4,0xed61ec48;\n\tsubc.cc.u32 %5,%5,0xce61a541;\n\t"
+        "subc.cc.u32 %6,%6,0xe70a257e;\n\tsubc.cc.u32 %7,%7,0xc8ee9709;\n\tsubc.cc.u32 %8,%8,0x869759ae;\n\t"
+        "subc.cc.u32 %9,%9,0x96374f6c;\n\tsubc.cc.u32 %10,%10,0x72ffcd34;\n\tsubc.cc.u32 %11,%11,0x340223d4;\n\t"
+        "subc.u32 %12,0,0;"
+        : BLS_R12(acc), "=r"(bw));
+    return bw;
+}
+
+BLS_FN void add_2p12(uint32_t *acc) {
+    asm("add.cc.u32 %0,%0,0xffff5556;\n\taddc.cc.u32 %1,%1,0x73fdffff;\n\taddc.cc.u32 %2,%2,0x62a7ffff;\n\t"
+        "addc.cc.u32 %3,%3,0x3d57fffd;\n\taddc.cc.u32 %4,%4,0xed61ec48;\n\taddc.cc.u32 %5,%5,0xce61a541;\n\t"
+        "addc.cc.u32 %6,%6,0xe70a257e;\n\taddc.cc.u32 %7,%7,0xc8ee9709;\n\taddc.cc.u32 %8,%8,0x869759ae;\n\t"
+        "addc.cc.u32 %9,%9,0x96374f6c;\n\taddc.cc.u32 %10,%10,0x72ffcd34;\n\taddc.u32 %11,%11,0x340223d4;"
+        : BLS_R12(acc));
+}
+
 #define BLS_LANE_C(lo, hi, a, b) \
     "madc.lo.cc.u32 " lo "," a "," b "," lo ";\n\tmadc.hi.cc.u32 " hi "," a "," b "," hi ";\n\t"
 #define BLS_LANE_0(lo, hi, a, b) \
@@ -138,7 +143,43 @@
 }
 #endif
 
-BLS_FN void fp_add(fp &r, const fp &a, const fp &b) {
+BLS_FN void fp_canon(fp &r, const fp &a) {
+#ifdef __CUDA_ARCH__
+    reduce_once12(r.l, a.l);
+#else
+    uint32_t u[12];
+    int64_t bw = 0;
+    for (int i = 0; i < 12; i++) { bw += (int64_t)a.l[i] - P32(i); u[i] = (uint32_t)bw; bw >>= 32; }
+    for (int i = 0; i < 12; i++) r.l[i] = bw ? a.l[i] : u[i];
+#endif
+}
+
+BLS_FN fp canon(const fp &a) {
+    fp r;
+    fp_canon(r, a);
+    return r;
+}
+
+BLS_FN bool fp_is_zero(const fp &a) {
+    fp c;
+    fp_canon(c, a);
+    uint32_t t = 0;
+#pragma unroll
+    for (int i = 0; i < 12; i++) t |= c.l[i];
+    return t == 0;
+}
+
+BLS_FN bool fp_eq(const fp &a, const fp &b) {
+    fp x, y;
+    fp_canon(x, a);
+    fp_canon(y, b);
+    uint32_t t = 0;
+#pragma unroll
+    for (int i = 0; i < 12; i++) t |= x.l[i] ^ y.l[i];
+    return t == 0;
+}
+
+BLS_FN void fp_add_canon(fp &r, const fp &a, const fp &b) {
 #ifdef __CUDA_ARCH__
     uint32_t t[12];
 #pragma unroll
@@ -155,7 +196,7 @@
 #endif
 }
 
-BLS_FN void fp_sub(fp &r, const fp &a, const fp &b) {
+BLS_FN void fp_sub_canon(fp &r, const fp &a, const fp &b) {
 #ifdef __CUDA_ARCH__
     uint32_t t[12], u[12];
 #pragma unroll
@@ -172,6 +213,53 @@
     for (int i = 0; i < 12; i++) { bw += (int64_t)a.l[i] - b.l[i]; t[i] = (uint32_t)bw; bw >>= 32; }
     uint64_t c = 0;
     for (int i = 0; i < 12; i++) { c += (uint64_t)t[i] + (bw ? P32(i) : 0u); r.l[i] = (uint32_t)c; c >>= 32; }
+#endif
+}
+
+BLS_FN void fp_dbl_canon(fp &r, const fp &a) { fp_add_canon(r, a, a); }
+
+BLS_FN void fp_add(fp &r, const fp &a, const fp &b) {
+#ifdef __CUDA_ARCH__
+    uint32_t t[12], u[12];
+#pragma unroll
+    for (int i = 0; i < 12; i++) t[i] = a.l[i];
+    add12(t, b.l);
+#pragma unroll
+    for (int i = 0; i < 12; i++) u[i] = t[i];
+    uint32_t bw = sub_2p12(u);
+#pragma unroll
+    for (int i = 0; i < 12; i++) r.l[i] = bw ? t[i] : u[i];
+#else
+    fp_add_canon(r, a, b);
+#endif
+}
+
+BLS_FN void fp_add_nr(fp &r, const fp &a, const fp &b) {
+#ifdef __CUDA_ARCH__
+    uint32_t t[12];
+#pragma unroll
+    for (int i = 0; i < 12; i++) t[i] = a.l[i];
+    add12(t, b.l);
+#pragma unroll
+    for (int i = 0; i < 12; i++) r.l[i] = t[i];
+#else
+    fp_add_canon(r, a, b);
+#endif
+}
+
+BLS_FN void fp_sub(fp &r, const fp &a, const fp &b) {
+#ifdef __CUDA_ARCH__
+    uint32_t t[12], u[12];
+#pragma unroll
+    for (int i = 0; i < 12; i++) t[i] = a.l[i];
+    uint32_t bw = sub12(t, b.l);
+#pragma unroll
+    for (int i = 0; i < 12; i++) u[i] = t[i];
+    add_2p12(u);
+#pragma unroll
+    for (int i = 0; i < 12; i++) r.l[i] = bw ? u[i] : t[i];
+#else
+    fp_sub_canon(r, a, b);
 #endif
 }
 
@@ -219,7 +307,8 @@
         mad6_top(E, P32(0), P32(2), P32(4), P32(6), P32(8), P32(10), m);
     }
     add12(O, E + 1);
-    reduce_once12(r.l, O);
+#pragma unroll
+    for (int i = 0; i < 12; i++) r.l[i] = O[i];
 #else
 #ifdef BLS_COUNT_MULS
     extern unsigned long long g_fp_mul_count;
@@ -256,19 +345,18 @@
 
 BLS_FN void fp_sqr(fp &r, const fp &a) {
 #if defined(__CUDA_ARCH__) && !defined(BLS_NO_FP_SQR)
-    uint32_t t[12];
-    fp_sqr_ptx(t, a.l);
-    reduce_once12(r.l, t);
+    fp_sqr_ptx(r.l, a.l);
 #else
     fp_mul(r, a, a);
 #endif
 }
 
 BLS_FN void fp_from_mont(fp &r, const fp &a) {
-    fp one;
+    fp one, t;
     fp_set_zero(one);
     one.l[0] = 1;
-    fp_mul(r, a, one);
+    fp_mul(t, a, one);
+    fp_canon(r, t);
 }
 
 BLS_FN uint32_t fp_parity(const fp &a) {
diff --git a/nim_blscurve_b200/csrc/fp2.cuh b/nim_blscurve_b200/csrc/fp2.cuh
--- a/nim_blscurve_b200/csrc/fp2.cuh
+++ b/nim_blscurve_b200/csrc/fp2.cuh
@@ -10,10 +10,15 @@
     fp_mul(t, x, y);
     r = t;
 }
-BLS_NOINLINE void fp_sqr_ni(fp &r, const fp &a) {
-    fp x = a, t;
-    fp_sqr(t, x);
-    r = t;
+BLS_NOINLINE void fp_sqr_ni(fp &r, const fp &a, int n = 1) {
+    fp x = a;
+#pragma unroll 1
+    for (int s = 0; s < n; s++) {
+        fp t;
+        fp_sqr(t, x);
+        x = t;
+    }
+    r = x;
 }
 
 #if defined(__CUDACC__) && !defined(BLS_SMALL_CODE)
@@ -36,6 +41,8 @@
 #endif
 
 BLS_FN void fp2_set_zero(fp2 &r) { fp_set_zero(r.c0); fp_set_zero(r.c1); }
+BLS_FN void fp2_canon(fp2 &r, const fp2 &a) { fp_canon(r.c0, a.c0); fp_canon(r.c1, a.c1); }
+BLS_FN fp2 canon(const fp2 &a) { fp2 r; fp2_canon(r, a); return r; }
 BLS_FN bool fp2_is_zero(const fp2 &a) { return fp_is_zero(a.c0) & fp_is_zero(a.c1); }
 BLS_FN bool fp2_eq(const fp2 &a, const fp2 &b) { return fp_eq(a.c0, b.c0) & fp_eq(a.c1, b.c1); }
 BLS_FN void fp2_select(fp2 &r, bool c, const fp2 &a, const fp2 &b) {
@@ -117,7 +124,8 @@
     }
     add12(O, E + 1);
     add12(O, T + 12);
-    reduce_once12(r, O);
+#pragma unroll
+    for (int i = 0; i < 12; i++) r[i] = O[i];
 }
 BLS_FN uint32_t sub12_b(uint32_t *acc, const uint32_t *b, uint32_t bw_in) {
     uint32_t bw;
@@ -139,7 +147,7 @@
 
 BLS_NOINLINE void fp2_mul_r3(fp2 &r, const fp2 &a, const fp2 &b) {
     fp s0, s1, t0, t1, t2;
-    FP_ADD(s0, a.c0, a.c1);
+    fp_add_nr(s0, a.c0, a.c1);
     FP_ADD(s1, b.c0, b.c1);
     FP_MUL(t2, s0, s1);
     FP_MUL(t0, a.c0, b.c0);
@@ -155,8 +163,11 @@
 #define BLS_FP2_LAZY 0
 #endif
 
-BLS_NOINLINE void fp2_mul(fp2 &r, const fp2 &a, const fp2 &b) {
+BLS_NOINLINE void fp2_mul(fp2 &r, const fp2 &a_in, const fp2 &b_in) {
 #if defined(__CUDA_ARCH__) && BLS_FP2_LAZY
+    fp2 a, b;
+    fp2_canon(a, a_in);
+    fp2_canon(b, b_in);
     uint32_t T2[24], T0[24];
     {
         uint32_t s0[12], s1[12];
@@ -187,13 +198,13 @@
     r.c1 = im;
     return;
 #else
-    fp2_mul_r3(r, a, b);
+    fp2_mul_r3(r, a_in, b_in);
 #endif
 }
 
 BLS_NOINLINE void fp2_sqr(fp2 &r, const fp2 &a) {
     fp s, d, t, u;
-    FP_ADD(s, a.c0, a.c1);
+    fp_add_nr(s, a.c0, a.c1);
     FP_SUB(d, a.c0, a.c1);
     FP_MUL(u, s, d);
     FP_MUL(t, a.c0, a.c1);
diff --git a/nim_blscurve_b200/csrc/fp2h.cuh b/nim_blscurve_b200/csrc/fp2h.cuh
--- a/nim_blscurve_b200/csrc/fp2h.cuh
+++ b/nim_blscurve_b200/csrc/fp2h.cuh
@@ -58,7 +58,8 @@
         mad6_top(E, P32(0), P32(2), P32(4), P32(6), P32(8), P32(10), m);
     }
     add12(O, E + 1);
-    reduce_once12(r.l, O);
+#pragma unroll
+    for (int i = 0; i < 12; i++) r.l[i] = O[i];
 #endif
 }
 
@@ -78,7 +79,7 @@
     h_xchg(ap, ao);
     const bool odd = h_odd();
     fp_select(t, odd, ao, ap);
-    fp_add(x, ao, t);
+    fp_add_nr(x, ao, t);
     fp_sub(d, ao, ap);
     fp_select(y, odd, ap, d);
     fp_mul(t, x, y);
@@ -114,6 +115,7 @@
 __device__ __forceinline__ bool f_is_zero(const fp2h &a) { return h_both(fp_is_zero(a.v)); }
 __device__ __forceinline__ bool f_eq(const fp2h &a, const fp2h &b) { return h_both(fp_eq(a.v, b.v)); }
 __device__ __forceinline__ void f_set_zero(fp2h &r) { fp_set_zero(r.v); }
+__device__ __forceinline__ fp2h canon(const fp2h &a) { fp2h r; fp_canon(r.v, a.v); return r; }
 __device__ __forceinline__ void f_set_one(fp2h &r) { if (h_odd()) fp_set_zero(r.v); else r.v = FP_ONE; }
 __device__ __forceinline__ void f_inv(fp2h &r, const fp2h &a) { h_inv(r, a); }
 __device__ __forceinline__ void f_inv_vt(fp2h &r, const fp2h &a) { h_inv(r, a); }
diff --git a/nim_blscurve_b200/csrc/fpx.cuh b/nim_blscurve_b200/csrc/fpx.cuh
--- a/nim_blscurve_b200/csrc/fpx.cuh
+++ b/nim_blscurve_b200/csrc/fpx.cuh
@@ -12,7 +12,7 @@
     acc = tbl[first];
     for (int k = 0; k < len; k++) {
         int ns = ops[k][0], idx = ops[k][1];
-        for (int s = 0; s < ns; s++) fp_sqr_ni(acc, acc);
+        if (ns) fp_sqr_ni(acc, acc, ns);
         if (idx != 255) fp_mul_ni(acc, acc, tbl[idx]);
     }
     r = acc;
@@ -20,7 +20,9 @@
 
 BLS_FN void fp_inv(fp &r, const fp &a) { fp_pow_chain(r, a, CHAIN_PM2_FIRST, CHAIN_PM2_OPS, CHAIN_PM2_LEN); }
 
-BLS_NOINLINE void fp_inv_vartime(fp &r, const fp &a) {
+BLS_NOINLINE void fp_inv_vartime(fp &r, const fp &a_in) {
+    fp a;
+    fp_canon(a, a_in);
     if (fp_is_zero(a)) { fp_set_zero(r); return; }
     uint32_t u[12], v[12], x1[12], x2[12];
 #pragma unroll
diff --git a/nim_blscurve_b200/csrc/kernels.cuh b/nim_blscurve_b200/csrc/kernels.cuh
--- a/nim_blscurve_b200/csrc/kernels.cuh
+++ b/nim_blscurve_b200/csrc/kernels.cuh
@@ -139,7 +139,7 @@
     }
     g2_jac h;
     hash_to_g2_jac_eth2(h, msg);
-    H[i] = h;
+    H[i] = canon(h);
 }
 
 __global__ void BLS_LB k_hash_sets_pair(const sigset *sets, size_t n, g2_jac *H) {
@@ -164,7 +164,7 @@
     iso3_g2(q, q);
     g2_jac h;
     g2_clear_cofactor(h, q);
-    H[i] = h;
+    H[i] = canon(h);
 }
 
 __global__ void BLS_LB k_hash_sets_lanes2(const sigset *sets, size_t n, g2_jac *H) {
@@ -184,9 +184,9 @@
     g2h_jac h;
     hash_to_g2_pair(h, msg, 32, nullptr, 0);
     fp *out = (fp *)&H[i] + (h_odd() ? 1 : 0);
-    out[0] = h.x.v;
-    out[2] = h.y.v;
-    out[4] = h.z.v;
+    out[0] = canon(h.x.v);
+    out[2] = canon(h.y.v);
+    out[4] = canon(h.z.v);
 }
 __global__ void __launch_bounds__(128, BLS_LB_BLOCKS) k_miller_lines_lanes2(const g2_aff *Q, const g1_aff *P, size_t np,
                                                                             uint32_t *lines, size_t stride) {
@@ -213,7 +213,8 @@
         fp2_sqr(z2, p.z);
         fp2_mul(z, z2, p.z);
     }
-    hom[0] = x.c0; hom[1] = x.c1; hom[2] = y.c0; hom[3] = y.c1; hom[4] = z.c0; hom[5] = z.c1;
+    hom[0] = canon(x.c0); hom[1] = canon(x.c1); hom[2] = canon(y.c0); hom[3] = canon(y.c1); hom[4] = canon(z.c0);
+    hom[5] = canon(z.c1);
 }
 __global__ void BLS_LB k_hash_map_pair(const sigset *sets, size_t n, fp *hom) {
     const size_t t = (size_t)blockIdx.x * blockDim.x + threadIdx.x;
@@ -253,9 +254,9 @@
     fp2h X, Y, Z;
     jac_to_hom_pair(X, Y, Z, q);
     fp *out = hom + 6 * i + (h_odd() ? 1 : 0);
-    out[0] = X.v;
-    out[2] = Y.v;
-    out[4] = Z.v;
+    out[0] = canon(X.v);
+    out[2] = canon(Y.v);
+    out[4] = canon(Z.v);
 }
 __global__ void BLS_LB k_hash_map_pair_msgs(const uint8_t *msgs, const uint32_t *offs, const uint8_t *dst, uint32_t dst_len,
                                             size_t n, fp *hom) {
@@ -287,7 +288,7 @@
     fp2_inv_vartime(zi, Z);
     fp2_mul(a.x, X, zi);
     fp2_mul(a.y, Y, zi);
-    out[blockIdx.x] = a;
+    out[blockIdx.x] = canon(a);
 }
 __global__ void k_g2_hom_to_jac(const fp *hom, size_t n, g2_jac *out) {
     const size_t i = (size_t)blockIdx.x * blockDim.x + threadIdx.x;
@@ -298,7 +299,7 @@
     g2_jac j;
     if (fp2_is_zero(Z)) pt_set_inf(j);
     else { fp2 z2; fp2_mul(j.x, X, Z); fp2_sqr(z2, Z); fp2_mul(j.y, Y, z2); j.z = Z; }
-    out[i] = j;
+    out[i] = canon(j);
 }
 __global__ void k_g2_mul_prep(const sigset *sets, const uint64_t *r, size_t n, fp *hom, fp *bits) {
     const size_t t = (size_t)blockIdx.x * blockDim.x + threadIdx.x;
@@ -328,7 +329,7 @@
     if (aff_is_inf(pk)) atomicOr(flags, 1);
     g1_jac j;
     pt_mul_u64_w4(j, pk, r[i]);
-    Pj[i] = j;
+    Pj[i] = canon(j);
 }
 
 #define AFF_B 8
@@ -412,8 +413,8 @@
         g1_aff a;
         pt_to_affine_zinv(q, h, zhinv);
         pt_to_affine_zinv(a, p, zpinv);
-        Q[i] = q;
-        P[i] = a;
+        Q[i] = canon(q);
+        P[i] = canon(a);
     }
 }
 
@@ -423,7 +424,7 @@
     g2_aff sig = sets[i].sig;
     g2_jac j;
     pt_mul_u64(j, sig, r[i]);
-    S[i] = j;
+    S[i] = canon(j);
 }
 
 __global__ void BLS_LB k_g2_tree(g2_jac *S, size_t n, size_t half) {
@@ -431,7 +432,7 @@
     if (i >= half || i + half >= n) return;
     g2_jac a = S[i], b = S[i + half];
     pt_add(a, a, b);
-    S[i] = a;
+    S[i] = canon(a);
 }
 
 __global__ void BLS_LB k_g1_tree(g1_jac *S, size_t n, size_t half) {
@@ -439,7 +440,7 @@
     if (i >= half || i + half >= n) return;
     g1_jac a = S[i], b = S[i + half];
     pt_add(a, a, b);
-    S[i] = a;
+    S[i] = canon(a);
 }
 
 __global__ void BLS_LB k_fp12_tree(fp12 *F, size_t n, size_t half) {
@@ -447,7 +448,7 @@
     if (i >= half || i + half >= n) return;
     fp12 a = F[i], b = F[i + half];
     fp12_mul(a, a, b);
-    F[i] = a;
+    F[i] = canon(a);
 }
 
 
@@ -456,11 +457,11 @@
     g2_jac s = *S;
     g2_aff sa;
     pt_to_affine_vt(sa, s);
-    Q[n] = sa;
+    Q[n] = canon(sa);
     g1_aff g;
     g.x = G1_GEN_X;
     fp_neg(g.y, G1_GEN_Y);
-    P[n] = g;
+    P[n] = canon(g);
 }
 
 #ifndef BLS_LINES_BLOCKS
@@ -525,7 +526,7 @@
     if (g < ngroups) miller_accumulate(f, lines, stride, np, g, ngroups, G, ml_seg_hi(j, nseg), ml_seg_lo(j, nseg));
     else fp12_set_one(f);
     block_fp12_product(f, sm);
-    if (threadIdx.x == 0) Fseg[(size_t)j * row_stride + col_off + blockIdx.x] = f;
+    if (threadIdx.x == 0) Fseg[(size_t)j * row_stride + col_off + blockIdx.x] = canon(f);
 }
 
 #ifndef BLS_ACCT_BLOCKS
@@ -562,7 +563,7 @@
                 }
                 T.l[k] = v;
                 __syncwarp(mask);
-                if (k < 3) { fp sum; fp_add(sum, T.l[2 * k], T.l[2 * k + 1]); T.l[6 + k] = sum; }
+                if (k < 3) { fp sum; fp_add_canon(sum, T.l[2 * k], T.l[2 * k + 1]); T.l[6 + k] = sum; }
                 __syncwarp(mask);
                 if (first) {
                     fp c0, c1;
@@ -592,7 +593,7 @@
     fp12 f;
     if (c < ncols) f = in[(size_t)blockIdx.y * in_stride + c]; else fp12_set_one(f);
     block_fp12_product(f, sm);
-    if (threadIdx.x == 0) out[(size_t)blockIdx.y * out_stride + blockIdx.x] = f;
+    if (threadIdx.x == 0) out[(size_t)blockIdx.y * out_stride + blockIdx.x] = canon(f);
 }
 
 __global__ void k_fp12_pad_one(fp12 *F, size_t stride, size_t ncols) {
@@ -615,14 +616,14 @@
         if (have) fp12_mul(f, f, b); else { f = b; have = true; }
     }
     block_fp12_product(f, sm, ncols < BLS_ACC_BS ? (int)ncols : BLS_ACC_BS);
-    if (threadIdx.x == 0) seg[blockIdx.x] = f;
+    if (threadIdx.x == 0) seg[blockIdx.x] = canon(f);
 }
 
 __global__ void k_combine(const fp12 *seg, int nseg, fp12 *out) {
     if (blockIdx.x != 0 || threadIdx.x != 0) return;
     fp12 F;
     miller_combine(F, seg, nseg);
-    *out = F;
+    *out = canon(F);
 }
 
 __global__ void k_partial_one(fp12 *out, int *flag_out) {
@@ -690,7 +691,7 @@
                     else fp_sub(t, x, y);
                     slots[(w >> 20) & 1023] = t;
                 } else if (w) {
-                    out0[(((w >> 20) & 1023) << 10) | (w & 1023)] = slots[(w >> 10) & 1023];
+                    out0[(((w >> 20) & 1023) << 10) | (w & 1023)] = canon(slots[(w >> 10) & 1023]);
                 }
             } else if (w) {
                 fp x = slots[(w >> 10) & 1023], y = slots[w & 1023], t;
@@ -704,7 +705,7 @@
         }
     }
     const uint32_t *op = prog + 4 + 2 * nin;
-    for (uint32_t e = lane; e < nout; e += 32) out0[op[2 * e + 1] & 0xffffffu] = slots[op[2 * e]];
+    for (uint32_t e = lane; e < nout; e += 32) out0[op[2 * e + 1] & 0xffffffu] = canon(slots[op[2 * e]]);
 }
 __global__ void __launch_bounds__(32) k_fp_program(const uint32_t *prog, const fp *in0, const fp *in1, const fp *cst, fp *out0,
                                                    size_t s_in0, size_t s_in1, size_t s_out) {
@@ -748,7 +749,7 @@
                 if (op == 1) {
                     fp x = slots[w.y & 1023], y = slots[(w.y >> 10) & 1023], t;
                     fp_mul(t, x, y);
-                    slots[(w.x >> 20) & 1023] = t;
+                    slots[(w.x >> 20) & 1023] = canon(t);
                 }
             } else {
                 const uint32_t npos = op == 2 ? (w.x >> 17) & 7 : 0, nneg = op == 2 ? (w.x >> 14) & 7 : 0;
@@ -810,7 +811,7 @@
     if (blockIdx.x != 0 || threadIdx.x != 0) return;
     fp a = *in, r;
     fp_inv_vartime(r, a);
-    *out = r;
+    *out = canon(r);
 }
 
 __global__ void k_final_out(const fp12 *gt, int count, const int *flags, uint8_t *gt_bytes, int *is_one) {
@@ -852,7 +853,7 @@
     else hash_to_g2_jac(h, msgs + i * msg_len, msg_len, dst, dst_len);
     g2_aff a;
     pt_to_affine(a, h);
-    if (out_aff) out_aff[i] = a;
+    if (out_aff) out_aff[i] = canon(a);
     if (out_comp) g2_compress(out_comp + 96 * i, a);
 }
 
@@ -867,7 +868,7 @@
         g1_aff g;
         g.x = G1_GEN_X;
         fp_neg(g.y, G1_GEN_Y);
-        P[n] = g;
+        P[n] = canon(g);
     }
 }
 
@@ -892,7 +893,7 @@
         }
         __syncwarp();
     }
-    if (lane == 0) out[sgm] = acc;
+    if (lane == 0) out[sgm] = canon(acc);
 }
 __global__ void BLS_LB k_g1_to_affine_many(const g1_jac *in, size_t n, g1_aff *out) {
     size_t i = (size_t)blockIdx.x * blockDim.x + threadIdx.x;
@@ -900,7 +901,7 @@
     g1_jac j = in[i];
     g1_aff a;
     pt_to_affine(a, j);
-    out[i] = a;
+    out[i] = canon(a);
 }
 
 __global__ void BLS_LB k_pubkeys_from_bytes(const uint8_t *in, size_t n, int len, int group_check, g1_aff *out,
@@ -911,7 +912,7 @@
     for (int k = 0; k < len; k++) raw[k] = in[i * len + k];
     g1_aff p;
     int err = pubkey_from_bytes(p, raw, len, group_check != 0);
-    out[i] = p;
+    out[i] = canon(p);
     status[i] = (uint8_t)err;
     if (err) atomicAdd(nfail, 1);
 }
@@ -923,7 +924,7 @@
     for (int k = 0; k < len; k++) raw[k] = in[i * len + k];
     g2_aff p;
     int err = signature_from_bytes(p, raw, len, group_check != 0);
-    out[i] = p;
+    out[i] = canon(p);
     status[i] = (uint8_t)err;
     if (err) atomicAdd(nfail, 1);
 }
@@ -961,21 +962,37 @@
     g1_jac j = *in;
     g1_aff a;
     pt_to_affine_vt(a, j);
-    *out = a;
+    *out = canon(a);
 }
 __global__ void k_g2_to_affine(const g2_jac *in, g2_aff *out) {
     if (blockIdx.x != 0 || threadIdx.x != 0) return;
     g2_jac j = *in;
     g2_aff a;
     pt_to_affine_vt(a, j);
-    *out = a;
+    *out = canon(a);
 }
 
 template <class F> __global__ void k_pt_neg(jac_t<F> *p) {
     if (blockIdx.x != 0 || threadIdx.x != 0) return;
     jac_t<F> a = *p, r;
     pt_neg(r, a);
-    *p = r;
+    *p = canon(r);
+}
+
+BLS_NOINLINE void test_fp_redundant_chain(fp &r, const fp &x, const fp &y) {
+    fp s, d, t, u, v;
+    fp_add_nr(s, x, y);
+    fp_sub(d, x, y);
+    fp_mul(t, s, d);
+    fp_sqr(u, t);
+    fp_add(v, u, x);
+    fp_neg(v, v);
+    fp_dbl(v, v);
+    fp_mul(t, v, y);
+    fp_sub(t, t, u);
+    fp_dot2(u, t, x, v, y);
+    fp_add(u, u, u);
+    fp_mul(r, u, t);
 }
 
 __global__ void k_test_fp(int op, const fp *a, const fp *b, size_t n, fp *out) {
@@ -989,9 +1006,10 @@
         case 2: fp_sub(r, x, y); break;
         case 3: fp_sqr(r, x); break;
         case 6: fp_inv_vartime(r, x); break;
+        case 7: test_fp_redundant_chain(r, x, y); break;
         default: fp_inv(r, x); break;
     }
-    out[i] = r;
+    out[i] = canon(r);
 }
 
 template <int WIDE>
@@ -1075,8 +1093,12 @@
     hash_to_g2_jac(hj, msg, 32, dst, 43);
     pt_mul_words(sj, hj, sk, 8);
     sigset s;
-    pt_to_affine(s.pk, pkj);
-    pt_to_affine(s.sig, sj);
+    g1_aff pk;
+    g2_aff sig;
+    pt_to_affine(pk, pkj);
+    pt_to_affine(sig, sj);
+    s.pk = canon(pk);
+    s.sig = canon(sig);
     for (int k = 0; k < 32; k++) s.msg[k] = msg[k];
     out[i] = s;
 }
diff --git a/nim_blscurve_b200/csrc/msm.cuh b/nim_blscurve_b200/csrc/msm.cuh
--- a/nim_blscurve_b200/csrc/msm.cuh
+++ b/nim_blscurve_b200/csrc/msm.cuh
@@ -162,7 +162,7 @@
     pt_set_inf(acc);
     for (uint32_t e = e0; e < e1; e++) {
         if (e == bend) {
-            partials[t + (rank[b] - rank0)] = acc;
+            partials[t + (rank[b] - rank0)] = canon(acc);
             pt_set_inf(acc);
             do { b++; bend = offsets[b + 1]; } while (bend <= e);
         }
@@ -171,7 +171,7 @@
         if (ent & 1) f_neg(p.y, p.y);
         pt_add_affine(acc, acc, p);
     }
-    partials[t + (rank[b] - rank0)] = acc;
+    partials[t + (rank[b] - rank0)] = canon(acc);
 }
 
 __device__ __forceinline__ void msm_bucket_slots(const uint32_t *offsets, const uint32_t *rank, size_t b, uint32_t K,
@@ -201,7 +201,7 @@
         jac_t<F> x = partials[base + t];
         pt_add(acc, acc, x);
     }
-    buckets[b] = acc;
+    buckets[b] = canon(acc);
 }
 
 template <class F>
@@ -231,7 +231,7 @@
         __syncthreads();
         if (threadIdx.x == 0) {
             for (int w = 1; w < 4; w++) { jac_t<F> x = wsum[w]; pt_add(acc, acc, x); }
-            buckets[b] = acc;
+            buckets[b] = canon(acc);
         }
         __syncthreads();
     }
@@ -259,7 +259,7 @@
         pt_mul_words(m, running, &k, 1);
         pt_add(acc, acc, m);
     }
-    segs[t] = acc;
+    segs[t] = canon(acc);
 }
 
 template <class F>
@@ -270,7 +270,7 @@
     if (i + half >= m) return;
     jac_t<F> a = S[r * stride + i], b = S[r * stride + i + half];
     pt_add(a, a, b);
-    S[r * stride + i] = a;
+    S[r * stride + i] = canon(a);
 }
 
 template <class F>
@@ -285,12 +285,12 @@
         jac_t<F> x = W[(size_t)w * stride];
         pt_add(acc, acc, x);
     }
-    if (!last) { *carry = acc; return; }
-    if (out_jac) *out_jac = acc;
+    if (!last) { *carry = canon(acc); return; }
+    if (out_jac) *out_jac = canon(acc);
     if (out_aff) {
         aff_t<F> a;
         pt_to_affine_vt(a, acc);
-        *out_aff = a;
+        *out_aff = canon(a);
     }
 }
 
@@ -308,7 +308,7 @@
         fp_sqr_ni(z2, p.z);
         fp_mul_ni(z, z2, p.z);
     }
-    hom[3 * w] = x; hom[3 * w + 1] = y; hom[3 * w + 2] = z;
+    hom[3 * w] = canon(x); hom[3 * w + 1] = canon(y); hom[3 * w + 2] = canon(z);
 }
 __global__ void k_msm_horner_finish(const fp *hom, g1_jac *out_jac, g1_aff *out_aff) {
     if (blockIdx.x != 0 || threadIdx.x != 0) return;
@@ -317,7 +317,7 @@
         g1_jac j;
         if (fp_is_zero(Z)) pt_set_inf(j);
         else { fp z2; fp_mul_ni(j.x, X, Z); fp_sqr_ni(z2, Z); fp_mul_ni(j.y, Y, z2); j.z = Z; }
-        *out_jac = j;
+        *out_jac = canon(j);
     }
     if (out_aff) {
         g1_aff a;
@@ -325,7 +325,7 @@
         fp_inv_vartime(zi, Z);
         fp_mul_ni(a.x, X, zi);
         fp_mul_ni(a.y, Y, zi);
-        *out_aff = a;
+        *out_aff = canon(a);
     }
 }
 
@@ -343,7 +343,7 @@
         g2_jac j;
         if (fp2_is_zero(Z)) pt_set_inf(j);
         else { fp2 z2; fp2_mul(j.x, X, Z); fp2_sqr(z2, Z); fp2_mul(j.y, Y, z2); j.z = Z; }
-        *out_jac = j;
+        *out_jac = canon(j);
     }
     if (out_aff) {
         g2_aff a;
@@ -351,7 +351,7 @@
         fp2_inv_vartime(zi, Z);
         fp2_mul(a.x, X, zi);
         fp2_mul(a.y, Y, zi);
-        *out_aff = a;
+        *out_aff = canon(a);
     }
 }
 
@@ -373,7 +373,7 @@
     pt_mul_words(r, g, kw, 3);
     g1_aff a;
     pt_to_affine(a, r);
-    points[i] = a;
+    points[i] = canon(a);
     for (int w = 0; w < 4; w++)
         for (int b = 0; b < 8; b++) scalars[32 * i + 8 * w + b] = (uint8_t)(v[2 + w] >> (8 * b));
     scalars[32 * i + 31] &= 0x7f;
diff --git a/nim_blscurve_b200/csrc/pair_route.cuh b/nim_blscurve_b200/csrc/pair_route.cuh
--- a/nim_blscurve_b200/csrc/pair_route.cuh
+++ b/nim_blscurve_b200/csrc/pair_route.cuh
@@ -258,7 +258,9 @@
     l1p = th;
     l2p = la;
 }
-__device__ __forceinline__ void line_store_pair(uint32_t *dst, size_t stride, int s, const fp2h &l0, const fp2h &l1, const fp2h &l2) {
+__device__ __forceinline__ void line_store_pair(uint32_t *dst, size_t stride, int s, const fp2h &l0_in, const fp2h &l1_in,
+                                                const fp2h &l2_in) {
+    const fp2h l0 = canon(l0_in), l1 = canon(l1_in), l2 = canon(l2_in);
     uint32_t *d = dst + ((size_t)s * ML_LINE_WORDS + (h_odd() ? 12 : 0)) * stride;
     for (int w = 0; w < 12; w++) {
         d[(size_t)w * stride] = l0.v.l[w];
diff --git a/nim_blscurve_b200/csrc/pairing.cuh b/nim_blscurve_b200/csrc/pairing.cuh
--- a/nim_blscurve_b200/csrc/pairing.cuh
+++ b/nim_blscurve_b200/csrc/pairing.cuh
@@ -175,7 +175,8 @@
 BLS_HD int ml_seg_hi(int j, int nseg) { return 62 - (63 * j) / nseg; }
 BLS_HD int ml_seg_lo(int j, int nseg) { return 62 - (63 * (j + 1)) / nseg + 1; }
 
-BLS_FN void line_store(uint32_t *dst, size_t stride, int s, const fp2 &l0, const fp2 &l1, const fp2 &l2) {
+BLS_FN void line_store(uint32_t *dst, size_t stride, int s, const fp2 &l0_in, const fp2 &l1_in, const fp2 &l2_in) {
+    const fp2 l0 = canon(l0_in), l1 = canon(l1_in), l2 = canon(l2_in);
     uint32_t *d = dst + (size_t)s * ML_LINE_WORDS * stride;
     for (int w = 0; w < 12; w++) {
         d[(size_t)w * stride] = l0.c0.l[w];
diff --git a/nim_blscurve_b200/csrc/tower.cuh b/nim_blscurve_b200/csrc/tower.cuh
--- a/nim_blscurve_b200/csrc/tower.cuh
+++ b/nim_blscurve_b200/csrc/tower.cuh
@@ -5,6 +5,15 @@
 
 struct fp6 { fp2 c0, c1, c2; };
 struct fp12 { fp6 c0, c1; };
+
+BLS_FN fp12 canon(const fp12 &a) {
+    fp12 r;
+    const fp2 *s = &a.c0.c0;
+    fp2 *d = &r.c0.c0;
+#pragma unroll
+    for (int i = 0; i < 6; i++) fp2_canon(d[i], s[i]);
+    return r;
+}
 
 BLS_FN void fp6_add(fp6 &r, const fp6 &a, const fp6 &b) { fp2_add(r.c0, a.c0, b.c0); fp2_add(r.c1, a.c1, b.c1); fp2_add(r.c2, a.c2, b.c2); }
 BLS_FN void fp6_sub(fp6 &r, const fp6 &a, const fp6 &b) { fp2_sub(r.c0, a.c0, b.c0); fp2_sub(r.c1, a.c1, b.c1); fp2_sub(r.c2, a.c2, b.c2); }
```
